# patrickzbhe/ray-tracing-series-rust

Hardware: AMD Instinct MI355X
Metric: Msamples/s (pixels x spp) on Book-1 final scene (higher is better)
Workload: dtype f64

## Files before the change

### include/rtx_abi.h

```cpp
#ifndef RTX_ABI_H
#define RTX_ABI_H

#include <stddef.h>
#include <stdint.h>

#ifdef __cplusplus
extern "C" {
#endif

#define RTX_ABI_VERSION 1

typedef int32_t rtx_status;
#define RTX_OK 0
#define RTX_EINVAL 1
#define RTX_ENOMEM 2
#define RTX_EHIP 3
#define RTX_EUNSUPPORTED 4
#define RTX_EIO 5
#define RTX_ENCCL 6

typedef int32_t rtx_handle;

typedef struct rtx_builder rtx_builder;
typedef struct rtx_flat rtx_flat;
typedef struct rtx_scene rtx_scene;

int32_t rtx_abi_version(void);
const char* rtx_last_error(void);

rtx_status rtx_builder_create(uint64_t scene_seed, rtx_builder** out);
void rtx_builder_destroy(rtx_builder* b);
double rtx_builder_random(rtx_builder* b);

rtx_handle rtx_solid_color(rtx_builder* b, const double rgb[3]);
rtx_handle rtx_checker(rtx_builder* b, rtx_handle even, rtx_handle odd);
rtx_handle rtx_noise(rtx_builder* b, double scale);
rtx_handle rtx_image_from_ppm(rtx_builder* b, const char* path);
rtx_handle rtx_image_from_texels(rtx_builder* b, int32_t width, int32_t height,
                                 const double* rgb_0_255);
rtx_handle rtx_lambertian(rtx_builder* b, rtx_handle texture);
rtx_handle rtx_metal(rtx_builder* b, const double albedo[3], double fuzz);
rtx_handle rtx_dielectric(rtx_builder* b, double ir);
rtx_handle rtx_diffuse_light(rtx_builder* b, rtx_handle texture);
rtx_handle rtx_isotropic(rtx_builder* b, rtx_handle texture);
rtx_handle rtx_sphere(rtx_builder* b, const double center[3], double radius, rtx_handle mat);
rtx_handle rtx_moving_sphere(rtx_builder* b, const double center0[3], const double center1[3],
                             double time0, double time1, double radius, rtx_handle mat);
rtx_handle rtx_gravity_sphere(rtx_builder* b, const double start[3], double time0, double radius, rtx_handle mat);
rtx_handle rtx_triangle(rtx_builder* b, const double v0[3], const double v1[3], const double v2[3],
                        rtx_handle mat);
rtx_handle rtx_xy_rect(rtx_builder* b, double x0, double x1, double y0, double y1, double k, rtx_handle mat);
rtx_handle rtx_xz_rect(rtx_builder* b, double x0, double x1, double y0, double y1, double k, rtx_handle mat);
rtx_handle rtx_yz_rect(rtx_builder* b, double x0, double x1, double y0, double y1, double k, rtx_handle mat);
rtx_handle rtx_rect_prism(rtx_builder* b, const double p0[3], const double p1[3], rtx_handle mat);
rtx_handle rtx_hittable_list_new(rtx_builder* b);
rtx_status rtx_hittable_list_add(rtx_builder* b, rtx_handle list, rtx_handle object);
rtx_handle rtx_bvh_from_list(rtx_builder* b, rtx_handle list, double time0, double time1);
rtx_handle rtx_translate(rtx_builder* b, const double offset[3], rtx_handle object);
rtx_handle rtx_rotate_y(rtx_builder* b, double angle_degrees, rtx_handle object);
rtx_handle rtx_constant_medium(rtx_builder* b, const double rgb[3], double density, rtx_handle boundary);
rtx_handle rtx_triangle_model(rtx_builder* b, const char* path, double scale);
rtx_handle rtx_triangle_mesh(rtx_builder* b, const double* vertices, int64_t n_vertices,
                             const int64_t* faces, int64_t n_faces, rtx_handle mat);

typedef struct RtxCamera {
  double origin[3], lower_left_corner[3], horizontal[3], vertical[3], u[3], v[3], w[3];
  double lens_radius, time1, time2;
} RtxCamera;
rtx_status rtx_camera_new(const double lookfrom[3], const double lookat[3], const double vup[3],
                          double vfov_degrees, double aspect_ratio, double aperture,
                          double focus_dist, double time1, double time2, RtxCamera* out);

typedef struct RtxConfig {
  double aspect_ratio;
  int32_t image_width;
  int32_t samples_per_pixel;
  int32_t max_depth;
  int32_t threads;
  uint64_t seed;
  double background[3];
  int32_t row_chunk_compat;
  int32_t reserved;
  uint64_t sample_buffer_bytes;
} RtxConfig;
rtx_status rtx_config_new(double aspect_ratio, int32_t image_width, int32_t samples_per_pixel,
                          int32_t max_depth, int32_t threads, RtxConfig* out);
int32_t rtx_image_height(const RtxConfig* cfg);

typedef struct RtxSceneOptions {
  double camera_aspect;
  const char* earth_ppm;
  const char* dragon_ply;
  int64_t mesh_triangles;
  int32_t book2_boxes_per_side;
  int32_t book2_spheres;
} RtxSceneOptions;
rtx_status rtx_get_world_cam(rtx_builder* b, int32_t scene_id, const RtxSceneOptions* options,
                             rtx_handle* world_out, RtxCamera* cam_out, double background_out[3]);

typedef struct RtxBuildOptions {
  int32_t max_leaf;
  int32_t sah_bins;
  int32_t reference_bvh;
  int32_t gpu_builder;
  uint64_t bvh_seed;
} RtxBuildOptions;
typedef struct RtxFlatInfo {
  int64_t n_spheres, n_moving_spheres, n_rects, n_triangles;
  int64_t n_nodes, n_refs, n_entries, n_top_level, n_materials, n_textures, n_perlins, n_images, n_texels;
  int64_t total_bytes;
  int32_t max_stack, n_bvh;
  double sah_cost;
  double bvh_build_ms;
  double bvh_device_ms;
  int64_t n_gravity_spheres;
} RtxFlatInfo;
rtx_status rtx_flatten(const rtx_builder* b, rtx_handle world, const RtxBuildOptions* options,
                       rtx_flat** out);
void rtx_flat_destroy(rtx_flat* f);
rtx_status rtx_flat_info(const rtx_flat* f, RtxFlatInfo* out);
int32_t rtx_flat_top_level_kind(const rtx_flat* f, int32_t index);
rtx_status rtx_scene_upload(const rtx_flat* f, rtx_scene** out);
rtx_status rtx_scene_upload_f32(const rtx_flat* f, rtx_scene** out);
int32_t rtx_scene_is_f32(const rtx_scene* s);
void rtx_scene_destroy(rtx_scene* s);
rtx_status rtx_scene_trim(rtx_scene* s);

typedef struct RtxFrame {
  double* accum_rgb;
  uint8_t* rgb8;
} RtxFrame;
typedef struct RtxRenderStats {
  uint64_t samples, rays, box_tests, sphere_tests, moving_sphere_tests, rect_tests, triangle_tests;
  uint64_t scatters, texels, perlin_calls;
  double trace_ms, reduce_ms, tonemap_ms;
  int32_t trace_launches, passes;
  uint64_t sample_buffer_bytes;
  int32_t trace_kernel;
  int32_t reserved;
} RtxRenderStats;
enum {
  RTX_KERNEL_SIMPLE = 0,
  RTX_KERNEL_PERSISTENT = 1,
  RTX_KERNEL_STREAM = 2,
  RTX_KERNEL_VOTE = 3,
  RTX_KERNEL_LDS = 4,
  RTX_KERNEL_WQ = 5,
  RTX_KERNEL_WORLD = 6,
  RTX_KERNEL_WAVEFRONT = 7
};
const char* rtx_trace_kernel_name(int32_t kernel);
rtx_status rtx_render(const rtx_scene* s, const RtxCamera* cam, const RtxConfig* cfg, RtxFrame* out);

typedef struct RtxShard {
  int32_t shard_index, shard_count, block_rows, reserved;
} RtxShard;
int32_t rtx_shard_rows(const RtxConfig* cfg, const RtxShard* shard);
rtx_status rtx_render_device(const rtx_scene* s, const RtxCamera* cam, const RtxConfig* cfg,
                             const RtxShard* shard, double* d_accum_rgb, uint8_t* d_rgb8,
                             void* hip_stream, RtxRenderStats* stats);
rtx_status rtx_render_count(const rtx_scene* s, const RtxCamera* cam, const RtxConfig* cfg,
                            const RtxShard* shard, RtxRenderStats* stats);

typedef struct rtx_multi rtx_multi;
typedef struct RtxMultiStats {
  double render_ms_max;
  double total_ms;
  uint64_t gathered_bytes;
  int32_t n_shards, n_devices, used_rccl;
  int32_t rccl_ranks;
  double gather_ms;
  double render_ms[16];
} RtxMultiStats;
rtx_status rtx_multi_create(const rtx_flat* f, int32_t n_shards, const int32_t* device_ids, int32_t block_rows,
                            rtx_multi** out);
rtx_status rtx_multi_create_f32(const rtx_flat* f, int32_t n_shards, const int32_t* device_ids, int32_t block_rows,
                                rtx_multi** out);
void rtx_multi_destroy(rtx_multi* m);
rtx_status rtx_multi_render(rtx_multi* m, const RtxCamera* cam, const RtxConfig* cfg, RtxFrame* out, RtxMultiStats* stats);
rtx_status rtx_render_multi(const rtx_flat* f, const RtxCamera* cam, const RtxConfig* cfg, int32_t n_gpus, RtxFrame* out);

typedef struct rtx_progressive rtx_progressive;
typedef struct RtxNoiseStats {
  int32_t spp_done;
  int32_t pixels;
  int32_t pixels_above;
  int32_t reserved;
  double max_rel_err, mean_rel_err, target_rel_err;
} RtxNoiseStats;
rtx_status rtx_progressive_create(const rtx_scene* s, const RtxCamera* cam, const RtxConfig* cfg, const RtxShard* shard,
                                  rtx_progressive** out);
void rtx_progressive_destroy(rtx_progressive* p);
int32_t rtx_progressive_spp(const rtx_progressive* p);
rtx_status rtx_progressive_add(rtx_progressive* p, int32_t n_samples, void* hip_stream, RtxRenderStats* stats);
rtx_status rtx_progressive_read(const rtx_progressive* p, RtxFrame* out, double* sumsq_rgb);
rtx_status rtx_progressive_stats(rtx_progressive* p, double target_rel_err, RtxNoiseStats* out);
rtx_status rtx_progressive_until(rtx_progressive* p, int32_t batch, double target_rel_err, RtxNoiseStats* out);

typedef struct RtxAdaptiveStats {
  int32_t spp_done;
  int32_t min_spp;
  int32_t pixels;
  int32_t pixels_active;
  int32_t pixels_above;
  int32_t reserved;
  uint64_t samples;
  double max_rel_err, mean_rel_err;
  double target_rel_err;
} RtxAdaptiveStats;
rtx_status rtx_progressive_add_adaptive(rtx_progressive* p, int32_t n_samples, int32_t min_spp, double target_rel_err,
                                        void* hip_stream, RtxRenderStats* stats);
rtx_status rtx_progressive_until_adaptive(rtx_progressive* p, int32_t batch, int32_t min_spp, double target_rel_err,
                                          RtxAdaptiveStats* out);
rtx_status rtx_progressive_pixel_spp(const rtx_progressive* p, int32_t* spp);

typedef struct RtxDenoiseParams {
  int32_t iterations, feature_spp, demodulate, reserved;
  double sigma_luminance, sigma_normal, sigma_albedo;
} RtxDenoiseParams;
rtx_status rtx_progressive_features(rtx_progressive* p, int32_t feature_spp, float* albedo_rgb, float* normal_xyz);
rtx_status rtx_progressive_denoise(rtx_progressive* p, const RtxDenoiseParams* params, double* mean_rgb, uint8_t* rgb8);
rtx_status rtx_device_denoise(const double* mean_rgb, const double* var_rgb, const float* albedo_rgb, const float* normal_xyz,
                              int32_t width, int32_t height, const RtxDenoiseParams* params, double* out_mean_rgb,
                              uint8_t* out_rgb8);

rtx_status rtx_render_scene_with_time(const rtx_scene* s, double t0, double t1, const char* path, int32_t row_chunk_compat,
                                      const RtxConfig* overrides);

rtx_status rtx_write_ppm(const char* path, int32_t width, int32_t height, const uint8_t* rgb8);

rtx_status rtx_device_math(int32_t fn, const double* x, const double* y, int64_t n, double* out);
rtx_status rtx_device_stream(uint64_t seed, uint64_t pixel, uint32_t sample, int32_t n, double* out);
rtx_status rtx_device_retire(const double* S, const double* Q, uint32_t npix, const uint32_t* active, uint32_t n,
                             uint32_t spp, double target, int32_t* counts, uint32_t* next, uint32_t* kept);
rtx_status rtx_device_noise_reduce(const double* S, const double* Q, const int32_t* counts, uint32_t npix, uint32_t spp,
                                   double target, double* max_r, double* sum_r, uint64_t* above);

const void* rtx_builder_graph(const rtx_builder* b);
const void* rtx_flat_arrays(const rtx_flat* f);

#ifdef __cplusplus
}
#endif
#endif
```

### ray-tracing-series-rust_amd/api.py

```python
import ctypes as C
import os
import sys

import numpy as np

_PKG_DIR = os.path.dirname(os.path.abspath(__file__))
_LIB_PATH = os.environ.get("RTX_LIBRARY") or os.path.join(_PKG_DIR, "lib", "librtx_hip.so")

RTX_OK, RTX_EINVAL, RTX_ENOMEM, RTX_EHIP, RTX_EUNSUPPORTED, RTX_EIO, RTX_ENCCL = 0, 1, 2, 3, 4, 5, 6
_STATUS_NAMES = {0: "RTX_OK", 1: "RTX_EINVAL", 2: "RTX_ENOMEM", 3: "RTX_EHIP", 4: "RTX_EUNSUPPORTED", 5: "RTX_EIO", 6: "RTX_ENCCL"}

SCENE_CHECKERED_SPHERES, SCENE_TWO_PERLIN, SCENE_EARTH, SCENE_SIMPLE_LIGHT = 0, 1, 2, 3
SCENE_CORNELL_BOX, SCENE_CORNELL_SMOKE, SCENE_BOOK2_FINAL, SCENE_MOVING_TEST = 4, 5, 6, 7
SCENE_RANDOM_MOVING, SCENE_BENCHMARK_TEST, SCENE_TRIANGLE_TEST, SCENE_STANFORD_DRAGON = 8, 9, 10, 11
SCENE_TRIANGULAR_PRISM, SCENE_BOOK1_HEAD, SCENE_BOOK1_CANONICAL, SCENE_EMPTY = 12, 13, 100, 101


class RtxError(RuntimeError):
    def __init__(self, status, message):
        super().__init__("%s: %s" % (_STATUS_NAMES.get(status, status), message))
        self.status = status


class RtxCamera(C.Structure):
    _fields_ = [(n, C.c_double * 3) for n in ("origin", "lower_left_corner", "horizontal", "vertical", "u", "v", "w")] + \
               [("lens_radius", C.c_double), ("time1", C.c_double), ("time2", C.c_double)]


class RtxConfig(C.Structure):
    _fields_ = [("aspect_ratio", C.c_double), ("image_width", C.c_int32), ("samples_per_pixel", C.c_int32),
                ("max_depth", C.c_int32), ("threads", C.c_int32), ("seed", C.c_uint64),
                ("background", C.c_double * 3), ("row_chunk_compat", C.c_int32), ("reserved", C.c_int32),
                ("sample_buffer_bytes", C.c_uint64)]


class RtxSceneOptions(C.Structure):
    _fields_ = [("camera_aspect", C.c_double), ("earth_ppm", C.c_char_p), ("dragon_ply", C.c_char_p),
                ("mesh_triangles", C.c_int64), ("book2_boxes_per_side", C.c_int32), ("book2_spheres", C.c_int32)]


class RtxBuildOptions(C.Structure):
    _fields_ = [("max_leaf", C.c_int32), ("sah_bins", C.c_int32), ("reference_bvh", C.c_int32), ("gpu_builder", C.c_int32),
                ("bvh_seed", C.c_uint64)]


class RtxFlatInfo(C.Structure):
    _fields_ = [(n, C.c_int64) for n in ("n_spheres", "n_moving_spheres", "n_rects", "n_triangles", "n_nodes",
                                         "n_refs", "n_entries", "n_top_level", "n_materials", "n_textures",
                                         "n_perlins", "n_images", "n_texels", "total_bytes")] + \
               [("max_stack", C.c_int32), ("n_bvh", C.c_int32), ("sah_cost", C.c_double), ("bvh_build_ms", C.c_double),
                ("bvh_device_ms", C.c_double), ("n_gravity_spheres", C.c_int64)]


class RtxFrame(C.Structure):
    _fields_ = [("accum_rgb", C.POINTER(C.c_double)), ("rgb8", C.POINTER(C.c_uint8))]


class RtxRenderStats(C.Structure):
    _fields_ = [(n, C.c_uint64) for n in ("samples", "rays", "box_tests", "sphere_tests", "moving_sphere_tests",
                                          "rect_tests", "triangle_tests", "scatters", "texels", "perlin_calls")] + \
               [("trace_ms", C.c_double), ("reduce_ms", C.c_double), ("tonemap_ms", C.c_double),
                ("trace_launches", C.c_int32), ("passes", C.c_int32), ("sample_buffer_bytes", C.c_uint64),
                ("trace_kernel", C.c_int32), ("reserved", C.c_int32)]


class RtxMultiStats(C.Structure):
    _fields_ = [("render_ms_max", C.c_double), ("total_ms", C.c_double), ("gathered_bytes", C.c_uint64),
                ("n_shards", C.c_int32), ("n_devices", C.c_int32), ("used_rccl", C.c_int32), ("rccl_ranks", C.c_int32),
                ("gather_ms", C.c_double), ("render_ms", C.c_double * 16)]


class RtxShard(C.Structure):
    _fields_ = [("shard_index", C.c_int32), ("shard_count", C.c_int32), ("block_rows", C.c_int32), ("reserved", C.c_int32)]


class RtxNoiseStats(C.Structure):
    _fields_ = [("spp_done", C.c_int32), ("pixels", C.c_int32), ("pixels_above", C.c_int32), ("reserved", C.c_int32),
                ("max_rel_err", C.c_double), ("mean_rel_err", C.c_double), ("target_rel_err", C.c_double)]


class RtxAdaptiveStats(C.Structure):
    _fields_ = [("spp_done", C.c_int32), ("min_spp", C.c_int32), ("pixels", C.c_int32), ("pixels_active", C.c_int32),
                ("pixels_above", C.c_int32), ("reserved", C.c_int32), ("samples", C.c_uint64),
                ("max_rel_err", C.c_double), ("mean_rel_err", C.c_double), ("target_rel_err", C.c_double)]


class RtxDenoiseParams(C.Structure):
    _fields_ = [("iterations", C.c_int32), ("feature_spp", C.c_int32), ("demodulate", C.c_int32), ("reserved", C.c_int32),
                ("sigma_luminance", C.c_double), ("sigma_normal", C.c_double), ("sigma_albedo", C.c_double)]


_D3 = C.POINTER(C.c_double)
_F3 = C.POINTER(C.c_float)
_VP = C.c_void_p
_H = C.c_int32
ABI = {
    "rtx_abi_version": (C.c_int32, []),
    "rtx_last_error": (C.c_char_p, []),
    "rtx_trace_kernel_name": (C.c_char_p, [C.c_int32]),
    "rtx_builder_create": (C.c_int32, [C.c_uint64, C.POINTER(_VP)]),
    "rtx_builder_destroy": (None, [_VP]),
    "rtx_builder_random": (C.c_double, [_VP]),
    "rtx_solid_color": (_H, [_VP, _D3]),
    "rtx_checker": (_H, [_VP, _H, _H]),
    "rtx_noise": (_H, [_VP, C.c_double]),
    "rtx_image_from_ppm": (_H, [_VP, C.c_char_p]),
    "rtx_image_from_texels": (_H, [_VP, C.c_int32, C.c_int32, _D3]),
    "rtx_lambertian": (_H, [_VP, _H]),
    "rtx_metal": (_H, [_VP, _D3, C.c_double]),
    "rtx_dielectric": (_H, [_VP, C.c_double]),
    "rtx_diffuse_light": (_H, [_VP, _H]),
    "rtx_isotropic": (_H, [_VP, _H]),
    "rtx_sphere": (_H, [_VP, _D3, C.c_double, _H]),
    "rtx_moving_sphere": (_H, [_VP, _D3, _D3, C.c_double, C.c_double, C.c_double, _H]),
    "rtx_triangle": (_H, [_VP, _D3, _D3, _D3, _H]),
    "rtx_gravity_sphere": (_H, [_VP, _D3, C.c_double, C.c_double, _H]),
    "rtx_render_scene_with_time": (C.c_int32, [_VP, C.c_double, C.c_double, C.c_char_p, C.c_int32, C.POINTER(RtxConfig)]),
    "rtx_xy_rect": (_H, [_VP] + [C.c_double] * 5 + [_H]),
    "rtx_xz_rect": (_H, [_VP] + [C.c_double] * 5 + [_H]),
    "rtx_yz_rect": (_H, [_VP] + [C.c_double] * 5 + [_H]),
    "rtx_rect_prism": (_H, [_VP, _D3, _D3, _H]),
    "rtx_hittable_list_new": (_H, [_VP]),
    "rtx_hittable_list_add": (C.c_int32, [_VP, _H, _H]),
    "rtx_bvh_from_list": (_H, [_VP, _H, C.c_double, C.c_double]),
    "rtx_translate": (_H, [_VP, _D3, _H]),
    "rtx_rotate_y": (_H, [_VP, C.c_double, _H]),
    "rtx_constant_medium": (_H, [_VP, _D3, C.c_double, _H]),
    "rtx_triangle_model": (_H, [_VP, C.c_char_p, C.c_double]),
    "rtx_triangle_mesh": (_H, [_VP, _D3, C.c_int64, C.POINTER(C.c_int64), C.c_int64, _H]),
    "rtx_camera_new": (C.c_int32, [_D3, _D3, _D3] + [C.c_double] * 6 + [C.POINTER(RtxCamera)]),
    "rtx_config_new": (C.c_int32, [C.c_double, C.c_int32, C.c_int32, C.c_int32, C.c_int32, C.POINTER(RtxConfig)]),
    "rtx_image_height": (C.c_int32, [C.POINTER(RtxConfig)]),
    "rtx_flat_top_level_kind": (C.c_int32, [_VP, C.c_int32]),
    "rtx_scene_trim": (C.c_int32, [_VP]),
    "rtx_multi_create": (C.c_int32, [_VP, C.c_int32, C.POINTER(C.c_int32), C.c_int32, C.POINTER(_VP)]),
    "rtx_multi_create_f32": (C.c_int32, [_VP, C.c_int32, C.POINTER(C.c_int32), C.c_int32, C.POINTER(_VP)]),
    "rtx_multi_destroy": (None, [_VP]),
    "rtx_multi_render": (C.c_int32, [_VP, C.POINTER(RtxCamera), C.POINTER(RtxConfig), C.POINTER(RtxFrame), C.POINTER(RtxMultiStats)]),
    "rtx_render_multi": (C.c_int32, [_VP, C.POINTER(RtxCamera), C.POINTER(RtxConfig), C.c_int32, C.POINTER(RtxFrame)]),
    "rtx_get_world_cam": (C.c_int32, [_VP, C.c_int32, C.POINTER(RtxSceneOptions), C.POINTER(_H), C.POINTER(RtxCamera), _D3]),
    "rtx_flatten": (C.c_int32, [_VP, _H, C.POINTER(RtxBuildOptions), C.POINTER(_VP)]),
    "rtx_flat_destroy": (None, [_VP]),
    "rtx_flat_info": (C.c_int32, [_VP, C.POINTER(RtxFlatInfo)]),
    "rtx_scene_upload": (C.c_int32, [_VP, C.POINTER(_VP)]),
    "rtx_scene_upload_f32": (C.c_int32, [_VP, C.POINTER(_VP)]),
    "rtx_scene_is_f32": (C.c_int32, [_VP]),
    "rtx_scene_destroy": (None, [_VP]),
    "rtx_render": (C.c_int32, [_VP, C.POINTER(RtxCamera), C.POINTER(RtxConfig), C.POINTER(RtxFrame)]),
    "rtx_shard_rows": (C.c_int32, [C.POINTER(RtxConfig), C.POINTER(RtxShard)]),
    "rtx_render_device": (C.c_int32, [_VP, C.POINTER(RtxCamera), C.POINTER(RtxConfig), C.POINTER(RtxShard),
                                      _VP, _VP, _VP, C.POINTER(RtxRenderStats)]),
    "rtx_render_count": (C.c_int32, [_VP, C.POINTER(RtxCamera), C.POINTER(RtxConfig), C.POINTER(RtxShard),
                                     C.POINTER(RtxRenderStats)]),
    "rtx_write_ppm": (C.c_int32, [C.c_char_p, C.c_int32, C.c_int32, C.POINTER(C.c_uint8)]),
    "rtx_device_math": (C.c_int32, [C.c_int32, _D3, _D3, C.c_int64, _D3]),
    "rtx_device_stream": (C.c_int32, [C.c_uint64, C.c_uint64, C.c_uint32, C.c_int32, _D3]),
    "rtx_device_retire": (C.c_int32, [_D3, _D3, C.c_uint32, C.POINTER(C.c_uint32), C.c_uint32, C.c_uint32, C.c_double,
                                      C.POINTER(C.c_int32), C.POINTER(C.c_uint32), C.POINTER(C.c_uint32)]),
    "rtx_device_noise_reduce": (C.c_int32, [_D3, _D3, C.POINTER(C.c_int32), C.c_uint32, C.c_uint32, C.c_double, _D3, _D3,
                                            C.POINTER(C.c_uint64)]),
    "rtx_progressive_create": (C.c_int32, [_VP, C.POINTER(RtxCamera), C.POINTER(RtxConfig), C.POINTER(RtxShard), C.POINTER(_VP)]),
    "rtx_progressive_destroy": (None, [_VP]),
    "rtx_progressive_spp": (C.c_int32, [_VP]),
    "rtx_progressive_add": (C.c_int32, [_VP, C.c_int32, _VP, C.POINTER(RtxRenderStats)]),
    "rtx_progressive_read": (C.c_int32, [_VP, C.POINTER(RtxFrame), _D3]),
    "rtx_progressive_stats": (C.c_int32, [_VP, C.c_double, C.POINTER(RtxNoiseStats)]),
    "rtx_progressive_until": (C.c_int32, [_VP, C.c_int32, C.c_double, C.POINTER(RtxNoiseStats)]),
    "rtx_progressive_add_adaptive": (C.c_int32, [_VP, C.c_int32, C.c_int32, C.c_double, _VP, C.POINTER(RtxRenderStats)]),
    "rtx_progressive_until_adaptive": (C.c_int32, [_VP, C.c_int32, C.c_int32, C.c_double, C.POINTER(RtxAdaptiveStats)]),
    "rtx_progressive_pixel_spp": (C.c_int32, [_VP, C.POINTER(C.c_int32)]),
    "rtx_progressive_features": (C.c_int32, [_VP, C.c_int32, _F3, _F3]),
    "rtx_progressive_denoise": (C.c_int32, [_VP, C.POINTER(RtxDenoiseParams), _D3, C.POINTER(C.c_uint8)]),
    "rtx_device_denoise": (C.c_int32, [_D3, _D3, _F3, _F3, C.c_int32, C.c_int32, C.POINTER(RtxDenoiseParams), _D3,
                                       C.POINTER(C.c_uint8)]),
    "rtx_builder_graph": (_VP, [_VP]),
    "rtx_flat_arrays": (_VP, [_VP]),
}


def _load():
    if not os.path.exists(_LIB_PATH):
        raise ImportError(
            "HIP library %s is missing: run `python __graft_entry__.py` (or ray-tracing-series-rust_amd/build.py). "
            "This package has no CPU fallback." % _LIB_PATH)
    lib = C.CDLL(_LIB_PATH)
    for name, (res, args) in ABI.items():
        fn = getattr(lib, name)
        fn.restype = res
        fn.argtypes = args
    return lib


lib = _load()
LIB_PATH = _LIB_PATH


def last_error():
    return (lib.rtx_last_error() or b"").decode("utf-8", "replace")


def _check(status):
    if status != RTX_OK:
        raise RtxError(status, last_error())


def _v3(v):
    a = (C.c_double * 3)(float(v[0]), float(v[1]), float(v[2]))
    return a


def _handle(h):
    if h < 0:
        raise RtxError(RTX_EINVAL, last_error())
    return h


class Camera:

    @staticmethod
    def new(lookfrom, lookat, vup, vfov, aspect_ratio, aperture, focus_dist, time1, time2):
        cam = RtxCamera()
        _check(lib.rtx_camera_new(_v3(lookfrom), _v3(lookat), _v3(vup), vfov, aspect_ratio, aperture, focus_dist,
                                  time1, time2, C.byref(cam)))
        return cam


class Config:

    @staticmethod
    def new(aspect_ratio, image_width, samples_per_pixel, max_depth, threads, seed=1, background=(0.7, 0.8, 1.0),
            row_chunk_compat=False, sample_buffer_bytes=0):
        cfg = RtxConfig()
        _check(lib.rtx_config_new(aspect_ratio, image_width, samples_per_pixel, max_depth, threads, C.byref(cfg)))
        cfg.seed = seed
        cfg.background[0], cfg.background[1], cfg.background[2] = background
        cfg.row_chunk_compat = 1 if row_chunk_compat else 0
        cfg.sample_buffer_bytes = sample_buffer_bytes
        return cfg


def image_height(cfg):
    return lib.rtx_image_height(C.byref(cfg))


class Builder:

    def __init__(self, scene_seed=1):
        p = _VP()
        _check(lib.rtx_builder_create(scene_seed, C.byref(p)))
        self._p = p

    def __del__(self):
        p, self._p = getattr(self, "_p", None), None
        if p:
            lib.rtx_builder_destroy(p)

    @property
    def ptr(self):
        return self._p

    def graph_ptr(self):
        return lib.rtx_builder_graph(self._p)

    def random(self):
        return lib.rtx_builder_random(self._p)

    def solid_color(self, rgb):
        return _handle(lib.rtx_solid_color(self._p, _v3(rgb)))

    def checker(self, even, odd):
        return _handle(lib.rtx_checker(self._p, even, odd))

    def checker_from_colors(self, even_rgb, odd_rgb):
        return self.checker(self.solid_color(even_rgb), self.solid_color(odd_rgb))

    def noise(self, scale):
        return _handle(lib.rtx_noise(self._p, scale))

    def image_from_ppm(self, path):
        return _handle(lib.rtx_image_from_ppm(self._p, os.fsencode(path)))

    def image_from_texels(self, texels):
        t = np.ascontiguousarray(texels, dtype=np.float64)
        h, w = t.shape[0], t.shape[1]
        return _handle(lib.rtx_image_from_texels(self._p, w, h, t.ctypes.data_as(_D3)))

    def lambertian(self, albedo):
        tex = albedo if isinstance(albedo, int) else self.solid_color(albedo)
        return _handle(lib.rtx_lambertian(self._p, tex))

    def metal(self, albedo, fuzz):
        return _handle(lib.rtx_metal(self._p, _v3(albedo), fuzz))

    def dielectric(self, ir):
        return _handle(lib.rtx_dielectric(self._p, ir))

    def diffuse_light(self, emit):
        tex = emit if isinstance(emit, int) else self.solid_color(emit)
        return _handle(lib.rtx_diffuse_light(self._p, tex))

    def isotropic(self, albedo):
        tex = albedo if isinstance(albedo, int) else self.solid_color(albedo)
        return _handle(lib.rtx_isotropic(self._p, tex))

    def sphere(self, center, radius, mat):
        return _handle(lib.rtx_sphere(self._p, _v3(center), radius, mat))

    def moving_sphere(self, center0, center1, time0, time1, radius, mat):
        return _handle(lib.rtx_moving_sphere(self._p, _v3(center0), _v3(center1), time0, time1, radius, mat))

    def gravity_sphere(self, start, time0, radius, mat):
        return _handle(lib.rtx_gravity_sphere(self._p, _v3(start), time0, radius, mat))

    def triangle(self, v0, v1, v2, mat):
        return _handle(lib.rtx_triangle(self._p, _v3(v0), _v3(v1), _v3(v2), mat))

    def xy_rect(self, x0, x1, y0, y1, k, mat):
        return _handle(lib.rtx_xy_rect(self._p, x0, x1, y0, y1, k, mat))

    def xz_rect(self, x0, x1, y0, y1, k, mat):
        return _handle(lib.rtx_xz_rect(self._p, x0, x1, y0, y1, k, mat))

    def yz_rect(self, x0, x1, y0, y1, k, mat):
        return _handle(lib.rtx_yz_rect(self._p, x0, x1, y0, y1, k, mat))

    def rect_prism(self, p0, p1, mat):
        return _handle(lib.rtx_rect_prism(self._p, _v3(p0), _v3(p1), mat))

    def hittable_list(self, objects=()):
        lst = _handle(lib.rtx_hittable_list_new(self._p))
        for o in objects:
            self.list_add(lst, o)
        return lst

    def list_add(self, lst, obj):
        _check(lib.rtx_hittable_list_add(self._p, lst, obj))

    def bvh_from_list(self, lst, time0, time1):
        return _handle(lib.rtx_bvh_from_list(self._p, lst, time0, time1))

    def translate(self, offset, obj):
        return _handle(lib.rtx_translate(self._p, _v3(offset), obj))

    def rotate_y(self, angle_degrees, obj):
        return _handle(lib.rtx_rotate_y(self._p, angle_degrees, obj))

    def constant_medium(self, rgb, density, boundary):
        return _handle(lib.rtx_constant_medium(self._p, _v3(rgb), density, boundary))

    def triangle_model(self, path, scale):
        return _handle(lib.rtx_triangle_model(self._p, os.fsencode(path), scale))

    def triangle_mesh(self, vertices, faces, mat):
        v = np.ascontiguousarray(vertices, dtype=np.float64).reshape(-1, 3)
        f = np.ascontiguousarray(faces, dtype=np.int64).reshape(-1, 3)
        return _handle(lib.rtx_triangle_mesh(self._p, v.ctypes.data_as(_D3), v.shape[0],
                                             f.ctypes.data_as(C.POINTER(C.c_int64)), f.shape[0], mat))

    def get_world_cam(self, scene_id, camera_aspect=0.0, earth_ppm=None, dragon_ply=None, mesh_triangles=0,
                      book2_boxes_per_side=0, book2_spheres=0):
        opt = RtxSceneOptions(camera_aspect, os.fsencode(earth_ppm) if earth_ppm else None,
                              os.fsencode(dragon_ply) if dragon_ply else None, mesh_triangles,
                              book2_boxes_per_side, book2_spheres)
        world = _H()
        cam = RtxCamera()
        bg = (C.c_double * 3)()
        _check(lib.rtx_get_world_cam(self._p, scene_id, C.byref(opt), C.byref(world), C.byref(cam), bg))
        return world.value, cam, (bg[0], bg[1], bg[2])

    def flatten(self, world, max_leaf=0, sah_bins=0, reference_bvh=False, bvh_seed=0, gpu_builder=False):
        return Flat(self, world, max_leaf, sah_bins, reference_bvh, bvh_seed, gpu_builder)


class Flat:

    def __init__(self, builder, world, max_leaf=0, sah_bins=0, reference_bvh=False, bvh_seed=0, gpu_builder=False):
        opt = RtxBuildOptions(max_leaf, sah_bins, 1 if reference_bvh else 0, 1 if gpu_builder else 0, bvh_seed)
        p = _VP()
        _check(lib.rtx_flatten(builder.ptr, world, C.byref(opt), C.byref(p)))
        self._p = p
        self._builder = builder

    def __del__(self):
        p, self._p = getattr(self, "_p", None), None
        if p:
            lib.rtx_flat_destroy(p)

    @property
    def ptr(self):
        return self._p

    def arrays_ptr(self):
        return lib.rtx_flat_arrays(self._p)

    def info(self):
        info = RtxFlatInfo()
        _check(lib.rtx_flat_info(self._p, C.byref(info)))
        return {n: getattr(info, n) for n, _ in RtxFlatInfo._fields_}

    def top_level_kinds(self):
        n = self.info()["n_top_level"]
        return [lib.rtx_flat_top_level_kind(self._p, i) for i in range(n)]

    def upload(self, f32=False):
        return Scene(self, f32=f32)


class Scene:

    def __init__(self, flat, f32=False):
        p = _VP()
        _check((lib.rtx_scene_upload_f32 if f32 else lib.rtx_scene_upload)(flat.ptr, C.byref(p)))
        self._p = p

    @property
    def is_f32(self):
        return bool(lib.rtx_scene_is_f32(self._p))

    def __del__(self):
        p, self._p = getattr(self, "_p", None), None
        if p:
            lib.rtx_scene_destroy(p)

    @property
    def ptr(self):
        return self._p

    def render(self, cam, cfg, want_accum=True):
        w, h = cfg.image_width, image_height(cfg)
        accum = np.zeros((h, w, 3), dtype=np.float64) if want_accum else None
        rgb8 = np.zeros((h, w, 3), dtype=np.uint8)
        frame = RtxFrame(accum.ctypes.data_as(C.POINTER(C.c_double)) if want_accum else None,
                         rgb8.ctypes.data_as(C.POINTER(C.c_uint8)))
        _check(lib.rtx_render(self._p, C.byref(cam), C.byref(cfg), C.byref(frame)))
        return Screen(w, h, rgb8, accum)

    def trim(self):
        _check(lib.rtx_scene_trim(self._p))

    def render_scene_with_time(self, t0, t1, path, row_chunk_compat=True, overrides=None):
        _check(lib.rtx_render_scene_with_time(self._p, t0, t1, path.encode(), 1 if row_chunk_compat else 0,
                                              C.byref(overrides) if overrides is not None else None))

    def render_device(self, cam, cfg, shard=None, d_accum=0, d_rgb8=0, stream=0, want_stats=False):
        sh = RtxShard(*shard, 0) if shard is not None else None
        stats = RtxRenderStats() if want_stats else None
        _check(lib.rtx_render_device(self._p, C.byref(cam), C.byref(cfg), C.byref(sh) if sh else None,
                                     _VP(d_accum or None), _VP(d_rgb8 or None), _VP(stream or None),
                                     C.byref(stats) if stats else None))
        return stats

    def progressive(self, cam, cfg, shard=None):
        return Progressive(self, cam, cfg, shard)

    def render_count(self, cam, cfg, shard=None):
        sh = RtxShard(*shard, 0) if shard is not None else None
        stats = RtxRenderStats()
        _check(lib.rtx_render_count(self._p, C.byref(cam), C.byref(cfg), C.byref(sh) if sh else None, C.byref(stats)))
        return stats


class Progressive:

    def __init__(self, scene, cam, cfg, shard=None):
        self.scene = scene
        self.width = cfg.image_width
        self.height = shard_rows(cfg, shard) if shard is not None else image_height(cfg)
        sh = RtxShard(*shard, 0) if shard is not None else None
        p = _VP()
        _check(lib.rtx_progressive_create(scene.ptr, C.byref(cam), C.byref(cfg), C.byref(sh) if sh else None, C.byref(p)))
        self._p = p

    def __del__(self):
        p, self._p = getattr(self, "_p", None), None
        if p:
            lib.rtx_progressive_destroy(p)

    @property
    def spp_done(self):
        return lib.rtx_progressive_spp(self._p)

    def add(self, n, stream=0, want_stats=False):
        stats = RtxRenderStats() if want_stats else None
        _check(lib.rtx_progressive_add(self._p, n, _VP(stream or None), C.byref(stats) if stats else None))
        return stats

    def screen(self, want_accum=True):
        accum = np.zeros((self.height, self.width, 3), dtype=np.float64) if want_accum else None
        rgb8 = np.zeros((self.height, self.width, 3), dtype=np.uint8)
        frame = RtxFrame(accum.ctypes.data_as(_D3) if want_accum else None, rgb8.ctypes.data_as(C.POINTER(C.c_uint8)))
        _check(lib.rtx_progressive_read(self._p, C.byref(frame), None))
        return Screen(self.width, self.height, rgb8, accum)

    def moments(self):
        s = np.zeros((self.height, self.width, 3), dtype=np.float64)
        q = np.zeros_like(s)
        frame = RtxFrame(s.ctypes.data_as(_D3), None)
        _check(lib.rtx_progressive_read(self._p, C.byref(frame), q.ctypes.data_as(_D3)))
        return s, q

    def stats(self, target_rel_err=0.0):
        out = RtxNoiseStats()
        _check(lib.rtx_progressive_stats(self._p, target_rel_err, C.byref(out)))
        return out

    def until(self, batch, target_rel_err):
        out = RtxNoiseStats()
        _check(lib.rtx_progressive_until(self._p, batch, target_rel_err, C.byref(out)))
        return out

    def add_adaptive(self, n, min_spp, target_rel_err, stream=0, want_stats=False):
        stats = RtxRenderStats() if want_stats else None
        _check(lib.rtx_progressive_add_adaptive(self._p, n, min_spp, target_rel_err, _VP(stream or None),
                                                C.byref(stats) if stats else None))
        return stats

    def until_adaptive(self, batch, min_spp, target_rel_err):
        out = RtxAdaptiveStats()
        _check(lib.rtx_progressive_until_adaptive(self._p, batch, min_spp, target_rel_err, C.byref(out)))
        return out

    def pixel_spp(self):
        out = np.zeros((self.height, self.width), dtype=np.int32)
        _check(lib.rtx_progressive_pixel_spp(self._p, out.ctypes.data_as(C.POINTER(C.c_int32))))
        return out

    def features(self, feature_spp=4):
        albedo = np.zeros((self.height, self.width, 3), dtype=np.float32)
        normal = np.zeros_like(albedo)
        _check(lib.rtx_progressive_features(self._p, feature_spp, albedo.ctypes.data_as(_F3), normal.ctypes.data_as(_F3)))
        return albedo, normal

    def denoise(self, **params):
        prm = denoise_params(**params)
        accum = np.zeros((self.height, self.width, 3), dtype=np.float64)
        rgb8 = np.zeros((self.height, self.width, 3), dtype=np.uint8)
        _check(lib.rtx_progressive_denoise(self._p, C.byref(prm), accum.ctypes.data_as(_D3),
                                           rgb8.ctypes.data_as(C.POINTER(C.c_uint8))))
        return Screen(self.width, self.height, rgb8, accum)


class MultiScene:

    def __init__(self, flat, n_shards, device_ids=None, block_rows=1, f32=False):
        ids = (C.c_int32 * n_shards)(*device_ids) if device_ids is not None else None
        p = _VP()
        _check((lib.rtx_multi_create_f32 if f32 else lib.rtx_multi_create)(flat.ptr, n_shards, ids, block_rows, C.byref(p)))
        self._p = p

    def __del__(self):
        p, self._p = getattr(self, "_p", None), None
        if p:
            lib.rtx_multi_destroy(p)

    def render(self, cam, cfg, want_accum=True):
        w, h = cfg.image_width, image_height(cfg)
        accum = np.zeros((h, w, 3), dtype=np.float64) if want_accum else None
        rgb8 = np.zeros((h, w, 3), dtype=np.uint8)
        frame = RtxFrame(accum.ctypes.data_as(C.POINTER(C.c_double)) if want_accum else None,
                         rgb8.ctypes.data_as(C.POINTER(C.c_uint8)))
        stats = RtxMultiStats()
        _check(lib.rtx_multi_render(self._p, C.byref(cam), C.byref(cfg), C.byref(frame), C.byref(stats)))
        screen = Screen(w, h, rgb8, accum)
        screen.stats = stats
        return screen


def render_multi(flat, cam, cfg, n_gpus, want_accum=True):
    w, h = cfg.image_width, image_height(cfg)
    accum = np.zeros((h, w, 3), dtype=np.float64) if want_accum else None
    rgb8 = np.zeros((h, w, 3), dtype=np.uint8)
    frame = RtxFrame(accum.ctypes.data_as(C.POINTER(C.c_double)) if want_accum else None,
                     rgb8.ctypes.data_as(C.POINTER(C.c_uint8)))
    _check(lib.rtx_render_multi(flat.ptr, C.byref(cam), C.byref(cfg), n_gpus, C.byref(frame)))
    return Screen(w, h, rgb8, accum)


def trace_kernel_name(kernel):
    return (lib.rtx_trace_kernel_name(kernel) or b"").decode()


def device_math(fn, x, y=None):
    names = {"sin": 0, "cos": 1, "log": 2, "acos": 3, "atan2": 4, "tan": 5, "sqrt": 6, "div": 7, "muladd": 8, "floor": 9, "wide_key": 10}
    x = np.ascontiguousarray(x, dtype=np.float64)
    y = np.ascontiguousarray(y if y is not None else np.ones_like(x), dtype=np.float64)
    out = np.empty_like(x)
    _check(lib.rtx_device_math(names[fn], x.ctypes.data_as(_D3), y.ctypes.data_as(_D3), x.size, out.ctypes.data_as(_D3)))
    return out


def device_stream(seed, pixel, sample, n):
    out = np.empty(n, dtype=np.float64)
    _check(lib.rtx_device_stream(seed, pixel, sample, n, out.ctypes.data_as(_D3)))
    return out


def _moments_arg(S, Q):
    S = np.ascontiguousarray(S, dtype=np.float64).reshape(-1, 3)
    Q = np.ascontiguousarray(Q, dtype=np.float64).reshape(-1, 3)
    if S.shape != Q.shape:
        raise ValueError("S and Q must have the same shape")
    return S, Q


def device_retire(S, Q, active, spp, target, counts):
    S, Q = _moments_arg(S, Q)
    active = np.ascontiguousarray(active, dtype=np.uint32).ravel()
    counts = np.array(counts, dtype=np.int32).ravel()
    if counts.size != S.shape[0]:
        raise ValueError("counts must hold one entry per pixel")
    nxt = np.zeros(max(active.size, 1), dtype=np.uint32)
    kept = C.c_uint32()
    u32 = C.POINTER(C.c_uint32)
    _check(lib.rtx_device_retire(S.ctypes.data_as(_D3), Q.ctypes.data_as(_D3), S.shape[0], active.ctypes.data_as(u32),
                                 active.size, spp, target, counts.ctypes.data_as(C.POINTER(C.c_int32)), nxt.ctypes.data_as(u32),
                                 C.byref(kept)))
    return nxt[:kept.value].copy(), counts


def device_noise_reduce(S, Q, spp, target, counts=None):
    S, Q = _moments_arg(S, Q)
    if counts is not None:
        counts = np.ascontiguousarray(counts, dtype=np.int32).ravel()
        if counts.size != S.shape[0]:
            raise ValueError("counts must hold one entry per pixel")
    max_r, sum_r, above = C.c_double(), C.c_double(), C.c_uint64()
    _check(lib.rtx_device_noise_reduce(S.ctypes.data_as(_D3), Q.ctypes.data_as(_D3),
                                       counts.ctypes.data_as(C.POINTER(C.c_int32)) if counts is not None else None,
                                       S.shape[0], spp, target, C.byref(max_r), C.byref(sum_r), C.byref(above)))
    return max_r.value, sum_r.value, above.value


def denoise_params(**params):
    prm = RtxDenoiseParams()
    names = [n for n, _ in RtxDenoiseParams._fields_ if n != "reserved"]
    for k, v in params.items():
        if k not in names:
            raise TypeError("unknown denoise parameter %r (expected one of %s)" % (k, ", ".join(names)))
        setattr(prm, k, v)
    return prm


def device_denoise(mean, var, albedo, normal, **params):
    mean = np.ascontiguousarray(mean, dtype=np.float64)
    if mean.ndim != 3 or mean.shape[2] != 3:
        raise ValueError("mean must be rows x width x 3")
    var = np.ascontiguousarray(var, dtype=np.float64)
    albedo = np.ascontiguousarray(albedo, dtype=np.float32)
    normal = np.ascontiguousarray(normal, dtype=np.float32)
    for a in (var, albedo, normal):
        if a.shape != mean.shape:
            raise ValueError("mean, var, albedo and normal must have the same shape")
    h, w = mean.shape[:2]
    prm = denoise_params(**params)
    out = np.zeros_like(mean)
    rgb8 = np.zeros(mean.shape, dtype=np.uint8)
    _check(lib.rtx_device_denoise(mean.ctypes.data_as(_D3), var.ctypes.data_as(_D3), albedo.ctypes.data_as(_F3),
                                  normal.ctypes.data_as(_F3), w, h, C.byref(prm), out.ctypes.data_as(_D3),
                                  rgb8.ctypes.data_as(C.POINTER(C.c_uint8))))
    return out, rgb8


def shard_rows(cfg, shard):
    sh = RtxShard(*shard, 0)
    return lib.rtx_shard_rows(C.byref(cfg), C.byref(sh))


class Screen:

    def __init__(self, width, height, rgb8, accum=None):
        self.width, self.height, self.rgb8, self.accum = width, height, rgb8, accum

    def write_to_ppm_file(self, path):
        buf = np.ascontiguousarray(self.rgb8)
        _check(lib.rtx_write_ppm(os.fsencode(path), self.width, self.height, buf.ctypes.data_as(C.POINTER(C.c_uint8))))

    def write_to_ppm(self):
        sys.stdout.flush()
        buf = np.ascontiguousarray(self.rgb8)
        _check(lib.rtx_write_ppm(None, self.width, self.height, buf.ctypes.data_as(C.POINTER(C.c_uint8))))


def render_scene(builder, world, cam, background, config, max_leaf=0):
    cfg = RtxConfig.from_buffer_copy(config)
    cfg.background[0], cfg.background[1], cfg.background[2] = background
    scene = builder.flatten(world, max_leaf=max_leaf).upload()
    return scene.render(cam, cfg)


def render_scene_progressive(builder, world, cam, background, config, batch, target_rel_err, max_leaf=0, adaptive=False,
                             min_spp=2, denoise=False):
    cfg = RtxConfig.from_buffer_copy(config)
    cfg.background[0], cfg.background[1], cfg.background[2] = background
    scene = builder.flatten(world, max_leaf=max_leaf).upload()
    prog = scene.progressive(cam, cfg)
    if adaptive:
        stats = prog.until_adaptive(batch, min_spp, target_rel_err)
    else:
        stats = prog.until(batch, target_rel_err)
    screen = prog.screen()
    if adaptive:
        screen.spp = prog.pixel_spp()
    if denoise:
        noisy, screen = screen, prog.denoise()
        screen.noisy = noisy
        if adaptive:
            screen.spp = noisy.spp
    return screen, stats
```

### ray-tracing-series-rust_amd/build.py

```python
import os
import shutil
import subprocess
import sys

PKG_DIR = os.path.dirname(os.path.abspath(__file__))
REPO_DIR = os.path.dirname(PKG_DIR)
LIB_DIR = os.path.join(PKG_DIR, "lib")
LIB_PATH = os.path.join(LIB_DIR, "librtx_hip.so")
APP_PATH = os.path.join(LIB_DIR, "rtx_render")

HIP_SOURCES = [
    "csrc/hip/render.hip",
    "csrc/hip/render_f32.hip",
    "csrc/hip/lbvh.hip",
    "csrc/hip/abi.cpp",
    "csrc/host/scene_graph.cpp",
    "csrc/host/flatten.cpp",
    "csrc/host/bvh_build.cpp",
    "csrc/host/scenes.cpp",
]
HIP_FLAGS = [
    "--offload-arch=gfx950", "-O3", "-std=c++17", "-ffp-contract=off", "-fPIC",
    "-Wall", "-Wno-unused-function",
]
LICM_FLAGS = ["-Xarch_device", "-mllvm=-disable-machine-licm"]
CFG_FLAGS = ["-Xarch_device", "-mllvm=-structurizecfg-skip-uniform-regions"]
TRACE_SOURCES = ("csrc/hip/render.hip", "csrc/hip/render_f32.hip")
_probed = {}


def _accepted(flags):
    key = " ".join(flags)
    if key not in _probed:
        import tempfile
        with tempfile.TemporaryDirectory() as td:
            src = os.path.join(td, "probe.hip")
            with open(src, "w") as f:
                f.write("#include <hip/hip_runtime.h>\n__global__ void k(float* p) { p[threadIdx.x] = 1.f; }\n")
            rc = subprocess.run([_hipcc(), "--offload-arch=gfx950", "-O3", "-c", src, "-o", os.path.join(td, "probe.o")] + flags,
                                stdout=subprocess.DEVNULL, stderr=subprocess.DEVNULL).returncode
        _probed[key] = list(flags) if rc == 0 else []
    return _probed[key]


def licm_flags():
    return _accepted(LICM_FLAGS)


def cfg_flags():
    return _accepted(CFG_FLAGS)


def trace_flags():
    return licm_flags() + cfg_flags()


def flags_for(src):
    return HIP_FLAGS + (trace_flags() if src in TRACE_SOURCES else []) + os.environ.get("RTX_EXTRA_HIPFLAGS", "").split()


def _hipcc():
    for cand in (shutil.which("hipcc"), "/opt/rocm/bin/hipcc"):
        if cand and os.path.exists(cand):
            return cand
    raise RuntimeError("hipcc not found: the HIP library cannot be built")


def _newest(paths):
    t = 0.0
    for p in paths:
        for root, _, files in os.walk(p) if os.path.isdir(p) else [(os.path.dirname(p), [], [os.path.basename(p)])]:
            for f in files:
                fp = os.path.join(root, f)
                if os.path.exists(fp):
                    t = max(t, os.path.getmtime(fp))
    return t


def needs_build(target, deps):
    return (not os.path.exists(target)) or os.path.getmtime(target) < _newest(deps)


def build_library(force=False, verbose=True):
    deps = [os.path.join(PKG_DIR, "csrc"), os.path.join(REPO_DIR, "include")]
    if not force and not needs_build(LIB_PATH, deps):
        return LIB_PATH
    obj_dir = os.path.join(LIB_DIR, "obj")
    os.makedirs(obj_dir, exist_ok=True)
    jobs = []
    for src in HIP_SOURCES:
        obj = os.path.join(obj_dir, os.path.basename(src).rsplit(".", 1)[0] + ".o")
        if force or needs_build(obj, deps):
            cmd = [_hipcc()] + flags_for(src) + ["-c", os.path.join(PKG_DIR, src), "-o", obj]
            if verbose:
                print("[build]", " ".join(cmd), flush=True)
            jobs.append((cmd, subprocess.Popen(cmd, cwd=PKG_DIR)))
        else:
            jobs.append((None, None))
    for cmd, proc in jobs:
        if proc is not None and proc.wait() != 0:
            for _, other in jobs:
                if other is not None:
                    other.wait()
            raise subprocess.CalledProcessError(proc.returncode, cmd)
    objs = [os.path.join(obj_dir, os.path.basename(src).rsplit(".", 1)[0] + ".o") for src in HIP_SOURCES]
    cmd = [_hipcc(), "--offload-arch=gfx950", "-fPIC", "-shared"] + objs + ["-o", LIB_PATH]
    if verbose:
        print("[build]", " ".join(cmd), flush=True)
    subprocess.run(cmd, check=True, cwd=PKG_DIR)
    import json
    with open(os.path.join(LIB_DIR, "build_flags.json"), "w") as f:
        json.dump({"hip_flags": HIP_FLAGS, "trace_kernel_flags": trace_flags(), "machine_licm_disabled": bool(licm_flags()),
                   "uniform_regions_not_structurized": bool(cfg_flags()), "trace_sources": list(TRACE_SOURCES)}, f, indent=1)
    return LIB_PATH


def build_roofline_tools(force=False, verbose=True):
    mix = os.path.join(LIB_DIR, "kernel_mix.json")
    calib = os.path.join(LIB_DIR, "issue_calib")
    tools = os.path.join(REPO_DIR, "tools")
    deps = [os.path.join(PKG_DIR, "csrc")] + [os.path.join(tools, f) for f in sorted(os.listdir(tools)) if os.path.isfile(os.path.join(tools, f))]
    if not force and not needs_build(mix, deps) and not needs_build(calib, deps):
        return mix
    gen_dir = os.path.join(tools, "_gen")
    os.makedirs(gen_dir, exist_ok=True)
    asm = os.path.join(gen_dir, "render_gfx950.s")
    flags = [f for f in flags_for("csrc/hip/render.hip") if f != "-fPIC"]
    cmds = [
        [_hipcc()] + flags + ["-S", "--cuda-device-only", os.path.join(PKG_DIR, "csrc/hip/render.hip"), "-o", asm],
        [sys.executable, os.path.join(tools, "kernel_mix.py"), asm, mix],
        [sys.executable, os.path.join(tools, "gen_issue_calib.py"), asm, os.path.join(gen_dir, "issue_calib_auto.hip")],
        [_hipcc(), "--offload-arch=gfx950", "-O1", "-std=c++17", os.path.join(gen_dir, "issue_calib_auto.hip"), "-o", calib],
    ]
    for cmd in cmds:
        if verbose:
            print("[build]", " ".join(cmd), flush=True)
        subprocess.run(cmd, check=True, cwd=PKG_DIR)
    return mix


def build_app(force=False, verbose=True):
    src = os.path.join(PKG_DIR, "apps", "rtx_render.cpp")
    if not os.path.exists(src):
        return None
    if not force and not needs_build(APP_PATH, [src, LIB_PATH]):
        return APP_PATH
    cmd = [_hipcc(), "-O2", "-std=c++17", "-ffp-contract=off", src, "-I", os.path.join(REPO_DIR, "include"),
           "-L", LIB_DIR, "-lrtx_hip", "-Wl,-rpath,$ORIGIN", "-o", APP_PATH]
    if verbose:
        print("[build]", " ".join(cmd), flush=True)
    subprocess.run(cmd, check=True, cwd=PKG_DIR)
    return APP_PATH


if __name__ == "__main__":
    force = "--force" in sys.argv
    build_library(force=force)
    build_app(force=force)
    build_roofline_tools(force=force)
```

### ray-tracing-series-rust_amd/csrc/hip/abi.cpp

```cpp
#include <cstdio>
#include <cstdlib>
#include <cstring>
#include <new>
#include <string>
#include "../host/scenes.hpp"
#include "abi_internal.hpp"

namespace rtx {
static thread_local std::string g_last_error;
void set_error(const std::string& msg) { g_last_error = msg; }
}

using namespace rtx;

namespace {
inline rtx_handle checked(rtx_builder* b, int32_t h) {
  if (h < 0) set_error(b->graph.error.empty() ? "invalid argument" : b->graph.error);
  return h;
}
#define NEED_BUILDER(b)                                  \
  if (!(b)) { set_error("NULL builder"); return -1; }
}

extern "C" {

int32_t rtx_abi_version(void) { return RTX_ABI_VERSION; }
const char* rtx_last_error(void) { return g_last_error.c_str(); }
const char* rtx_trace_kernel_name(int32_t kernel) {
  switch (kernel) {
    case RTX_KERNEL_SIMPLE: return "k_trace_simple";
    case RTX_KERNEL_PERSISTENT: return "k_trace_persistent";
    case RTX_KERNEL_STREAM: return "k_trace_stream";
    case RTX_KERNEL_VOTE: return "k_trace_vote";
    case RTX_KERNEL_LDS: return "k_trace_lds";
    case RTX_KERNEL_WQ: return "k_trace_wq";
    case RTX_KERNEL_WORLD: return "k_trace_world";
    case RTX_KERNEL_WAVEFRONT: return "k_wf_trace";
    default: return "?";
  }
}

rtx_status rtx_builder_create(uint64_t scene_seed, rtx_builder** out) {
  if (!out) { set_error("rtx_builder_create: NULL out"); return RTX_EINVAL; }
  *out = new (std::nothrow) rtx_builder(scene_seed);
  if (!*out) { set_error("out of memory"); return RTX_ENOMEM; }
  return RTX_OK;
}
void rtx_builder_destroy(rtx_builder* b) { delete b; }
double rtx_builder_random(rtx_builder* b) { return b ? rt::host_rng_f64(b->graph.rng) : 0.0; }

rtx_handle rtx_solid_color(rtx_builder* b, const double rgb[3]) { NEED_BUILDER(b); if (!rgb) { set_error("NULL rgb"); return -1; } return checked(b, b->graph.solid_color(rgb)); }
rtx_handle rtx_checker(rtx_builder* b, rtx_handle even, rtx_handle odd) { NEED_BUILDER(b); return checked(b, b->graph.checker(even, odd)); }
rtx_handle rtx_noise(rtx_builder* b, double scale) { NEED_BUILDER(b); return checked(b, b->graph.noise(scale)); }
rtx_handle rtx_image_from_ppm(rtx_builder* b, const char* path) { NEED_BUILDER(b); if (!path) { set_error("NULL path"); return -1; } return checked(b, b->graph.image_from_ppm(path)); }
rtx_handle rtx_image_from_texels(rtx_builder* b, int32_t w, int32_t h, const double* t) { NEED_BUILDER(b); return checked(b, b->graph.image_from_texels(w, h, t)); }

rtx_handle rtx_lambertian(rtx_builder* b, rtx_handle tex) { NEED_BUILDER(b); return checked(b, b->graph.lambertian(tex)); }
rtx_handle rtx_metal(rtx_builder* b, const double albedo[3], double fuzz) { NEED_BUILDER(b); if (!albedo) { set_error("NULL albedo"); return -1; } return checked(b, b->graph.metal(albedo, fuzz)); }
rtx_handle rtx_dielectric(rtx_builder* b, double ir) { NEED_BUILDER(b); return checked(b, b->graph.dielectric(ir)); }
rtx_handle rtx_diffuse_light(rtx_builder* b, rtx_handle tex) { NEED_BUILDER(b); return checked(b, b->graph.diffuse_light(tex)); }
rtx_handle rtx_isotropic(rtx_builder* b, rtx_handle tex) { NEED_BUILDER(b); return checked(b, b->graph.isotropic(tex)); }

rtx_handle rtx_sphere(rtx_builder* b, const double c[3], double r, rtx_handle mat) { NEED_BUILDER(b); if (!c) { set_error("NULL center"); return -1; } return checked(b, b->graph.sphere(c, r, mat)); }
rtx_handle rtx_gravity_sphere(rtx_builder* b, const double start[3], double time0, double radius, rtx_handle mat) {
  if (!b || !start) { set_error("rtx_gravity_sphere: NULL argument"); return -1; }
  return checked(b, b->graph.gravity_sphere(start, time0, radius, mat));
}
rtx_handle rtx_moving_sphere(rtx_builder* b, const double c0[3], const double c1[3], double t0, double t1, double r, rtx_handle mat) {
  NEED_BUILDER(b);
  if (!c0 || !c1) { set_error("NULL center"); return -1; }
  return checked(b, b->graph.moving_sphere(c0, c1, t0, t1, r, mat));
}
rtx_handle rtx_triangle(rtx_builder* b, const double v0[3], const double v1[3], const double v2[3], rtx_handle mat) {
  NEED_BUILDER(b);
  if (!v0 || !v1 || !v2) { set_error("NULL vertex"); return -1; }
  return checked(b, b->graph.triangle(v0, v1, v2, mat));
}
rtx_handle rtx_xy_rect(rtx_builder* b, double x0, double x1, double y0, double y1, double k, rtx_handle mat) { NEED_BUILDER(b); return checked(b, b->graph.rect(H_XY_RECT, x0, x1, y0, y1, k, mat)); }
rtx_handle rtx_xz_rect(rtx_builder* b, double x0, double x1, double y0, double y1, double k, rtx_handle mat) { NEED_BUILDER(b); return checked(b, b->graph.rect(H_XZ_RECT, x0, x1, y0, y1, k, mat)); }
rtx_handle rtx_yz_rect(rtx_builder* b, double x0, double x1, double y0, double y1, double k, rtx_handle mat) { NEED_BUILDER(b); return checked(b, b->graph.rect(H_YZ_RECT, x0, x1, y0, y1, k, mat)); }
rtx_handle rtx_rect_prism(rtx_builder* b, const double p0[3], const double p1[3], rtx_handle mat) {
  NEED_BUILDER(b);
  if (!p0 || !p1) { set_error("NULL corner"); return -1; }
  return checked(b, b->graph.rect_prism(p0, p1, mat));
}
rtx_handle rtx_hittable_list_new(rtx_builder* b) { NEED_BUILDER(b); return b->graph.list_new(); }
rtx_status rtx_hittable_list_add(rtx_builder* b, rtx_handle list, rtx_handle object) {
  if (!b) { set_error("NULL builder"); return RTX_EINVAL; }
  if (!b->graph.list_add(list, object)) { set_error(b->graph.error); return RTX_EINVAL; }
  return RTX_OK;
}
rtx_handle rtx_bvh_from_list(rtx_builder* b, rtx_handle list, double t0, double t1) { NEED_BUILDER(b); return checked(b, b->graph.bvh_from_list(list, t0, t1)); }
rtx_handle rtx_translate(rtx_builder* b, const double offset[3], rtx_handle obj) { NEED_BUILDER(b); if (!offset) { set_error("NULL offset"); return -1; } return checked(b, b->graph.translate(offset, obj)); }
rtx_handle rtx_rotate_y(rtx_builder* b, double angle, rtx_handle obj) { NEED_BUILDER(b); return checked(b, b->graph.rotate_y(angle, obj)); }
rtx_handle rtx_constant_medium(rtx_builder* b, const double rgb[3], double density, rtx_handle boundary) {
  NEED_BUILDER(b);
  if (!rgb) { set_error("NULL rgb"); return -1; }
  return checked(b, b->graph.constant_medium(rgb, density, boundary));
}
rtx_handle rtx_triangle_model(rtx_builder* b, const char* path, double scale) { NEED_BUILDER(b); if (!path) { set_error("NULL path"); return -1; } return checked(b, b->graph.triangle_model(path, scale)); }
rtx_handle rtx_triangle_mesh(rtx_builder* b, const double* vertices, int64_t n_vertices, const int64_t* faces, int64_t n_faces, rtx_handle mat) {
  NEED_BUILDER(b);
  if (!vertices || !faces || n_vertices < 0 || n_faces < 0) { set_error("triangle_mesh: NULL or negative"); return -1; }
  return checked(b, b->graph.triangle_mesh(vertices, n_vertices, faces, n_faces, mat));
}

rtx_status rtx_camera_new(const double lookfrom[3], const double lookat[3], const double vup[3],
                          double vfov, double aspect_ratio, double aperture, double focus_dist,
                          double time1, double time2, RtxCamera* out) {
  if (!lookfrom || !lookat || !vup || !out) { set_error("rtx_camera_new: NULL argument"); return RTX_EINVAL; }
  if (!(time1 < time2)) { set_error("rtx_camera_new: time1 >= time2 (gen_range(time1..time2) panics, camera.rs:69)"); return RTX_EINVAL; }
  rt::FlatCamera c = camera_new(lookfrom, lookat, vup, vfov, aspect_ratio, aperture, focus_dist, time1, time2);
  static_assert(sizeof(RtxCamera) == sizeof(rt::FlatCamera), "camera layout");
  memcpy(out, &c, sizeof(c));
  return RTX_OK;
}

rtx_status rtx_config_new(double aspect_ratio, int32_t image_width, int32_t samples_per_pixel,
                          int32_t max_depth, int32_t threads, RtxConfig* out) {
  if (!out) { set_error("rtx_config_new: NULL out"); return RTX_EINVAL; }
  if (threads <= 0) { set_error("Config::new: assert!(threads > 0)"); return RTX_EINVAL; }
  if (image_width <= 0) { set_error("Config::new: assert!(image_width > 0)"); return RTX_EINVAL; }
  if (samples_per_pixel <= 0) { set_error("Config::new: assert!(samples_per_pixel > 0)"); return RTX_EINVAL; }
  if (max_depth <= 0) { set_error("Config::new: assert!(max_depth > 0)"); return RTX_EINVAL; }
  memset(out, 0, sizeof(*out));
  out->aspect_ratio = aspect_ratio;
  out->image_width = image_width;
  out->samples_per_pixel = samples_per_pixel;
  out->max_depth = max_depth;
  out->threads = threads;
  out->seed = 1;
  out->background[0] = 0.7; out->background[1] = 0.8; out->background[2] = 1.0;
  return RTX_OK;
}

int32_t rtx_image_height(const RtxConfig* cfg) {
  if (!cfg) return 0;
  return rt::rt_f64_as_i32((double)cfg->image_width / cfg->aspect_ratio);
}

int32_t rtx_shard_rows(const RtxConfig* cfg, const RtxShard* shard) {
  if (!cfg) return 0;
  int32_t h = rtx_image_height(cfg);
  RtxShard sh = {0, 1, 1, 0};
  if (shard) sh = *shard;
  if (sh.shard_count <= 0 || sh.block_rows <= 0) return 0;
  int n = 0;
  for (int32_t j = 0; j < h; ++j)
    if ((j / sh.block_rows) % sh.shard_count == sh.shard_index) ++n;
  return n;
}

rtx_status rtx_get_world_cam(rtx_builder* b, int32_t scene_id, const RtxSceneOptions* options,
                             rtx_handle* world_out, RtxCamera* cam_out, double background_out[3]) {
  if (!b || !world_out || !cam_out || !background_out) { set_error("rtx_get_world_cam: NULL argument"); return RTX_EINVAL; }
  SceneOptions opt;
  if (options) {
    opt.camera_aspect = options->camera_aspect;
    opt.earth_ppm = options->earth_ppm;
    opt.dragon_ply = options->dragon_ply;
    if (options->mesh_triangles > 0) opt.mesh_triangles = options->mesh_triangles;
    if (options->book2_boxes_per_side > 0) opt.book2_boxes_per_side = options->book2_boxes_per_side;
    if (options->book2_spheres > 0) opt.book2_spheres = options->book2_spheres;
  }
  WorldCam wc;
  std::string err;
  if (!get_world_cam(b->graph, scene_id, opt, &wc, &err)) {
    set_error(err);
    return scene_id == RTX_SCENE_RANDOM_MOVING ? RTX_EUNSUPPORTED : RTX_EINVAL;
  }
  *world_out = wc.world;
  memcpy(cam_out, &wc.cam, sizeof(wc.cam));
  background_out[0] = wc.background[0]; background_out[1] = wc.background[1]; background_out[2] = wc.background[2];
  return RTX_OK;
}

rtx_status rtx_flatten(const rtx_builder* b, rtx_handle world, const RtxBuildOptions* options, rtx_flat** out) {
  if (!b || !out) { set_error("rtx_flatten: NULL argument"); return RTX_EINVAL; }
  *out = nullptr;
  BuildOptions opt;
  if (options) {
    if (options->max_leaf > 0) opt.max_leaf = options->max_leaf;
    if (options->sah_bins > 0) opt.sah_bins = options->sah_bins;
    opt.reference_bvh = options->reference_bvh ? 1 : 0;
    opt.gpu_builder = options->gpu_builder ? 1 : 0;
    if (options->bvh_seed) opt.bvh_seed = options->bvh_seed;
  }
  if (const char* e = getenv("RTX_LEAF_FIRST")) opt.leaf_first = atoi(e) != 0 ? 1 : 0;
  if (const char* e = getenv("RTX_MOTION_TOPOLOGY")) opt.motion_topology = atoi(e) != 0 ? 1 : 0;
  rtx_flat* f = new (std::nothrow) rtx_flat();
  if (!f) { set_error("out of memory"); return RTX_ENOMEM; }
  std::string err;
  if (!b->graph.valid_hittable(world)) { delete f; set_error("rtx_flatten: bad world handle"); return RTX_EINVAL; }
  if (!flatten_scene(b->graph, world, opt, &f->scene, &err)) {
    delete f;
    set_error(err);
    return RTX_EUNSUPPORTED;
  }
  *out = f;
  return RTX_OK;
}
void rtx_flat_destroy(rtx_flat* f) { delete f; }

rtx_status rtx_flat_info(const rtx_flat* f, RtxFlatInfo* o) {
  if (!f || !o) { set_error("rtx_flat_info: NULL argument"); return RTX_EINVAL; }
  const FlatScene& s = f->scene;
  o->n_spheres = (int64_t)s.spheres.size(); o->n_moving_spheres = (int64_t)s.moving_spheres.size();
  o->n_rects = (int64_t)s.rects.size(); o->n_triangles = (int64_t)s.triangles.size();
  o->n_nodes = (int64_t)s.nodes.size(); o->n_refs = (int64_t)s.refs.size();
  o->n_entries = (int64_t)s.entries.size(); o->n_top_level = (int64_t)s.top_level.size();
  o->n_materials = (int64_t)s.materials.size(); o->n_textures = (int64_t)s.textures.size();
  o->n_perlins = (int64_t)s.perlins.size(); o->n_images = (int64_t)s.images.size();
  o->n_texels = (int64_t)(s.texels.size() / 3);
  o->total_bytes = (int64_t)s.total_bytes();
  o->max_stack = s.max_stack; o->n_bvh = s.n_bvh; o->sah_cost = s.sah_cost;
  o->bvh_build_ms = s.bvh_build_ms; o->bvh_device_ms = s.bvh_device_ms;
  o->n_gravity_spheres = (int64_t)s.gravity_spheres.size();
  return RTX_OK;
}

int32_t rtx_flat_top_level_kind(const rtx_flat* f, int32_t index) {
  if (!f || index < 0 || (size_t)index >= f->scene.top_level.size()) return -1;
  return f->scene.entries[f->scene.top_level[index]].kind;
}

rtx_status rtx_write_ppm(const char* path, int32_t width, int32_t height, const uint8_t* rgb8) {
  if (width <= 0 || height <= 0 || !rgb8) { set_error("rtx_write_ppm: bad argument"); return RTX_EINVAL; }
  FILE* fp = stdout;
  bool to_file = path && strcmp(path, "-") != 0;
  if (to_file) {
    fp = fopen(path, "wb");
    if (!fp) { set_error(std::string("rtx_write_ppm: cannot open ") + path); return RTX_EIO; }
  }
  std::string buf;
  buf.reserve((size_t)width * height * 12 + 32);
  char line[64];
  snprintf(line, sizeof(line), "P3\n%d %d\n255\n", width, height);
  buf += line;
  for (int32_t j = height - 1; j >= 0; --j) {
    for (int32_t i = 0; i < width; ++i) {
      const uint8_t* p = rgb8 + 3 * ((size_t)j * width + i);
      int n = snprintf(line, sizeof(line), "%u %u %u\n", (unsigned)p[0], (unsigned)p[1], (unsigned)p[2]);
      buf.append(line, (size_t)n);
    }
  }
  size_t wrote = fwrite(buf.data(), 1, buf.size(), fp);
  if (to_file) fclose(fp); else fflush(fp);
  if (wrote != buf.size()) { set_error("rtx_write_ppm: short write"); return RTX_EIO; }
  return RTX_OK;
}

const void* rtx_builder_graph(const rtx_builder* b) { return b ? (const void*)&b->graph : nullptr; }
const void* rtx_flat_arrays(const rtx_flat* f) { return f ? (const void*)&f->scene : nullptr; }

}
```

### ray-tracing-series-rust_amd/csrc/hip/render.hip

```cpp
#include <hip/hip_runtime.h>
#include <cstdio>
#include <cstdlib>
#include <algorithm>
#include <chrono>
#include <cfloat>
#include <cmath>
#include <cstring>
#include <new>
#include <type_traits>
#include <utility>
#include <string>
#include <vector>
#include "../../../include/rtx_abi.h"
#include "../core/cull32.hpp"
#include "../core/integrator.hpp"
#include "../host/flat_scene.hpp"
#include "f32_bridge.hpp"
#ifndef RTX_F32_TU
#include "abi_internal.hpp"
#else
namespace rtx { void set_error(const std::string& msg); }
#endif

namespace rtx {

#include "pass_items.inc"

struct FlatNode4;
typedef const FlatNode4 FlatNode4Dev;
struct WorldDesc;

struct LdsSceneDims {
  uint32_t n_nodes, n_refs, n_spheres, n_moving;
  uint32_t node_dwords;
  uint32_t n_uni;
};

struct VoteTop {
  int32_t n;
  int32_t all_rects;
  int32_t k[8];
  uint32_t ref[8];
  rt::FlatRect rect[8];
};

enum class ForcedKernel { none, simple, vote, world, wavefront };

struct TraceSwitches {
  ForcedKernel kernel = ForcedKernel::none;
  bool diag = false;
  int ring = -1, wide = -1, scene_lds = -1;
  bool vote_top = true, tri_direct = true, mat_lds = true, perlin_lds = true;
  bool mv_common = true, motion = true, motion_axis = true;
  bool single_leaf = true, pass_pipeline = true, validate = false;
  uint32_t chunk = TRACE_CHUNK;
  uint32_t world_threshold = 8;
  uint32_t walk_threshold = 0, regen_min = 0, leaf_weight = 0;
  uint32_t wf_paths = 1u << 22, wf_refill = 16, wf_check = 8;
  int wf_occ = 4;
  bool wf_verbose = false;
};

struct Workspace {
  double* samples = nullptr;
  size_t samples_bytes = 0;
  double* accum = nullptr;
  size_t accum_bytes = 0;
  rt::TraceCounters* counters = nullptr;
  unsigned int* work_counter = nullptr;
  unsigned long long* diag = nullptr;
  hipEvent_t ev[2] = {nullptr, nullptr};
  hipStream_t aux_stream = nullptr;
  hipEvent_t ev_pass[3] = {nullptr, nullptr, nullptr};
  void* wave_mem = nullptr;
  size_t wave_bytes = 0;
  uint32_t* wave_host_ctrl = nullptr;
};

struct VotePlan {
  bool ok = false;
  int32_t bvh_pos = 0;
  int32_t tri_base = -1;
  VoteTop top;
  int blocks_per_cu[2] = {1, 1};
  bool ring[2] = {false, false};
  uint32_t tables = 0;
  size_t tables_bytes = 0;
};

struct WidePlan {
  FlatNode4Dev* nodes4 = nullptr;
  int levels = 0;
  int vote_blocks_per_cu = 1;
};

struct WorldPlan {
  const WorldDesc* desc = nullptr;
  uint32_t mat_lds = 0, tex_lds = 0;
  uint32_t perlin_lds = 0;
  int blocks_per_cu[4][2] = {{1, 1}, {1, 1}, {1, 1}, {1, 1}};
};

struct LdsFit {
  bool ok = false;
  uint32_t ring_cap = 0;
  uint32_t levels = 0;
  LdsSceneDims dims = {0, 0, 0, 0, 0, 0};
};

struct LdsPlan {
  LdsFit plain;
  LdsFit motion;
  int motion_axis = -1;
  double motion_t0 = 0.0, motion_t1 = 0.0;
  bool mv_common = false;
  double mv_t0 = 0.0, mv_t1 = 1.0;
};

struct WalkTuning {
  uint32_t walk_threshold = 18;
  uint32_t regen_min = 1;
  uint32_t leaf_weight = 3;
  bool single_leaf = false;
};

struct DeviceScene {
  int device = -1;
  std::vector<void*> allocations;
  rt::SceneView view;
  size_t scene_bytes = 0;
  int n_cu = 256;
  double gravity_time_limit = 1e300;
  TraceSwitches sw;
  Workspace ws;
  VotePlan vote;
  WidePlan wide;
  WorldPlan world;
  LdsPlan lds;
  WalkTuning walk;
};

#define HIP_TRY(expr)                                                                      \
  do {                                                                                     \
    hipError_t _e = (expr);                                                                \
    if (_e != hipSuccess) {                                                                \
      set_error(std::string(#expr) + ": " + hipGetErrorString(_e));                        \
      return RTX_EHIP;                                                                     \
    }                                                                                      \
  } while (0)

template <class T>
static rtx_status upload_array(DeviceScene* ds, const std::vector<T>& v, const T** out) {
  *out = nullptr;
  if (v.empty()) return RTX_OK;
  void* p = nullptr;
  size_t bytes = v.size() * sizeof(T);
  HIP_TRY(hipMalloc(&p, bytes));
  ds->allocations.push_back(p);
  HIP_TRY(hipMemcpy(p, v.data(), bytes, hipMemcpyHostToDevice));
  ds->scene_bytes += bytes;
  *out = (const T*)p;
  return RTX_OK;
}

static void free_device_scene(DeviceScene* ds) {
  if (!ds) return;
  Workspace& ws = ds->ws;
  for (void* p : ds->allocations) (void)hipFree(p);
  if (ws.samples) (void)hipFree(ws.samples);
  if (ws.accum) (void)hipFree(ws.accum);
  if (ws.counters) (void)hipFree(ws.counters);
  if (ws.work_counter) (void)hipFree(ws.work_counter);
  if (ws.diag) (void)hipFree(ws.diag);
  if (ws.wave_mem) (void)hipFree(ws.wave_mem);
  if (ws.wave_host_ctrl) (void)hipHostFree(ws.wave_host_ctrl);
  for (int i = 0; i < 2; ++i)
    if (ws.ev[i]) (void)hipEventDestroy(ws.ev[i]);
  for (int i = 0; i < 3; ++i)
    if (ws.ev_pass[i]) (void)hipEventDestroy(ws.ev_pass[i]);
  if (ws.aux_stream) (void)hipStreamDestroy(ws.aux_stream);
  delete ds;
}

template <class T>
__device__ __forceinline__ T dev_load_uniform(const T* p) { return *(const __attribute__((address_space(4))) T*)(p); }

__device__ __forceinline__ unsigned long long wave_ballot(bool p) { return __builtin_amdgcn_ballot_w64(p); }

#define TRACE_BLOCK 256
struct LdsStack {
  int32_t* base;
  int n;
  static constexpr bool kBottom = false;
  __device__ __forceinline__ void reset() { n = 0; }
  __device__ __forceinline__ void push(int32_t v) { base[n * TRACE_BLOCK] = v; ++n; }
  __device__ __forceinline__ int32_t pop() { --n; return base[n * TRACE_BLOCK]; }
  __device__ __forceinline__ bool empty() const { return n == 0; }
};
struct LdsStackB {
  int32_t* base;
  int n;
  static constexpr bool kBottom = true;
  __device__ __forceinline__ void reset() { base[0] = 0x7fffffff; n = 1; }
  __device__ __forceinline__ void init() { reset(); }
  __device__ __forceinline__ void push(int32_t v) { base[n * TRACE_BLOCK] = v; ++n; }
  __device__ __forceinline__ int32_t pop() { --n; return base[n * TRACE_BLOCK]; }
  __device__ __forceinline__ int32_t top() const { return base[(n - 1) * TRACE_BLOCK]; }
  __device__ __forceinline__ bool empty() const { return n <= 1; }
};

__device__ __forceinline__ void flush_counters(const rt::TraceCounters& c, rt::TraceCounters* g) {
  atomicAdd(&g->box_tests, c.box_tests);
  atomicAdd(&g->sphere_tests, c.sphere_tests);
  atomicAdd(&g->moving_sphere_tests, c.moving_sphere_tests);
  atomicAdd(&g->rect_tests, c.rect_tests);
  atomicAdd(&g->triangle_tests, c.triangle_tests);
  atomicAdd(&g->scatters, c.scatters);
  atomicAdd(&g->texels, c.texels);
  atomicAdd(&g->perlin_calls, c.perlin_calls);
  atomicAdd(&g->rays, c.rays);
  atomicAdd(&g->samples, c.samples);
}

#include "trace_basic.inc"
#include "trace_vote.inc"
#include "trace_world.inc"
#include "trace_lds.inc"
#include "trace_wave.inc"
#include "post_kernels.inc"
#include "denoise.inc"

static int shard_row_count(int32_t height, const RtxShard& sh, int32_t row_limit) {
  int n = 0;
  for (int32_t j = 0; j < height && j < row_limit; ++j)
    if ((j / sh.block_rows) % sh.shard_count == sh.shard_index) ++n;
  return n;
}

static rtx_status validate(const void* s, const RtxCamera* cam, const RtxConfig* cfg,
                           const RtxShard* shard, RtxShard* sh_out) {
  if (!s || !cam || !cfg) { set_error("render: NULL scene, camera or config"); return RTX_EINVAL; }
  if (cfg->threads <= 0 || cfg->image_width <= 0 || cfg->samples_per_pixel <= 0 || cfg->max_depth <= 0) {
    set_error("render: Config::new asserts threads, image_width, samples_per_pixel, max_depth > 0 (world.rs:36-40)");
    return RTX_EINVAL;
  }
  if (rtx_image_height(cfg) <= 0) { set_error("render: image height <= 0 (Screen::new asserts, screen.rs:14)"); return RTX_EINVAL; }
  if (!(cam->time1 < cam->time2)) { set_error("render: camera time1 >= time2 (gen_range panics on an empty range, camera.rs:69)"); return RTX_EINVAL; }
  RtxShard sh = {0, 1, 1, 0};
  if (shard) sh = *shard;
  if (sh.shard_count <= 0 || sh.shard_index < 0 || sh.shard_index >= sh.shard_count || sh.block_rows <= 0) {
    set_error("render: bad shard");
    return RTX_EINVAL;
  }
  *sh_out = sh;
  return RTX_OK;
}

static rt::RenderParams make_params(const RtxCamera* cam, const RtxConfig* cfg) {
  rt::RenderParams rp;
  static_assert(sizeof(RtxCamera) == 24 * sizeof(double) && sizeof(rt::FlatCamera) == 24 * sizeof(rt::real), "camera layout");
  for (int k = 0; k < 24; ++k) ((rt::real*)&rp.cam)[k] = (rt::real)((const double*)cam)[k];
  rp.background = rt::v3(cfg->background[0], cfg->background[1], cfg->background[2]);
  rp.image_width = cfg->image_width;
  rp.image_height = rtx_image_height(cfg);
  rp.samples_per_pixel = cfg->samples_per_pixel;
  rp.max_depth = cfg->max_depth;
  rp.seed = cfg->seed;
  return rp;
}

static TraceSwitches read_switches() {
  auto num = [](const char* n, int lo, int hi, uint32_t dflt) { const char* s = getenv(n); return s && atoi(s) >= lo && atoi(s) <= hi ? (uint32_t)atoi(s) : dflt; };
  auto flag = [](const char* n) { const char* s = getenv(n); return s ? (atoi(s) != 0 ? 1 : 0) : -1; };
  TraceSwitches sw;
  if (const char* k = getenv("RTX_TRACE_KERNEL")) {
    const std::string s = k;
    if (s == "simple") sw.kernel = ForcedKernel::simple;
    else if (s == "vote" || s == "vote_diag") sw.kernel = ForcedKernel::vote;
    else if (s == "world" || s == "world_diag") sw.kernel = ForcedKernel::world;
    else if (s == "wavefront") sw.kernel = ForcedKernel::wavefront;
    sw.diag = s == "vote_diag" || s == "world_diag";
  }
  sw.ring = flag("RTX_RING"); sw.wide = flag("RTX_WIDE"); sw.scene_lds = flag("RTX_SCENE_LDS");
  sw.vote_top = flag("RTX_VOTE_TOP") != 0; sw.tri_direct = flag("RTX_TRI_DIRECT") != 0;
  sw.mat_lds = flag("RTX_MAT_LDS") != 0; sw.perlin_lds = flag("RTX_PERLIN_LDS") != 0;
  sw.mv_common = flag("RTX_MV_COMMON") != 0; sw.motion = flag("RTX_MOTION") != 0; sw.motion_axis = flag("RTX_MOTION_AXIS") != 0;
  sw.single_leaf = flag("RTX_SINGLE_LEAF") != 0; sw.pass_pipeline = flag("RTX_PASS_PIPELINE") != 0;
  sw.validate = getenv("RTX_VALIDATE") != nullptr;
  sw.chunk = num("RTX_CHUNK", 64, 65536, sw.chunk);
  sw.world_threshold = num("RTX_WORLD_THRESHOLD", 0, 64, sw.world_threshold);
  sw.walk_threshold = num("RTX_WALK_THRESHOLD", 1, 64, 0); sw.regen_min = num("RTX_REGEN_MIN", 1, 64, 0); sw.leaf_weight = num("RTX_LEAF_WEIGHT", 1, 64, 0);
  const char* wp = getenv("RTX_WF_PATHS");
  if (wp && atol(wp) >= 256 && atol(wp) <= (1l << 27)) sw.wf_paths = (uint32_t)atol(wp);
  sw.wf_refill = num("RTX_WF_REFILL", 1, 64, sw.wf_refill); sw.wf_check = num("RTX_WF_CHECK", 1, 4096, sw.wf_check);
  sw.wf_occ = (int)num("RTX_WF_OCC", 4, 6, (uint32_t)sw.wf_occ); sw.wf_verbose = getenv("RTX_WF_VERBOSE") != nullptr;
  return sw;
}

static size_t stack_bytes(uint32_t levels) { return (size_t)levels * TRACE_BLOCK * sizeof(int32_t); }

template <class K>
static int occupancy(K kernel, size_t lds) {
  int nb = 0;
  return hipOccupancyMaxActiveBlocksPerMultiprocessor(&nb, kernel, TRACE_BLOCK, lds) == hipSuccess ? nb : 0;
}

static uint32_t grid_size(uint32_t total, uint32_t block, uint64_t resident) {
  const uint64_t want = ((uint64_t)total + block - 1) / block;
  return (uint32_t)(want < resident ? want : resident);
}

static rtx_status grow_buffer(void** p, size_t* bytes, size_t need, hipStream_t stream) {
  if (need <= *bytes) return RTX_OK;
  if (*p) { HIP_TRY(hipStreamSynchronize(stream)); HIP_TRY(hipFree(*p)); *p = nullptr; *bytes = 0; }
  HIP_TRY(hipMalloc(p, need));
  *bytes = need;
  return RTX_OK;
}

struct PassArgs {
  rt::RenderParams rp;
  ShardMap sm;
  uint32_t s_begin, total, npix;
  double* samples;
  unsigned int* work_counter;
  hipStream_t stream;
  int preset;
  uint32_t feat;
  uint32_t stack_levels;
  size_t stack_lds;
  const uint32_t* active;
};

template <class Launch>
static void with_map(const PassArgs& a, Launch launch) {
  if (a.active) launch(ActiveMap{a.sm, a.active});
  else launch(a.sm);
}

template <class Launch>
static rtx_status run_diag(DeviceScene* ds, hipStream_t stream, Launch launch, const char* tag, int width, const char* const* names,
                           int n, unsigned long long (&h)[24]) {
  if (!ds->ws.diag) HIP_TRY(hipMalloc((void**)&ds->ws.diag, sizeof(h)));
  HIP_TRY(hipMemsetAsync(ds->ws.diag, 0, sizeof(h), stream));
  launch();
  HIP_TRY(hipStreamSynchronize(stream));
  HIP_TRY(hipMemcpy(h, ds->ws.diag, sizeof(h), hipMemcpyDeviceToHost));
  for (int k = 0; k < n; ++k)
    fprintf(stderr, "[%s] %-*s executions %llu lanes %llu mean lanes %.2f\n", tag, width, names[k], h[2 * k], h[2 * k + 1],
            h[2 * k] ? (double)h[2 * k + 1] / (double)h[2 * k] : 0.0);
  return RTX_OK;
}

struct LeafScan { uint32_t max_count = 0, max_end = 0; };
static LeafScan scan_leaves(const FlatScene& fs) {
  LeafScan s;
  for (const rt::FlatNode& nd : fs.nodes)
    for (int ch = 0; ch < 2; ++ch)
      if (nd.child[ch] < 0) {
        s.max_count = std::max(s.max_count, rt::leaf_count(nd.child[ch]));
        s.max_end = std::max(s.max_end, rt::leaf_first(nd.child[ch]) + rt::leaf_count(nd.child[ch]));
      }
  return s;
}

static void plan_vote(DeviceScene* ds, const FlatScene& fs) {
  VotePlan& p = ds->vote;
  const TraceSwitches& sw = ds->sw;
  const size_t lds = stack_bytes((uint32_t)fs.max_stack + 1u), lds_ring = lds + (TRACE_BLOCK / 64) * ring_bytes(64);
  const bool ring_fits = lds_ring <= 64 * 1024;
  auto fit = [&](int preset, int nb0, int nb1, bool ring_by_default) {
    p.ring[preset] = ring_by_default && nb1 > 0 && nb1 >= nb0 && ring_fits;
    if (sw.ring >= 0 && nb1 > 0 && ring_fits) p.ring[preset] = sw.ring != 0;
    const int nb = p.ring[preset] ? nb1 : nb0;
    if (nb > 0) p.blocks_per_cu[preset] = nb;
  };
  fit(0, occupancy(k_trace_vote<P_SPHERES, false, false, false>, lds), occupancy(k_trace_vote<P_SPHERES, false, true, false>, lds_ring), true);
  fit(1, occupancy(k_trace_vote<P_MESH, false, false, false>, lds), occupancy(k_trace_vote<P_MESH, false, true, false>, lds_ring), false);

  memset(&p.top, 0, sizeof(p.top));
  p.top.n = -1;
  int n_bvh = 0, n_other = 0;
  for (size_t k = 0; k < fs.top_level.size(); ++k) {
    const int32_t kind = fs.entries[fs.top_level[k]].kind;
    if (kind == rt::ENTRY_BVH) { ++n_bvh; p.bvh_pos = (int32_t)k; }
    else if (kind != rt::ENTRY_PRIM) ++n_other;
  }
  p.ok = n_bvh == 1 && n_other == 0;
  if (p.ok && fs.top_level.size() <= 9 && sw.vote_top) {
    p.top.n = 0;
    p.top.all_rects = 1;
    for (size_t k = 0; k < fs.top_level.size(); ++k) {
      if ((int32_t)k == p.bvh_pos) continue;
      const rt::PrimRef ref = (rt::PrimRef)fs.entries[fs.top_level[k]].a;
      p.top.k[p.top.n] = (int32_t)k;
      p.top.ref[p.top.n] = (uint32_t)ref;
      if (rt::primref_type(ref) == rt::PRIM_RECT) p.top.rect[p.top.n] = fs.rects[rt::primref_index(ref)];
      else p.top.all_rects = 0;
      p.top.n += 1;
    }
    if (!p.top.all_rects) p.top.n = -1;
  }
  if (p.ok) {
    const rt::FlatEntry& be = fs.entries[fs.top_level[p.bvh_pos]];
    bool pure = be.c > 0 && rt::primref_type(fs.refs[be.b]) == rt::PRIM_TRIANGLE;
    const uint32_t t0 = pure ? rt::primref_index(fs.refs[be.b]) : 0u;
    for (int32_t k = 0; pure && k < be.c; ++k)
      pure = fs.refs[be.b + k] == rt::make_primref(rt::PRIM_TRIANGLE, t0 + (uint32_t)k);
    if (pure && sw.tri_direct) p.tri_base = (int32_t)t0;
  }
  if (!fs.materials.empty() && !fs.textures.empty() && fs.materials.size() <= 16 && fs.textures.size() <= 16 && sw.mat_lds) {
    p.tables = (uint32_t)fs.materials.size() | ((uint32_t)fs.textures.size() << 16);
    p.tables_bytes = fs.materials.size() * sizeof(rt::FlatMaterial) + fs.textures.size() * sizeof(rt::FlatTexture);
  }
}

static rtx_status launch_vote_wide(DeviceScene* ds, const PassArgs& a, bool diag) {
  const VotePlan& p = ds->vote;
  const WidePlan& wt = ds->wide;
  uint32_t lds_tables = 0;
  size_t lds = stack_bytes((uint32_t)wt.levels);
  if (p.tables_bytes > 0 && (lds + p.tables_bytes) * (size_t)wt.vote_blocks_per_cu <= 160 * 1024) {
    lds_tables = p.tables;
    lds += p.tables_bytes;
  }
  const uint32_t grid = grid_size(a.total, TRACE_BLOCK, (uint64_t)ds->n_cu * (uint64_t)wt.vote_blocks_per_cu);
  const uint32_t threshold = ds->walk.walk_threshold | (ds->walk.regen_min << 16);
#define LAUNCH_VOTE_WIDE(FEAT, DIAGF, THRESHOLD, MAP)                                                                  \
  hipLaunchKernelGGL(HIP_KERNEL_NAME(k_trace_vote<FEAT, DIAGF, false, true, decltype(MAP)>), dim3(grid), dim3(TRACE_BLOCK), lds, \
                     a.stream, ds->view, a.rp, MAP, a.s_begin, a.total, a.npix, a.samples, a.work_counter,             \
                     DIAGF ? ds->ws.diag : nullptr, ds->walk.leaf_weight, THRESHOLD, (uint32_t)wt.levels,              \
                     (uint32_t)p.bvh_pos, wt.nodes4, p.tri_base, lds_tables, p.top)
  const bool room = (a.feat & ~P_MESH_ROOM) == 0;
  if (diag && room) {
    unsigned long long h[24];
    static const char* const names[6] = {"outer", "regen", "node_step", "leaf_step", "shade_hit", "shade_all"};
    const rtx_status st = run_diag(ds, a.stream, [&] { LAUNCH_VOTE_WIDE(P_MESH_ROOM, true, ds->walk.walk_threshold, a.sm); }, "vote_diag", 10, names, 6, h);
    if (st != RTX_OK) return st;
    if (h[12]) {
      float v[12];
      for (int k = 0; k < 6; ++k) { uint32_t lo = (uint32_t)h[13 + k], hi = (uint32_t)(h[13 + k] >> 32); memcpy(&v[2 * k], &lo, 4); memcpy(&v[2 * k + 1], &hi, 4); }
      fprintf(stderr, "[vote_diag] %llu walks of >= 50000 node steps; the first: origin (%g %g %g) direction (%g %g %g) 1/d (%g %g %g) err2 %g t_min %g t_max %g depth left %llu\n",
              h[12], v[0], v[1], v[2], v[3], v[4], v[5], v[6], v[7], v[8], v[9], v[10], v[11], h[19]);
    }
  } else if (room) {
    with_map(a, [&](auto map) { LAUNCH_VOTE_WIDE(P_MESH_ROOM, false, threshold, map); });
  } else {
    with_map(a, [&](auto map) { LAUNCH_VOTE_WIDE(P_MESH, false, threshold, map); });
  }
#undef LAUNCH_VOTE_WIDE
  return RTX_OK;
}

static rtx_status launch_vote(DeviceScene* ds, const PassArgs& a) {
  const VotePlan& p = ds->vote;
  HIP_TRY(hipMemsetAsync(a.work_counter, 0, sizeof(unsigned int), a.stream));
  const bool diag = ds->sw.kernel == ForcedKernel::vote && ds->sw.diag && !a.active;
  if (a.preset == 1 && ds->wide.nodes4) return launch_vote_wide(ds, a, diag);
  const bool ring = p.ring[a.preset];
  const size_t lds = a.stack_lds + (ring ? (TRACE_BLOCK / 64) * ring_bytes(64) : 0);
  const uint32_t grid = grid_size(a.total, TRACE_BLOCK, (uint64_t)ds->n_cu * (uint64_t)p.blocks_per_cu[a.preset]);
#define LAUNCH_VOTE3(FEAT, DIAGF, RINGF, MAP)                                                                            \
  hipLaunchKernelGGL(HIP_KERNEL_NAME(k_trace_vote<FEAT, DIAGF, RINGF, false, decltype(MAP)>), dim3(grid), dim3(TRACE_BLOCK), lds, \
                     a.stream, ds->view, a.rp, MAP, a.s_begin, a.total, a.npix, a.samples, a.work_counter,              \
                     DIAGF ? ds->ws.diag : nullptr, ds->walk.leaf_weight, ds->walk.walk_threshold, a.stack_levels,      \
                     (uint32_t)p.bvh_pos, (const FlatNode4*)nullptr, p.tri_base, 0u, p.top)
#define LAUNCH_VOTE2(FEAT, RINGF) with_map(a, [&](auto map) { LAUNCH_VOTE3(FEAT, false, RINGF, map); })
#define LAUNCH_VOTE(FEAT) do { if (ring) { LAUNCH_VOTE2(FEAT, true); } else { LAUNCH_VOTE2(FEAT, false); } } while (0)
  if (diag && a.preset == 0) {
    unsigned long long h[24];
    static const char* const names[6] = {"outer", "regen", "node_step", "leaf_step", "shade_hit", "walking"};
    return run_diag(ds, a.stream, [&] {
      if (ring) { LAUNCH_VOTE3(P_SPHERES, true, true, a.sm); } else { LAUNCH_VOTE3(P_SPHERES, true, false, a.sm); }
    }, "vote_diag", 10, names, 6, h);
  }
  if (a.preset == 0) { LAUNCH_VOTE(P_SPHERES); }
  else { LAUNCH_VOTE(P_MESH); }
#undef LAUNCH_VOTE
#undef LAUNCH_VOTE2
#undef LAUNCH_VOTE3
  return RTX_OK;
}

static void validate_wide_tree(const FlatScene& fs, const std::vector<FlatNode4>& wide, int levels) {
  for (const rt::FlatEntry& e : fs.entries) {
    if (e.kind != rt::ENTRY_BVH) continue;
    std::vector<std::pair<int32_t, int>> todo;
    todo.push_back({e.a, 0});
    size_t visited = 0, bad = 0; int deepest = 0;
    while (!todo.empty()) {
      auto [code, below] = todo.back(); todo.pop_back();
      if (code < 0) { if (rt::leaf_first(code) + rt::leaf_count(code) > (uint32_t)e.c) ++bad; continue; }
      if ((size_t)code >= wide.size()) { ++bad; continue; }
      ++visited;
      int nk = 0;
      for (int k = 0; k < 4; ++k) if (wide[code].child[k] != 0x7fffffff) ++nk;
      deepest = std::max(deepest, below + nk);
      for (int k = 0; k < 4; ++k) if (wide[code].child[k] != 0x7fffffff) todo.push_back({wide[code].child[k], below + nk - 1});
    }
    fprintf(stderr, "[rtx] RTX_VALIDATE: BVH root %d refs %d: %zu wide nodes walked, %zu bad codes, deepest stack %d of %d levels, sizeof(real) %zu\n",
            e.a, e.c, visited, bad, deepest, levels, sizeof(rt::real));
  }
}

static rtx_status plan_wide(DeviceScene* ds, const FlatScene& fs) {
  WidePlan& p = ds->wide;
  const bool spheres_preset = (fs.features & ~P_SPHERES) == 0;
  const bool mesh_preset = !spheres_preset && (fs.features & ~P_MESH) == 0;
  const int preset = spheres_preset ? 0 : (mesh_preset ? 1 : 2);
  const bool for_vote = ds->vote.ok && mesh_preset;
  const bool for_world = !(ds->vote.ok && preset < 2) && preset >= 1;
  bool want_wide = (for_vote && fs.nodes.size() >= 4096) || (for_world && fs.nodes.size() >= 256);
  if (ds->sw.wide >= 0) want_wide = (for_vote || for_world) && ds->sw.wide != 0 && !fs.nodes.empty();
  if (!want_wide) return RTX_OK;
  std::vector<FlatNode4> wide(fs.nodes.size());
  memset(wide.data(), 0, wide.size() * sizeof(FlatNode4));
  int peak = 0;
  for (const rt::FlatEntry& e : fs.entries)
    if (e.kind == rt::ENTRY_BVH) peak = std::max(peak, build_wide_nodes(fs.nodes, e.a, &wide));
  p.levels = peak + 1;
  const size_t lds = stack_bytes((uint32_t)p.levels);
  bool ok = lds <= 64 * 1024;
  if (ok && for_vote) {
    const int nb = occupancy(k_trace_vote<P_MESH, false, false, true>, lds);
    ok = nb > 0;
    if (ok) p.vote_blocks_per_cu = nb;
  }
  if (ok) {
    rtx_status st = upload_array(ds, wide, &p.nodes4);
    if (st != RTX_OK) return st;
  }
  if (ds->sw.wide >= 0) fprintf(stderr, "[rtx] RTX_WIDE: 4-wide tree %s (%d stack levels)\n", p.nodes4 ? "on" : "off", p.levels);
  if (ds->sw.validate) validate_wide_tree(fs, wide, p.levels);
  return RTX_OK;
}

static rtx_status plan_world(DeviceScene* ds, const FlatScene& fs) {
  WorldPlan& p = ds->world;
  const TraceSwitches& sw = ds->sw;
  rtx_status st = upload_array(ds, build_world_desc(fs), &p.desc);
  if (st != RTX_OK) return st;
  for (int wd = 0; wd < 2; ++wd) {
    const uint32_t levels = (uint32_t)(wd ? ds->wide.levels : fs.max_stack + 1);
    size_t wl = stack_bytes(levels) + (size_t)WORLD_SLOT_F64 * TRACE_BLOCK * sizeof(rt::real);
    if (wl > 64 * 1024) continue;
    if ((wd != 0) == (ds->wide.nodes4 != nullptr)) {
      const size_t n_p = fs.perlins.size();
      if (n_p >= 1 && n_p <= 2 && sw.perlin_lds && wl + n_p * sizeof(rt::FlatPerlin) <= 52 * 1024) {
        p.perlin_lds = (uint32_t)n_p;
        wl += n_p * sizeof(rt::FlatPerlin);
      }
      const size_t mt = fs.materials.size() * sizeof(rt::FlatMaterial) + fs.textures.size() * sizeof(rt::FlatTexture);
      if (!fs.materials.empty() && !fs.textures.empty() && fs.materials.size() <= 64 && fs.textures.size() <= 64 && sw.mat_lds &&
          wl + mt <= 52 * 1024) {
        p.mat_lds = (uint32_t)fs.materials.size();
        p.tex_lds = (uint32_t)fs.textures.size();
        wl += mt;
      }
    }
    int n = 0;
#define WORLD_OCC(I, FEAT) if ((n = occupancy(wd ? k_trace_world<FEAT, true, WORLD_WPS> : k_trace_world<FEAT, false, WORLD_WPS>, wl)) > 0) p.blocks_per_cu[I][wd] = n
    WORLD_OCC(0, P_BOOK2); WORLD_OCC(1, P_ANY); WORLD_OCC(2, P_ALL); WORLD_OCC(3, P_NO_SPHERE_MEDIA);
#undef WORLD_OCC
  }
  return RTX_OK;
}

static rtx_status launch_world(DeviceScene* ds, const PassArgs& a) {
  const WorldPlan& p = ds->world;
  HIP_TRY(hipMemsetAsync(a.work_counter, 0, sizeof(unsigned int), a.stream));
  const bool wide = ds->wide.nodes4 != nullptr;
  const bool book2 = (a.feat & ~P_BOOK2) == 0;
  const bool has_gravity = (a.feat & rt::F_GRAVITY_SPHERE) != 0;
  const bool no_sphere_media = (a.feat & rt::F_MEDIUM_SPHERE) == 0;
  const uint32_t levels = wide ? (uint32_t)ds->wide.levels : a.stack_levels;
  const size_t lds = stack_bytes(levels) + (size_t)WORLD_SLOT_F64 * TRACE_BLOCK * sizeof(rt::real) +
                     (size_t)p.perlin_lds * sizeof(rt::FlatPerlin) + (size_t)p.mat_lds * sizeof(rt::FlatMaterial) +
                     (size_t)p.tex_lds * sizeof(rt::FlatTexture);
  const int family = has_gravity ? 2 : (book2 ? 0 : (no_sphere_media ? 3 : 1));
  const uint32_t grid = grid_size(a.total, TRACE_BLOCK, (uint64_t)ds->n_cu * (uint64_t)p.blocks_per_cu[family][wide ? 1 : 0]);
  const rt::SceneView& v = ds->view;
#define LAUNCH_WORLD3(FEAT, WIDEF, DIAGF, MAP)                                                                               \
  hipLaunchKernelGGL(HIP_KERNEL_NAME(k_trace_world<FEAT, WIDEF, WORLD_WPS, DIAGF, decltype(MAP)>), dim3(grid), dim3(TRACE_BLOCK), lds, \
                     a.stream, v, a.rp, MAP, a.s_begin, a.total, a.npix, a.samples, a.work_counter, v.entries, v.top_level, v.spheres, \
                     v.moving_spheres, v.rects, v.triangles, v.materials, v.textures, v.refs, ds->wide.nodes4, p.desc,     \
                     ds->walk.leaf_weight, ds->sw.world_threshold, levels, p.perlin_lds, p.mat_lds, p.tex_lds,             \
                     DIAGF ? ds->ws.diag : nullptr)
#define LAUNCH_WORLD2(FEAT, WIDEF) with_map(a, [&](auto map) { LAUNCH_WORLD3(FEAT, WIDEF, false, map); })
#define LAUNCH_WORLD(FEAT) do { if (wide) { LAUNCH_WORLD2(FEAT, true); } else { LAUNCH_WORLD2(FEAT, false); } } while (0)
  if (ds->sw.kernel == ForcedKernel::world && ds->sw.diag && book2 && wide && !a.active) {
    unsigned long long h[24];
    static const char* const names[8] = {"node_step", "leaf_step", "sweep", "shade(lean)", "regen", "direct_entry(all)", "direct_entry(run)", "shade(rare)"};
    return run_diag(ds, a.stream, [&] { LAUNCH_WORLD3(P_BOOK2, true, true, a.sm); }, "world_diag", 18, names, 8, h);
  }
  if (has_gravity) { LAUNCH_WORLD(P_ALL); }
  else if (book2) { LAUNCH_WORLD(P_BOOK2); }
  else if (no_sphere_media) { LAUNCH_WORLD(P_NO_SPHERE_MEDIA); }
  else { LAUNCH_WORLD(P_ANY); }
#undef LAUNCH_WORLD
#undef LAUNCH_WORLD2
#undef LAUNCH_WORLD3
  return RTX_OK;
}

static void fit_lds(LdsFit* f, bool want_ring, uint32_t lds_max) {
  for (uint32_t cap : {64u, 48u, 0u})
    if ((want_ring || cap == 0u) && ldsk_layout(f->levels, cap, f->dims).total <= lds_max) {
      f->ok = true;
      f->ring_cap = cap;
      return;
    }
}

static rtx_status plan_lds(DeviceScene* ds, const FlatScene& fs, const LeafScan& leaves) {
  const bool single_bvh = fs.top_level.size() == 1 && fs.entries[fs.top_level[0]].kind == rt::ENTRY_BVH;
  if (!single_bvh || (fs.features & ~P_SPHERES) != 0 || fs.nodes32.size() > LDSK_MAX_NODES) return RTX_OK;
  LdsPlan& p = ds->lds;
  const TraceSwitches& sw = ds->sw;
  const uint32_t max_end = leaves.max_end, levels = (uint32_t)fs.max_stack + 1u;
  int lds_max = 0;
  (void)hipDeviceGetAttribute(&lds_max, hipDeviceAttributeMaxSharedMemoryPerBlock, ds->device);
  if (lds_max > 160 * 1024) lds_max = 160 * 1024;
  p.plain.levels = levels;
  p.plain.dims = {(uint32_t)fs.nodes32.size(), max_end, max_end, 0u, LDSK_NODE_DWORDS, 0u};
  if (!fs.moving_spheres.empty()) {
    bool same = sw.mv_common;
    for (const rt::FlatMovingSphere& ms : fs.moving_spheres)
      same = same && ms.time0 == fs.moving_spheres[0].time0 && ms.time1 == fs.moving_spheres[0].time1;
    if (same) { p.mv_common = true; p.mv_t0 = (double)fs.moving_spheres[0].time0; p.mv_t1 = (double)fs.moving_spheres[0].time1; }
  }
  if (fs.features & rt::F_MOVING_SPHERE) {
    p.plain.dims.n_uni = (uint32_t)fs.spheres.size();
    p.plain.dims.n_moving = max_end;
    p.plain.dims.n_spheres = 0u;
  }
  p.motion.levels = levels;
  p.motion.dims = p.plain.dims;
  p.motion.dims.node_dwords = LDSK_MOTION_NODE_DWORDS;
  {
    bool moves[3] = {false, false, false};
    for (const rt::FlatMotion32& m : fs.motion32)
      for (int ch = 0; ch < 2; ++ch)
        for (int a = 0; a < 3; ++a) moves[a] = moves[a] || m.dlo[ch][a] != 0.0f || m.dhi[ch][a] != 0.0f;
    if (!fs.motion32.empty() && moves[1] && !moves[0] && !moves[2] && sw.motion_axis) {
      p.motion_axis = 1;
      p.motion.dims.node_dwords = LDSK_MOTION1_NODE_DWORDS;
    }
  }
  if (leaves.max_count <= 4 && max_end <= LDSK_MAX_SLOTS && sw.scene_lds != 0 && lds_max > 0) {
    const bool want_ring = sw.ring != 0;
    fit_lds(&p.plain, want_ring, (uint32_t)lds_max);
    const rt::FlatEntry& be = fs.entries[fs.top_level[0]];
    if (p.plain.ok && !fs.motion32.empty() && (fs.features & rt::F_MOVING_SPHERE) && (double)be.f[0] < (double)be.f[1] && sw.motion) {
      p.motion_t0 = (double)be.f[0]; p.motion_t1 = (double)be.f[1];
      fit_lds(&p.motion, want_ring, (uint32_t)lds_max);
    }
  }
  if (p.plain.ok) {
    hipError_t ae = hipSuccess;
#define LDS_ATTR1(K) if (ae == hipSuccess) ae = hipFuncSetAttribute((const void*)K, hipFuncAttributeMaxDynamicSharedMemorySize, lds_max)
#define LDS_ATTR(FEAT, RINGF, MOTIONF) LDS_ATTR1((k_trace_lds<FEAT, RINGF, MOTIONF>)); LDS_ATTR1((k_trace_lds<FEAT, RINGF, MOTIONF, ActiveMap>))
    LDS_ATTR(P_SPHERES, true, 0u); LDS_ATTR(P_SPHERES, false, 0u); LDS_ATTR(P_STATIC_SPHERES, true, 0u); LDS_ATTR(P_STATIC_SPHERES, false, 0u);
    LDS_ATTR(P_SPHERES, true, 1u); LDS_ATTR(P_SPHERES, false, 1u); LDS_ATTR(P_SPHERES, true, 3u); LDS_ATTR(P_SPHERES, false, 3u);
#undef LDS_ATTR
#undef LDS_ATTR1
    if (ae != hipSuccess) { (void)hipGetLastError(); p.plain.ok = false; }
  }
  if (sw.scene_lds >= 0) {
    auto bytes = [](const LdsFit& f) { return f.ok ? ldsk_layout(f.levels, f.ring_cap, f.dims).total : 0u; };
    fprintf(stderr, "[rtx] RTX_SCENE_LDS: k_trace_lds %s (ring of %u, %u B of LDS); time-aware boxes %s (ring of %u, %u B)\n",
            p.plain.ok ? "on" : "off", p.plain.ring_cap, ldsk_layout(levels, p.plain.ring_cap, p.plain.dims).total,
            p.motion.ok ? "on" : "off", p.motion.ring_cap, bytes(p.motion));
  }
  return RTX_OK;
}

static rtx_status launch_lds(DeviceScene* ds, const PassArgs& a, const RtxCamera* cam) {
  const LdsPlan& p = ds->lds;
  HIP_TRY(hipMemsetAsync(a.work_counter, 0, sizeof(unsigned int), a.stream));
  const bool motion = p.motion.ok && (double)cam->time1 >= p.motion_t0 && (double)cam->time2 <= p.motion_t1;
  const LdsFit& f = motion ? p.motion : p.plain;
  const bool ring = f.ring_cap != 0u;
  const rt::real m_t0 = (rt::real)p.motion_t0, m_inv = (rt::real)(1.0 / (p.motion_t1 - p.motion_t0));
  const LdsKernelLayout L = ldsk_layout(f.levels, f.ring_cap, f.dims);
  const uint32_t grid = grid_size(a.total, LDSK_BLOCK, (uint64_t)ds->n_cu);
  const WalkTuning& wk = ds->walk;
#define LAUNCH_LDS2(FEAT, RINGF, MOTIONF)                                                                               \
  with_map(a, [&](auto map) {                                                                                           \
    hipLaunchKernelGGL(HIP_KERNEL_NAME(k_trace_lds<FEAT, RINGF, MOTIONF, decltype(map)>), dim3(grid), dim3(LDSK_BLOCK), L.total, \
                       a.stream, ds->view, a.rp, map, a.s_begin, a.total, a.npix, a.samples, a.work_counter, wk.leaf_weight, \
                       wk.walk_threshold | (wk.single_leaf ? 0x100u : 0u), ds->sw.chunk, f.ring_cap, f.levels, f.dims,  \
                       m_t0, m_inv, p.mv_common ? 1u : 0u, (rt::real)p.mv_t0, (rt::real)p.mv_t1);                        \
  })
#define LAUNCH_LDS(FEAT, MOTIONF) do { if (ring) { LAUNCH_LDS2(FEAT, true, MOTIONF); } else { LAUNCH_LDS2(FEAT, false, MOTIONF); } } while (0)
  if ((a.feat & ~P_STATIC_SPHERES) == 0) { LAUNCH_LDS(P_STATIC_SPHERES, 0u); }
  else if (motion && p.motion_axis == 1) { LAUNCH_LDS(P_SPHERES, 3u); }
  else if (motion) { LAUNCH_LDS(P_SPHERES, 1u); }
  else { LAUNCH_LDS(P_SPHERES, 0u); }
#undef LAUNCH_LDS
#undef LAUNCH_LDS2
  return RTX_OK;
}

template <bool COUNT>
static void launch_simple(const DeviceScene* ds, const PassArgs& a) {
  const uint32_t grid = grid_size(a.total, TRACE_BLOCK, (uint64_t)ds->n_cu * 8);
#define LAUNCH_SIMPLE2(FEAT, MAP)                                                                                       \
  hipLaunchKernelGGL(HIP_KERNEL_NAME(k_trace_simple<FEAT, COUNT, decltype(MAP)>), dim3(grid), dim3(TRACE_BLOCK), a.stack_lds, \
                     a.stream, ds->view, a.rp, MAP, a.s_begin, a.total, a.npix, a.samples, ds->ws.counters)
#define LAUNCH_SIMPLE(FEAT) with_map(a, [&](auto map) { LAUNCH_SIMPLE2(FEAT, map); })
  if constexpr (COUNT) { LAUNCH_SIMPLE2(P_ALL, a.sm); }
  else {
    if (a.preset == 0) { LAUNCH_SIMPLE(P_SPHERES); }
    else if (a.preset == 1) { LAUNCH_SIMPLE(P_MESH); }
    else { LAUNCH_SIMPLE(P_ALL); }
  }
#undef LAUNCH_SIMPLE
#undef LAUNCH_SIMPLE2
}

static rtx_status wave_pass(DeviceScene* ds, const PassArgs& a) {
  Workspace& ws = ds->ws;
  const hipStream_t stream = a.stream;
  uint32_t P = ds->sw.wf_paths;
  if ((uint64_t)P > (uint64_t)a.total) P = a.total;
  P = (P + WF_SEG - 1u) & ~(WF_SEG - 1u);
  const uint32_t n_seg = P / WF_SEG;
  const size_t R = sizeof(rt::real);
  const size_t bytes = 64 + (size_t)P * (16 + 7 * R + 3 * R + 3 * R + R + 4 + 4 + 4 + 4) + (size_t)n_seg * 8;
  rtx_status st = grow_buffer(&ws.wave_mem, &ws.wave_bytes, bytes, stream);
  if (st != RTX_OK) return st;
  if (!ws.wave_host_ctrl) HIP_TRY(hipHostMalloc((void**)&ws.wave_host_ctrl, 4 * sizeof(uint32_t), hipHostMallocDefault));
  WavePool pool;
  {
    unsigned char* m = (unsigned char*)ws.wave_mem;
    pool.ctrl = (uint32_t*)m; m += 64;
    pool.rng = (unsigned long long*)m; m += (size_t)P * 16;
    pool.ray = (rt::real*)m; m += (size_t)P * 7 * R;
    pool.product = (rt::real*)m; m += (size_t)P * 3 * R;
    pool.output = (rt::real*)m; m += (size_t)P * 3 * R;
    pool.hit_t = (rt::real*)m; m += (size_t)P * R;
    pool.depth = (int32_t*)m; m += (size_t)P * 4;
    pool.g = (uint32_t*)m; m += (size_t)P * 4;
    pool.hit_ref = (uint32_t*)m; m += (size_t)P * 4;
    pool.free_list = (uint32_t*)m; m += (size_t)P * 4;
    pool.n_free = (uint32_t*)m; m += (size_t)n_seg * 4;
    pool.cursor = (uint32_t*)m; m += (size_t)n_seg * 4;
    pool.P = P;
  }
  const int preset = a.preset;
  const bool wide = preset == 1 && ds->wide.nodes4 != nullptr;
  const uint32_t levels = wide ? (uint32_t)ds->wide.levels : a.stack_levels;
  const size_t lds = stack_bytes(levels);
  if (lds > 64 * 1024) { set_error("render: BVH too deep for the LDS traversal stack"); return RTX_EUNSUPPORTED; }
  const bool room = (a.feat & ~P_MESH_ROOM) == 0;
  const int occ = ds->sw.wf_occ;
  const uint32_t leaf_weight = ds->walk.leaf_weight, refill = ds->sw.wf_refill, bvh_pos = (uint32_t)ds->vote.bvh_pos;
#define WF_CASES(X)                                                                                                          \
  if (preset == 0) { X(P_SPHERES, false, 4); }                                                                               \
  else if (!wide) { X(P_MESH, false, 4); }                                                                                   \
  else if (room && occ == 5) { X(P_MESH_ROOM, true, 5); }                                                                    \
  else if (room && occ == 6) { X(P_MESH_ROOM, true, 6); }                                                                    \
  else if (room) { X(P_MESH_ROOM, true, 4); }                                                                                \
  else { X(P_MESH, true, 4); }
  int nb = 0;
  hipError_t oe = hipSuccess;
#define WF_OCC(FEAT, WIDEF, MB) oe = hipOccupancyMaxActiveBlocksPerMultiprocessor(&nb, k_wf_trace<FEAT, WIDEF, MB>, TRACE_BLOCK, lds)
  WF_CASES(WF_OCC)
#undef WF_OCC
  if (oe != hipSuccess || nb <= 0) { (void)hipGetLastError(); nb = 1; }
  const uint32_t tgrid = grid_size(P, TRACE_BLOCK, (uint64_t)ds->n_cu * (uint64_t)nb);
  hipLaunchKernelGGL(k_wf_init, dim3((P + 255u) / 256u), dim3(256), 0, stream, pool);
  uint32_t check_every = ds->sw.wf_check;
  int it = 0;
  for (;; ++it) {
    with_map(a, [&](auto map) {
      hipLaunchKernelGGL(HIP_KERNEL_NAME(k_wf_generate<decltype(map)>), dim3(n_seg), dim3(WF_SEG), 0, stream, pool, a.rp, map,
                         a.s_begin, a.total, a.npix);
    });
    if ((uint32_t)(it + 1) % check_every == 0u) {
      HIP_TRY(hipMemsetAsync(pool.ctrl, 0, 16, stream));
      hipLaunchKernelGGL(k_wf_count, dim3(256), dim3(256), 0, stream, pool);
      HIP_TRY(hipGetLastError());
      HIP_TRY(hipMemcpyAsync(ws.wave_host_ctrl, pool.ctrl, 4 * sizeof(uint32_t), hipMemcpyDeviceToHost, stream));
      HIP_TRY(hipStreamSynchronize(stream));
      if (ws.wave_host_ctrl[0] == 0u) break;
      if (ws.wave_host_ctrl[0] < P / 2u) check_every = 2;
      if (it > 100000000) { set_error("render: wavefront integrator did not converge"); return RTX_EHIP; }
    }
#define WF_LAUNCH(FEAT, WIDEF, MB)                                                                                           \
  do {                                                                                                                       \
    hipLaunchKernelGGL(HIP_KERNEL_NAME(k_wf_trace<FEAT, WIDEF, MB>), dim3(tgrid), dim3(TRACE_BLOCK), lds, stream, ds->view, pool, \
                       leaf_weight, refill, bvh_pos, ds->wide.nodes4, ds->vote.tri_base);                                    \
    hipLaunchKernelGGL(HIP_KERNEL_NAME(k_wf_shade<FEAT>), dim3(n_seg), dim3(WF_SEG), 0, stream, ds->view, pool, a.rp, a.samples, bvh_pos); \
  } while (0)
    WF_CASES(WF_LAUNCH)
#undef WF_LAUNCH
  }
#undef WF_CASES
  if (ds->sw.wf_verbose) fprintf(stderr, "[rtx] wavefront: %u slots, %d iterations, %d blocks per CU (%u stack levels)\n", P, it + 1, nb, levels);
  return RTX_OK;
}

static void plan_walk(DeviceScene* ds, const LeafScan& leaves) {
  WalkTuning& w = ds->walk;
  const TraceSwitches& sw = ds->sw;
  w.leaf_weight = leaves.max_count <= 1 ? 1u : 3u;
  w.single_leaf = leaves.max_count <= 1;
  if (ds->wide.nodes4) { w.leaf_weight = 1u; w.walk_threshold = 24u; w.regen_min = 8u; }
  else if (ds->lds.plain.ok) w.walk_threshold = 12u;
  if (sw.regen_min) w.regen_min = sw.regen_min;
  if (sw.leaf_weight) w.leaf_weight = sw.leaf_weight;
  if (!sw.single_leaf) w.single_leaf = false;
  if (sw.walk_threshold) w.walk_threshold = sw.walk_threshold;
}

static int32_t choose_trace_kernel(const DeviceScene* ds, int preset, bool count) {
  const ForcedKernel k = ds->sw.kernel;
  if (count || k == ForcedKernel::simple) return RTX_KERNEL_SIMPLE;
  if (ds->lds.plain.ok && preset == 0 && k == ForcedKernel::none) return RTX_KERNEL_LDS;
  if (ds->vote.ok && preset < 2 && k == ForcedKernel::wavefront) return RTX_KERNEL_WAVEFRONT;
  if (ds->vote.ok && preset < 2 && k != ForcedKernel::world) return RTX_KERNEL_VOTE;
  return RTX_KERNEL_WORLD;
}

struct SampleRange {
  uint32_t first, count;
  int cont;
  double* sumsq;
  const uint32_t* active;
  uint32_t n_active;
};

struct PassPlan {
  uint32_t spp_pass;
  bool pipeline;
  size_t sample_bytes;
};

static rtx_status prepare_workspace(DeviceScene* ds, const RtxConfig* cfg, uint64_t npix, uint64_t npix_all, uint32_t spp, bool serial,
                                    hipStream_t stream, double** accum, PassPlan* pp) {
  Workspace& ws = ds->ws;
  uint64_t budget = cfg->sample_buffer_bytes;
  if (budget == 0) {
    budget = 24ull << 30;
    size_t free_b = 0, total_b = 0;
    if (hipMemGetInfo(&free_b, &total_b) == hipSuccess) {
      const uint64_t avail = ((uint64_t)free_b + ws.samples_bytes) / 3;
      if (avail < budget) budget = avail;
    } else {
      (void)hipGetLastError();
    }
    if (budget < ws.samples_bytes) budget = ws.samples_bytes;
  }
  const uint64_t per_sample_plane = npix * 24ull;
  uint32_t spp_pass = spp;
  const bool pipeline = ds->sw.pass_pipeline && !serial && ds->sw.kernel != ForcedKernel::simple && per_sample_plane > 0 &&
                        (uint64_t)spp * per_sample_plane > budget && budget / 2 >= per_sample_plane;
  const uint64_t pass_budget = pipeline ? budget / 2 : budget;
  if (per_sample_plane > 0 && (uint64_t)spp_pass * per_sample_plane > pass_budget) {
    spp_pass = (uint32_t)(pass_budget / per_sample_plane);
    if (spp_pass < 1) spp_pass = 1;
  }
  while (spp_pass > 1 && (uint64_t)spp_pass * npix >= 0xFFFF0000ull) --spp_pass;
  if ((uint64_t)spp_pass * npix >= 0xFFFF0000ull) { set_error("render: shard too large for one pass"); return RTX_EINVAL; }
  size_t need_samples = (size_t)spp_pass * per_sample_plane * (pipeline ? 2 : 1);
  if (need_samples > ws.samples_bytes) {
    if (ws.samples) { HIP_TRY(hipStreamSynchronize(stream)); HIP_TRY(hipFree(ws.samples)); ws.samples = nullptr; ws.samples_bytes = 0; }
    for (;;) {
      hipError_t me = hipMalloc((void**)&ws.samples, need_samples);
      if (me == hipSuccess) break;
      (void)hipGetLastError();
      ws.samples = nullptr;
      if (me != hipErrorOutOfMemory || spp_pass <= 1) {
        set_error(std::string("render: sample buffer of ") + std::to_string(need_samples) + " bytes: " + hipGetErrorString(me));
        return me == hipErrorOutOfMemory ? RTX_ENOMEM : RTX_EHIP;
      }
      spp_pass = (spp_pass + 1) / 2;
      need_samples = (size_t)spp_pass * per_sample_plane * (pipeline ? 2 : 1);
    }
    ws.samples_bytes = need_samples;
  }
  if (!*accum) {
    const rtx_status st = grow_buffer((void**)&ws.accum, &ws.accum_bytes, (size_t)npix_all * 24, stream);
    if (st != RTX_OK) return st;
    *accum = ws.accum;
  }
  if (!ws.counters) HIP_TRY(hipMalloc((void**)&ws.counters, sizeof(rt::TraceCounters)));
  if (!ws.work_counter) HIP_TRY(hipMalloc((void**)&ws.work_counter, 2 * sizeof(unsigned int)));
  if (pipeline && !ws.aux_stream) {
    HIP_TRY(hipStreamCreateWithFlags(&ws.aux_stream, hipStreamNonBlocking));
    for (int i = 0; i < 3; ++i) HIP_TRY(hipEventCreateWithFlags(&ws.ev_pass[i], hipEventDisableTiming));
  }
  if (!ws.ev[0]) { HIP_TRY(hipEventCreate(&ws.ev[0])); HIP_TRY(hipEventCreate(&ws.ev[1])); }
  *pp = {spp_pass, pipeline, need_samples};
  return RTX_OK;
}

template <bool COUNT>
static rtx_status render_impl(DeviceScene* ds, const RtxCamera* cam, const RtxConfig* cfg,
                              const RtxShard* shard, double* d_accum_out, uint8_t* d_rgb8_out,
                              hipStream_t stream, RtxRenderStats* stats, const SampleRange* range = nullptr) {
  RtxShard sh;
  rtx_status st = validate(ds, cam, cfg, shard, &sh);
  if (st != RTX_OK) return st;
  int cur = -1;
  HIP_TRY(hipGetDevice(&cur));
  if (cur != ds->device) { set_error("render: scene was uploaded to a different device than the current one"); return RTX_EINVAL; }
  if ((ds->view.features & rt::F_GRAVITY_SPHERE) && !(cam->time2 <= ds->gravity_time_limit)) {
    set_error("render: shutter time " + std::to_string(cam->time2) + " is beyond the GravitySpheres' stored trajectory (limit " +
              std::to_string(ds->gravity_time_limit) + " s): get_center's fallback loop (hit.rs:380-390) would run unbounded on the GPU");
    return RTX_EINVAL;
  }

  const rt::RenderParams rp = make_params(cam, cfg);
  const int32_t w = rp.image_width, h = rp.image_height;
  int32_t row_limit = h;
  if (cfg->row_chunk_compat) row_limit = (h / cfg->threads) * cfg->threads;
  const int rows_all = shard_row_count(h, sh, h);
  const int rows_active = shard_row_count(h, sh, row_limit);
  const uint64_t npix_all = (uint64_t)rows_all * w, npix = (uint64_t)rows_active * w;
  if (npix_all >= (1ull << 31)) { set_error("render: shard larger than 2^31 pixels"); return RTX_EINVAL; }
  if (stats) memset(stats, 0, sizeof(*stats));
  if (npix_all == 0) return RTX_OK;

  const uint32_t s_first = range ? range->first : 0u;
  const uint32_t spp = range ? range->count : (uint32_t)cfg->samples_per_pixel;
  const bool adaptive = range && range->active;
  if (adaptive && (!range->cont || !range->sumsq || d_rgb8_out || range->n_active > npix)) {
    set_error("render: an adaptive sample range continues S and Q of at most the shard's pixels");
    return RTX_EINVAL;
  }
  const uint64_t nitem = adaptive ? range->n_active : npix;
  double* accum = d_accum_out;
  PassPlan pp;
  st = prepare_workspace(ds, cfg, nitem, npix_all, spp, COUNT || stats != nullptr, stream, &accum, &pp);
  if (st != RTX_OK) return st;
  Workspace& ws = ds->ws;
  if (COUNT) HIP_TRY(hipMemsetAsync(ws.counters, 0, sizeof(rt::TraceCounters), stream));

  if (npix < npix_all) {
    HIP_TRY(hipMemsetAsync(accum + 3 * npix, 0, (size_t)(npix_all - npix) * 24, stream));
    if (d_rgb8_out) HIP_TRY(hipMemsetAsync(d_rgb8_out + 3 * npix, 0, (size_t)(npix_all - npix) * 3, stream));
    if (range && range->sumsq) HIP_TRY(hipMemsetAsync(range->sumsq + 3 * npix, 0, (size_t)(npix_all - npix) * 24, stream));
  }

  const uint32_t stack_levels = (uint32_t)ds->view.max_stack + 1u;
  if (stack_bytes(stack_levels) > 64 * 1024) { set_error("render: BVH too deep for the LDS traversal stack"); return RTX_EUNSUPPORTED; }
  const uint32_t feat = ds->view.features;
  const int preset = ((feat & ~P_SPHERES) == 0) ? 0 : (((feat & ~P_MESH) == 0) ? 1 : 2);
  const int32_t kernel = choose_trace_kernel(ds, preset, COUNT);
  PassArgs a = {rp, {w, sh.block_rows, sh.shard_index, sh.shard_count}, 0u, 0u, (uint32_t)nitem, nullptr, nullptr, stream,
                preset, feat, stack_levels, stack_bytes(stack_levels), adaptive ? range->active : nullptr};

  float trace_ms = 0.f;
  int passes = 0;
  if (nitem > 0) {
    if (pp.pipeline) {
      HIP_TRY(hipEventRecord(ws.ev_pass[2], stream));
      HIP_TRY(hipStreamWaitEvent(ws.aux_stream, ws.ev_pass[2], 0));
    }
    for (uint32_t s_off = 0; s_off < spp; s_off += pp.spp_pass, ++passes) {
      const int half = pp.pipeline ? (passes & 1) : 0;
      const uint32_t s_count = spp - s_off < pp.spp_pass ? spp - s_off : pp.spp_pass;
      a.s_begin = s_first + s_off;
      a.total = (uint32_t)((uint64_t)s_count * nitem);
      a.stream = half ? ws.aux_stream : stream;
      a.samples = ws.samples + (size_t)half * (size_t)pp.spp_pass * (size_t)nitem * 3u;
      a.work_counter = ws.work_counter + half;
      if (stats) HIP_TRY(hipEventRecord(ws.ev[0], a.stream));
      switch (kernel) {
        case RTX_KERNEL_SIMPLE: launch_simple<COUNT>(ds, a); break;
        case RTX_KERNEL_LDS: st = launch_lds(ds, a, cam); break;
        case RTX_KERNEL_WAVEFRONT: st = wave_pass(ds, a); break;
        case RTX_KERNEL_VOTE: st = launch_vote(ds, a); break;
        default: st = launch_world(ds, a); break;
      }
      if (st != RTX_OK) return st;
      HIP_TRY(hipGetLastError());
      if (stats) {
        HIP_TRY(hipEventRecord(ws.ev[1], a.stream));
        HIP_TRY(hipEventSynchronize(ws.ev[1]));
        float ms = 0.f;
        HIP_TRY(hipEventElapsedTime(&ms, ws.ev[0], ws.ev[1]));
        trace_ms += ms;
      }
      uint32_t pgrid = (uint32_t)((nitem + 255) / 256);
      if (pp.pipeline && passes > 0) HIP_TRY(hipStreamWaitEvent(a.stream, ws.ev_pass[1 - half], 0));
      const int first_pass = s_off == 0 && !(range && range->cont) ? 1 : 0;
      if (adaptive)
        hipLaunchKernelGGL(k_reduce_samples_moments_active, dim3(pgrid), dim3(256), 0, a.stream, a.samples, accum, range->sumsq,
                           range->active, (uint32_t)nitem, s_count);
      else if (range && range->sumsq)
        hipLaunchKernelGGL(k_reduce_samples_moments, dim3(pgrid), dim3(256), 0, a.stream, a.samples, accum, range->sumsq,
                           (uint32_t)npix, s_count, first_pass);
      else
        hipLaunchKernelGGL(k_reduce_samples, dim3(pgrid), dim3(256), 0, a.stream, a.samples, accum, (uint32_t)npix, s_count, first_pass);
      HIP_TRY(hipGetLastError());
      if (pp.pipeline) HIP_TRY(hipEventRecord(ws.ev_pass[half], a.stream));
    }
    if (pp.pipeline && passes > 0 && ((passes - 1) & 1)) HIP_TRY(hipStreamWaitEvent(stream, ws.ev_pass[1], 0));
    if (d_rgb8_out) {
      uint32_t pgrid = (uint32_t)((npix + 255) / 256);
      hipLaunchKernelGGL(k_tonemap, dim3(pgrid), dim3(256), 0, stream, accum, d_rgb8_out, (uint32_t)npix, s_first + spp);
      HIP_TRY(hipGetLastError());
    }
  }
  if (stats) {
    HIP_TRY(hipStreamSynchronize(stream));
    stats->trace_ms = trace_ms;
    stats->trace_launches = passes;
    stats->passes = passes;
    stats->trace_kernel = passes > 0 ? kernel : RTX_KERNEL_SIMPLE;
    stats->sample_buffer_bytes = pp.sample_bytes;
    stats->samples = (uint64_t)spp * nitem;
    if (COUNT) {
      rt::TraceCounters c;
      HIP_TRY(hipMemcpy(&c, ws.counters, sizeof(c), hipMemcpyDeviceToHost));
      stats->samples = c.samples; stats->rays = c.rays; stats->box_tests = c.box_tests;
      stats->sphere_tests = c.sphere_tests; stats->moving_sphere_tests = c.moving_sphere_tests;
      stats->rect_tests = c.rect_tests; stats->triangle_tests = c.triangle_tests;
      stats->scatters = c.scatters; stats->texels = c.texels; stats->perlin_calls = c.perlin_calls;
    }
  }
  return RTX_OK;
}

static rtx_status tonemap_impl(const double* accum, uint8_t* rgb8, uint32_t npix, uint32_t spp, hipStream_t stream) {
  if (npix == 0) return RTX_OK;
  hipLaunchKernelGGL(k_tonemap, dim3((npix + 255) / 256), dim3(256), 0, stream, accum, rgb8, npix, spp);
  HIP_TRY(hipGetLastError());
  return RTX_OK;
}

static rtx_status tonemap_counts_impl(const double* accum, uint8_t* rgb8, const int32_t* counts, uint32_t npix, uint32_t spp,
                                      hipStream_t stream) {
  if (npix == 0) return RTX_OK;
  hipLaunchKernelGGL(k_tonemap_counts, dim3((npix + 255) / 256), dim3(256), 0, stream, accum, rgb8, counts, npix, spp);
  HIP_TRY(hipGetLastError());
  return RTX_OK;
}

static rtx_status features_impl(DeviceScene* ds, const RtxCamera* cam, const RtxConfig* cfg, int32_t feature_spp,
                                float4* d_albedo, float4* d_normal, hipStream_t stream) {
  int cur = -1;
  HIP_TRY(hipGetDevice(&cur));
  if (cur != ds->device) { set_error("features: scene was uploaded to a different device than the current one"); return RTX_EINVAL; }
  if ((ds->view.features & rt::F_GRAVITY_SPHERE) && !(cam->time2 <= ds->gravity_time_limit)) {
    set_error("features: shutter time beyond the GravitySpheres' stored trajectory");
    return RTX_EINVAL;
  }
  const rt::RenderParams rp = make_params(cam, cfg);
  const uint64_t npix = (uint64_t)rp.image_width * (uint64_t)rp.image_height;
  if (npix == 0) return RTX_OK;
  const uint32_t stack_levels = (uint32_t)ds->view.max_stack + 1u;
  if (stack_bytes(stack_levels) > 64 * 1024) { set_error("features: BVH too deep for the LDS traversal stack"); return RTX_EUNSUPPORTED; }
  const uint32_t grid = grid_size((uint32_t)npix, TRACE_BLOCK, (uint64_t)ds->n_cu * 8);
  hipLaunchKernelGGL(HIP_KERNEL_NAME(k_features<P_ALL>), dim3(grid), dim3(TRACE_BLOCK), stack_bytes(stack_levels), stream, ds->view,
                     rp, (uint32_t)npix, (uint32_t)feature_spp, d_albedo, d_normal);
  HIP_TRY(hipGetLastError());
  return RTX_OK;
}

static rtx_status scene_upload_impl(const FlatScene& fs, DeviceScene** out) {
  *out = nullptr;
  DeviceScene* ds = new (std::nothrow) DeviceScene();
  if (!ds) { set_error("out of memory"); return RTX_ENOMEM; }
  hipError_t e = hipGetDevice(&ds->device);
  if (e != hipSuccess) {
    set_error(std::string("hipGetDevice: ") + hipGetErrorString(e) + " (this library has no CPU render path)");
    delete ds;
    return RTX_EHIP;
  }
  rt::SceneView& v = ds->view;
  memset(&v, 0, sizeof(v));
  rtx_status st;
#define UP(field, vec) if ((st = upload_array(ds, fs.vec, &v.field)) != RTX_OK) { free_device_scene(ds); return st; }
  UP(spheres, spheres) UP(moving_spheres, moving_spheres) UP(rects, rects) UP(triangles, triangles)
  UP(nodes, nodes) UP(nodes32, nodes32) UP(motion32, motion32) UP(refs, refs) UP(entries, entries) UP(top_level, top_level)
  UP(materials, materials) UP(textures, textures) UP(perlins, perlins) UP(images, images) UP(texels, texels)
  UP(top_box32, top_box32) UP(gravity_spheres, gravity_spheres) UP(gravity_y, gravity_y)
#undef UP
  v.n_top_level = (int32_t)fs.top_level.size();
  v.max_stack = fs.max_stack;
  v.features = fs.features;
  for (const rt::FlatGravitySphere& g : fs.gravity_spheres)
    ds->gravity_time_limit = std::min(ds->gravity_time_limit, (double)g.table_len * 0.001 + 10.0);
  hipDeviceProp_t prop;
  if (hipGetDeviceProperties(&prop, ds->device) == hipSuccess && prop.multiProcessorCount > 0) ds->n_cu = prop.multiProcessorCount;

  ds->sw = read_switches();
  const LeafScan leaves = scan_leaves(fs);
  plan_vote(ds, fs);
  if ((st = plan_wide(ds, fs)) != RTX_OK || (st = plan_world(ds, fs)) != RTX_OK || (st = plan_lds(ds, fs, leaves)) != RTX_OK) {
    free_device_scene(ds);
    return st;
  }
  plan_walk(ds, leaves);
  *out = ds;
  return RTX_OK;
}

static rtx_status scene_trim_impl(DeviceScene* ds) {
  int cur = -1;
  HIP_TRY(hipGetDevice(&cur));
  if (cur != ds->device) { set_error("rtx_scene_trim: scene lives on a different device than the current one"); return RTX_EINVAL; }
  HIP_TRY(hipDeviceSynchronize());
  Workspace& ws = ds->ws;
  if (ws.samples) { HIP_TRY(hipFree(ws.samples)); ws.samples = nullptr; ws.samples_bytes = 0; }
  if (ws.accum) { HIP_TRY(hipFree(ws.accum)); ws.accum = nullptr; ws.accum_bytes = 0; }
  return RTX_OK;
}

}

using namespace rtx;

#ifdef RTX_F32_TU
#include "f32_entry.inc"
#else
#include "f32_convert.inc"

template <bool COUNT>
static rtx_status render_any(const rtx_scene* s, const RtxCamera* cam, const RtxConfig* cfg, const RtxShard* shard,
                             double* d_accum_rgb, uint8_t* d_rgb8, hipStream_t stream, RtxRenderStats* stats) {
  if (!s) { set_error("render: NULL scene, camera or config"); return RTX_EINVAL; }
  if (s->f32) {
    if (COUNT) { set_error("rtx_render_count: the work counters belong to the f64 path (upload the scene with rtx_scene_upload)"); return RTX_EUNSUPPORTED; }
    return rtx_f32_render(s->device_scene, cam, cfg, shard, d_accum_rgb, d_rgb8, (void*)stream, stats);
  }
  return render_impl<COUNT>(scene_device(s), cam, cfg, shard, d_accum_rgb, d_rgb8, stream, stats);
}

extern "C" {

rtx_status rtx_scene_upload(const rtx_flat* f, rtx_scene** out) {
  if (!f || !out) { set_error("rtx_scene_upload: NULL argument"); return RTX_EINVAL; }
  *out = nullptr;
  DeviceScene* ds = nullptr;
  rtx_status st = scene_upload_impl(*flat_of(f), &ds);
  if (st != RTX_OK) return st;
  *out = make_scene_handle(ds, 0);
  return RTX_OK;
}

rtx_status rtx_scene_upload_f32(const rtx_flat* f, rtx_scene** out) {
  if (!f || !out) { set_error("rtx_scene_upload_f32: NULL argument"); return RTX_EINVAL; }
  *out = nullptr;
  void* ds32 = nullptr;
  rtx_status st = upload_as_f32(*flat_of(f), &ds32);
  if (st != RTX_OK) return st;
  *out = make_scene_handle((DeviceScene*)ds32, 1);
  return RTX_OK;
}

int32_t rtx_scene_is_f32(const rtx_scene* s) { return s && s->f32 ? 1 : 0; }

rtx_status rtx_scene_trim(rtx_scene* s) {
  if (!s) { set_error("rtx_scene_trim: NULL scene"); return RTX_EINVAL; }
  if (s->f32) return rtx_f32_trim(s->device_scene);
  return scene_trim_impl(scene_device(s));
}

void rtx_scene_destroy(rtx_scene* s) {
  if (!s) return;
  if (s->f32) rtx_f32_destroy(s->device_scene);
  else free_device_scene(scene_device(s));
  free_scene_handle(s);
}

rtx_status rtx_render_device(const rtx_scene* s, const RtxCamera* cam, const RtxConfig* cfg,
                             const RtxShard* shard, double* d_accum_rgb, uint8_t* d_rgb8,
                             void* hip_stream, RtxRenderStats* stats) {
  return render_any<false>(s, cam, cfg, shard, d_accum_rgb, d_rgb8, (hipStream_t)hip_stream, stats);
}

rtx_status rtx_render_count(const rtx_scene* s, const RtxCamera* cam, const RtxConfig* cfg,
                            const RtxShard* shard, RtxRenderStats* stats) {
  if (!stats) { set_error("rtx_render_count: stats is NULL"); return RTX_EINVAL; }
  return render_any<true>(s, cam, cfg, shard, nullptr, nullptr, (hipStream_t) nullptr, stats);
}

rtx_status rtx_device_math(int32_t fn, const double* x, const double* y, int64_t n, double* out) {
  if (!x || !y || !out || n < 0) { set_error("rtx_device_math: bad argument"); return RTX_EINVAL; }
  if (n == 0) return RTX_OK;
  double *dx = nullptr, *dy = nullptr, *dout = nullptr;
  size_t bytes = (size_t)n * sizeof(double);
  rtx_status st = RTX_OK;
  auto fail = [&](const char* what, hipError_t e) { set_error(std::string(what) + ": " + hipGetErrorString(e)); st = RTX_EHIP; };
  hipError_t e;
  if ((e = hipMalloc((void**)&dx, bytes)) != hipSuccess) fail("hipMalloc", e);
  if (st == RTX_OK && (e = hipMalloc((void**)&dy, bytes)) != hipSuccess) fail("hipMalloc", e);
  if (st == RTX_OK && (e = hipMalloc((void**)&dout, bytes)) != hipSuccess) fail("hipMalloc", e);
  if (st == RTX_OK && (e = hipMemcpy(dx, x, bytes, hipMemcpyHostToDevice)) != hipSuccess) fail("hipMemcpy", e);
  if (st == RTX_OK && (e = hipMemcpy(dy, y, bytes, hipMemcpyHostToDevice)) != hipSuccess) fail("hipMemcpy", e);
  if (st == RTX_OK) {
    hipLaunchKernelGGL(k_device_math, dim3((unsigned)((n + 255) / 256)), dim3(256), 0, 0, (int)fn, dx, dy, (long long)n, dout);
    if ((e = hipGetLastError()) != hipSuccess) fail("k_device_math", e);
  }
  if (st == RTX_OK && (e = hipMemcpy(out, dout, bytes, hipMemcpyDeviceToHost)) != hipSuccess) fail("hipMemcpy", e);
  if (dx) (void)hipFree(dx);
  if (dy) (void)hipFree(dy);
  if (dout) (void)hipFree(dout);
  return st;
}

rtx_status rtx_device_stream(uint64_t seed, uint64_t pixel, uint32_t sample, int32_t n, double* out) {
  if (!out || n < 0) { set_error("rtx_device_stream: bad argument"); return RTX_EINVAL; }
  if (n == 0) return RTX_OK;
  double* d = nullptr;
  HIP_TRY(hipMalloc((void**)&d, (size_t)n * sizeof(double)));
  hipLaunchKernelGGL(k_device_stream, dim3(1), dim3(64), 0, 0, (unsigned long long)seed, (unsigned long long)pixel, (unsigned int)sample, (int)n, d);
  hipError_t e = hipMemcpy(out, d, (size_t)n * sizeof(double), hipMemcpyDeviceToHost);
  (void)hipFree(d);
  if (e != hipSuccess) { set_error(std::string("rtx_device_stream: ") + hipGetErrorString(e)); return RTX_EHIP; }
  return RTX_OK;
}

rtx_status rtx_render(const rtx_scene* s, const RtxCamera* cam, const RtxConfig* cfg, RtxFrame* out) {
  if (!out) { set_error("rtx_render: NULL frame"); return RTX_EINVAL; }
  RtxShard sh;
  rtx_status st = validate(s, cam, cfg, nullptr, &sh);
  if (st != RTX_OK) return st;
  size_t npix = (size_t)cfg->image_width * (size_t)rtx_image_height(cfg);
  double* d_accum = nullptr;
  uint8_t* d_rgb = nullptr;
  if (hipMalloc((void**)&d_accum, npix * 24) != hipSuccess || hipMalloc((void**)&d_rgb, npix * 3) != hipSuccess) {
    if (d_accum) (void)hipFree(d_accum);
    set_error("rtx_render: hipMalloc of the frame failed");
    return RTX_EHIP;
  }
  st = render_any<false>(s, cam, cfg, nullptr, d_accum, d_rgb, (hipStream_t) nullptr, nullptr);
  if (st == RTX_OK) {
    hipError_t e = hipDeviceSynchronize();
    if (e == hipSuccess && out->accum_rgb) e = hipMemcpy(out->accum_rgb, d_accum, npix * 24, hipMemcpyDeviceToHost);
    if (e == hipSuccess && out->rgb8) e = hipMemcpy(out->rgb8, d_rgb, npix * 3, hipMemcpyDeviceToHost);
    if (e != hipSuccess) { set_error(std::string("rtx_render: ") + hipGetErrorString(e)); st = RTX_EHIP; }
  }
  (void)hipFree(d_accum);
  (void)hipFree(d_rgb);
  return st;
}

}

extern "C" rtx_status rtx_render_scene_with_time(const rtx_scene* s, double t0, double t1, const char* path,
                                                 int32_t row_chunk_compat, const RtxConfig* overrides) {
  using namespace rtx;
  if (!s || !path) { set_error("rtx_render_scene_with_time: NULL argument"); return RTX_EINVAL; }
  const double lookfrom[3] = {13, 2, 3}, lookat[3] = {0, 0, 0}, vup[3] = {0, 1, 0};
  RtxCamera cam;
  rtx_status st = rtx_camera_new(lookfrom, lookat, vup, 20.0, 1.0, 0.1, 10.0, t0, t1, &cam);
  if (st != RTX_OK) return st;
  RtxConfig cfg;
  st = rtx_config_new(1.0, 500, 500, 50, 11, &cfg);
  if (st != RTX_OK) return st;
  cfg.background[0] = 0.7; cfg.background[1] = 0.8; cfg.background[2] = 1.0;
  cfg.row_chunk_compat = row_chunk_compat ? 1 : 0;
  if (overrides) {
    if (overrides->image_width > 0) cfg.image_width = overrides->image_width;
    if (overrides->samples_per_pixel > 0) cfg.samples_per_pixel = overrides->samples_per_pixel;
    if (overrides->max_depth > 0) cfg.max_depth = overrides->max_depth;
    cfg.seed = overrides->seed;
    cfg.sample_buffer_bytes = overrides->sample_buffer_bytes;
  }
  const size_t npix = (size_t)cfg.image_width * (size_t)rtx_image_height(&cfg);
  std::vector<uint8_t> rgb(npix * 3);
  RtxFrame frame = {nullptr, rgb.data()};
  st = rtx_render(s, &cam, &cfg, &frame);
  if (st != RTX_OK) return st;
  return rtx_write_ppm(path, cfg.image_width, rtx_image_height(&cfg), rgb.data());
}

#include "multi.inc"
#include "progressive.inc"
#endif
```

### ray-tracing-series-rust_amd/csrc/hip/trace_lds.inc

```

#define LDSK_BLOCK 1024
#define LDSK_DONE (-1)
#define LDSK_NO_REF 0xFFFFFFFFu
#define LDSK_MAX_SLOTS 8190u
#define LDSK_MAX_NODES 8191u
#define LDSK_NODE_DWORDS 21u
#ifndef LDSK_NODE_BURST
#define LDSK_NODE_BURST 1
#endif
#define LDSK_MOTION_NODE_DWORDS 39u
#define LDSK_MOTION1_NODE_DWORDS 27u

struct LdsKernelLayout {
  uint32_t off_ring, off_nodes, off_refs, off_spheres, off_moving, total;
};
__host__ __device__ inline LdsKernelLayout ldsk_layout(uint32_t levels, uint32_t ring_cap, const LdsSceneDims& d) {
  LdsKernelLayout L;
  uint32_t o = levels * LDSK_BLOCK * 2u;
  o = (o + 15u) & ~15u;
  L.off_ring = o; o += (LDSK_BLOCK / 64u) * ring_bytes(ring_cap);
  L.off_nodes = o; o += (d.n_nodes * d.node_dwords * 4u + 15u) & ~15u;
  L.off_refs = o;
  L.off_spheres = o; o += (d.n_spheres * (uint32_t)sizeof(rt::FlatSphere) + 15u) & ~15u;
  L.off_moving = o; o += (d.n_moving * (uint32_t)sizeof(rt::FlatMovingSphere) + 15u) & ~15u;
  L.total = o;
  return L;
}

struct LdsStack16 {
  unsigned short* base;
  int n;
  __device__ __forceinline__ void init() { base[0] = 0xFFFFu; n = 1; }
  __device__ __forceinline__ void reset() { n = 1; }
  __device__ __forceinline__ void push(int32_t v) { base[n * LDSK_BLOCK] = (unsigned short)v; ++n; }
  __device__ __forceinline__ int32_t pop() { --n; return (int32_t)(short)base[n * LDSK_BLOCK]; }
  __device__ __forceinline__ int32_t top() const { return (int32_t)(short)base[(n - 1) * LDSK_BLOCK]; }
};
__host__ __device__ __forceinline__ int32_t ldsk_item(int32_t child) {
  if (child >= 0) return child;
  return (int32_t)(short)(unsigned short)(0x8000u | (rt::leaf_first(child) << 2) | (rt::leaf_count(child) - 1u));
}

template <uint32_t F, bool RING, uint32_t MOTION, class SM = ShardMap>
__global__ __launch_bounds__(LDSK_BLOCK) void k_trace_lds(rt::SceneView sv, rt::RenderParams rp, SM sm,
                                                          uint32_t s_begin, uint32_t total, uint32_t npix,
                                                          double* __restrict__ samples, unsigned int* work_counter,
                                                          uint32_t leaf_weight, uint32_t walk_threshold, uint32_t chunk, uint32_t ring_cap,
                                                          uint32_t stack_levels, LdsSceneDims dims, rt::real motion_t0, rt::real motion_inv_dt,
                                                          uint32_t mv_common, rt::real mv_t0, rt::real mv_t1) {
  static_assert(!MOTION || (F & rt::F_MOVING_SPHERE), "time-aware boxes only make sense with moving spheres");
  const bool single_leaf = (walk_threshold & 0x100u) != 0u;
  walk_threshold &= 0xFFu;
  constexpr bool UNI = (F & rt::F_MOVING_SPHERE) != 0;
  constexpr uint32_t FL = UNI ? (F & ~rt::F_SPHERE) : F;
  static_assert(MOTION <= 4u, "0: no slopes, 1: all axes, 2 + a: axis a only");
  constexpr uint32_t ND = MOTION == 1u ? LDSK_MOTION_NODE_DWORDS : (MOTION >= 2u ? LDSK_MOTION1_NODE_DWORDS : LDSK_NODE_DWORDS);
  constexpr uint32_t CBD = MOTION == 1u ? 19u : (MOTION >= 2u ? 13u : 10u);
  constexpr uint32_t MA = MOTION >= 2u ? MOTION - 2u : 0u;
  constexpr uint32_t CB = CBD * 4u;
  constexpr uint32_t ITEM_OFF = CB - 4u;
  static_assert((F & ~(rt::F_SPHERE | rt::F_MOVING_SPHERE | rt::F_BVH | rt::F_LAMBERTIAN | rt::F_METAL |
                       rt::F_DIELECTRIC | rt::F_CHECKER)) == 0, "k_trace_lds caches spheres and moving spheres only");
  extern __shared__ __attribute__((aligned(16))) unsigned char ldsk[];
  const LdsKernelLayout L = ldsk_layout(stack_levels, RING ? ring_cap : 0u, dims);
  const uint32_t lane = threadIdx.x & 63u;
  const rt::FlatEntry& bvh = sv.entries[sv.top_level[0]];
  const int32_t root = bvh.a | (sv.nodes32[bvh.a].axis << 13);
  const uint32_t first_ref = (uint32_t)bvh.b;

  uint32_t* const lds_nodes = (uint32_t*)(ldsk + L.off_nodes);
  rt::FlatSphere* const lds_spheres = (rt::FlatSphere*)(ldsk + L.off_spheres);
  rt::FlatMovingSphere* const lds_moving = (rt::FlatMovingSphere*)(ldsk + L.off_moving);
  {
    static_assert(sizeof(rt::FlatNode32) == 64 && offsetof(rt::FlatNode32, child) == 48 && offsetof(rt::FlatNode32, axis) == 56,
                  "the padded LDS copy assumes FlatNode32's layout");
    const uint32_t* src = (const uint32_t*)sv.nodes32;
    const uint32_t* msrc = (const uint32_t*)sv.motion32;
    for (uint32_t k = threadIdx.x; k < dims.n_nodes * 2u * CBD; k += LDSK_BLOCK) {
      const uint32_t node = k / (2u * CBD), field = k - node * (2u * CBD);
      const uint32_t c = field / CBD, r = field - c * CBD;
      uint32_t v;
      if (r < 9u) {
        const uint32_t a = r / 3u, t = r - a * 3u;
        v = MOTION ? msrc[node * 24u + (t == 1u ? 6u : 0u) + c * 3u + a]
                   : src[node * 16u + (t == 1u ? 6u : 0u) + c * 3u + a];
      } else if (MOTION == 1u && r < 18u) {
        const uint32_t a = (r - 9u) / 3u, t = (r - 9u) - a * 3u;
        v = msrc[node * 24u + (t == 1u ? 18u : 12u) + c * 3u + a];
      } else if (MOTION >= 2u && r < 12u) {
        const uint32_t t = r - 9u;
        v = msrc[node * 24u + (t == 1u ? 18u : 12u) + c * 3u + MA];
      } else {
        const int32_t child = (int32_t)src[node * 16u + 12u + c];
        int32_t item = ldsk_item(child);
        if (child >= 0) item |= sv.nodes32[child].axis << 13;
        v = (uint32_t)item;
      }
      lds_nodes[node * ND + field] = v;
    }
    if (UNI) {
      for (uint32_t k = threadIdx.x; k < dims.n_refs; k += LDSK_BLOCK) {
        const rt::PrimRef ref = sv.refs[first_ref + k];
        rt::FlatMovingSphere m;
        if (rt::primref_type(ref) == rt::PRIM_SPHERE) {
          const rt::FlatSphere sp = sv.spheres[rt::primref_index(ref)];
          m.c0[0] = sp.cx; m.c0[1] = sp.cy; m.c0[2] = sp.cz; m.c1[0] = sp.cx; m.c1[1] = sp.cy; m.c1[2] = sp.cz;
          m.time0 = rt::real(0.0); m.time1 = rt::real(1.0); m.radius = sp.radius; m.mat = sp.mat; m.pad = 0;
        } else {
          m = sv.moving_spheres[rt::primref_index(ref)];
        }
        lds_moving[k] = m;
      }
    } else {
      constexpr uint32_t SD = (uint32_t)(sizeof(rt::FlatSphere) / 4);
      uint32_t* ds = (uint32_t*)lds_spheres;
      const uint32_t* ss = (const uint32_t*)sv.spheres;
      for (uint32_t k = threadIdx.x; k < dims.n_refs * SD; k += LDSK_BLOCK) {
        const uint32_t slot = k / SD, field = k - slot * SD;
        ds[k] = ss[rt::primref_index(sv.refs[first_ref + slot]) * SD + field];
      }
    }
  }
  __syncthreads();
  rt::SceneView lsv = sv;
  lsv.spheres = lds_spheres;
  lsv.moving_spheres = lds_moving;

  LdsStack16 stack;
  stack.base = (unsigned short*)ldsk + threadIdx.x;
  stack.init();
  double* const ring_f = (double*)(ldsk + L.off_ring + (threadIdx.x >> 6) * ring_bytes(ring_cap));
  uint32_t* const ring_g = (uint32_t*)(ring_f + RING_F64 * ring_cap);
  uint32_t ring_n = 0;
  uint32_t chunk_pos = 0, chunk_end = 0;
  bool queue_empty = false;
  bool active = false;
  uint32_t g = 0;
  rt::PathState ps;
  bool midwalk = false;
  rt::Ray32 q = {0.f, 0.f, 0.f, 0.f, 0.f, 0.f, 0.f, 0.f};
  uint32_t dir_neg = 0;
  uint32_t off_x = 0, off_y = 12, off_z = 24;
  uint32_t flip_b = 0;
  float t_max32 = 0.f;
  float s32 = 0.f;
  rt::real mv_ratio = rt::real(0.0);
  int32_t cur = LDSK_DONE;
  rt::Closest best;
  best.t = 0.0; best.ref = LDSK_NO_REF; best.order = 0; best.hit = false;

  for (;;) {
    const unsigned long long need_mask = wave_ballot(!active);
    if (need_mask != 0ull) {
      const uint32_t n_need = (uint32_t)__popcll(need_mask);
      const uint32_t rank = __builtin_amdgcn_mbcnt_hi((uint32_t)(need_mask >> 32),
                                                      __builtin_amdgcn_mbcnt_lo((uint32_t)need_mask, 0u));
      if (RING) {
        for (int rep = 0; rep < 2 && ring_n < n_need && !queue_empty; ++rep) {
          if (chunk_pos >= chunk_end) {
            uint32_t base = 0;
            if (lane == 0) base = atomicAdd(work_counter, chunk);
            base = __builtin_amdgcn_readfirstlane(base);
            if (base >= total) { queue_empty = true; break; }
            chunk_pos = base;
            chunk_end = (total - base < chunk) ? total : base + chunk;
          }
          const uint32_t room = ring_cap - ring_n, avail = chunk_end - chunk_pos;
          const uint32_t m = room < avail ? room : avail;
          if (lane < m) {
            const uint32_t gg = chunk_pos + lane;
            rt::PathState fresh;
            start_path(rp, sm, npix, s_begin, gg, &fresh);
            const uint32_t slot = ring_n + lane;
            ring_f[0 * ring_cap + slot] = fresh.ray.origin.x; ring_f[1 * ring_cap + slot] = fresh.ray.origin.y;
            ring_f[2 * ring_cap + slot] = fresh.ray.origin.z; ring_f[3 * ring_cap + slot] = fresh.ray.direction.x;
            ring_f[4 * ring_cap + slot] = fresh.ray.direction.y; ring_f[5 * ring_cap + slot] = fresh.ray.direction.z;
            ring_f[6 * ring_cap + slot] = fresh.ray.time;
            ring_f[7 * ring_cap + slot] = rt::bits_f64(fresh.rng.s0); ring_f[8 * ring_cap + slot] = rt::bits_f64(fresh.rng.s1);
            ring_g[slot] = gg;
          }
          chunk_pos += m;
          ring_n += m;
          __builtin_amdgcn_fence(__ATOMIC_ACQ_REL, "wavefront");
        }
        const uint32_t take = n_need < ring_n ? n_need : ring_n;
        if (!active && rank < take) {
          const uint32_t slot = ring_n - 1u - rank;
          ps.ray = rt::make_ray(rt::v3(ring_f[0 * ring_cap + slot], ring_f[1 * ring_cap + slot], ring_f[2 * ring_cap + slot]),
                                rt::v3(ring_f[3 * ring_cap + slot], ring_f[4 * ring_cap + slot], ring_f[5 * ring_cap + slot]),
                                ring_f[6 * ring_cap + slot]);
          ps.rng.s0 = rt::f64_bits(ring_f[7 * ring_cap + slot]); ps.rng.s1 = rt::f64_bits(ring_f[8 * ring_cap + slot]);
          ps.product = rt::v3(1, 1, 1);
          ps.output = rt::v3(0, 0, 0);
          ps.depth = rp.max_depth;
          g = ring_g[slot];
          active = true;
        }
        ring_n -= take;
        __builtin_amdgcn_fence(__ATOMIC_ACQ_REL, "wavefront");
      } else {
        if (chunk_pos >= chunk_end && !queue_empty) {
          uint32_t base = 0;
          if (lane == 0) base = atomicAdd(work_counter, chunk);
          base = __builtin_amdgcn_readfirstlane(base);
          if (base >= total) {
            queue_empty = true;
          } else {
            chunk_pos = base;
            chunk_end = (total - base < chunk) ? total : base + chunk;
          }
        }
        if (chunk_pos < chunk_end) {
          const uint32_t avail = chunk_end - chunk_pos;
          if (!active && rank < avail) {
            g = chunk_pos + rank;
            start_path(rp, sm, npix, s_begin, g, &ps);
            active = true;
          }
          chunk_pos += (n_need < avail) ? n_need : avail;
        }
      }
    }
    if (wave_ballot(active) == 0ull) break;
    if (active && !midwalk) {
      if (rt::path_bounce_begin(&ps)) {
        store_sample(samples, g, ps.output);
        active = false;
      } else {
        q = rt::make_ray32(ps.ray, rt::ray_t_min(ps.ray));
        dir_neg = rt::ray_dir_neg(ps.ray);
        off_x = (dir_neg & 1u) << 2; off_y = 12u + ((dir_neg & 2u) << 1); off_z = 24u + (dir_neg & 4u);
        flip_b = ((dir_neg & 1u) * CB) | (((dir_neg >> 1) & 1u) * (CB << 8)) | (((dir_neg >> 2) & 1u) * (CB << 16));
        t_max32 = __builtin_huge_valf();
        if (UNI && mv_common != 0u) mv_ratio = (ps.ray.time - mv_t0) / (mv_t1 - mv_t0);
        if (MOTION) s32 = __builtin_fminf(__builtin_fmaxf((float)((ps.ray.time - motion_t0) * motion_inv_dt), 0.f), 1.f);
        best.t = RT_INFINITY; best.ref = LDSK_NO_REF; best.order = 0;
        stack.reset();
        cur = root;
        midwalk = true;
      }
    }
    const uint32_t threshold = (queue_empty && ring_n == 0u) ? 1u : walk_threshold;
    auto node_step = [&]() {
      const unsigned char* nd = (const unsigned char*)(lds_nodes + ((uint32_t)cur & 0x1FFFu) * ND);
      const uint32_t first_b = __builtin_amdgcn_ubfe(flip_b, ((uint32_t)cur >> 10) & 0x18u, 8u);
      const unsigned char* bf = nd + first_b;
      const unsigned char* bs = nd + (CB - first_b);
      const float *fx = (const float*)(bf + off_x), *fy = (const float*)(bf + off_y), *fz = (const float*)(bf + off_z);
      const float *sx = (const float*)(bs + off_x), *sy = (const float*)(bs + off_y), *sz = (const float*)(bs + off_z);
      const int32_t top = stack.top();
      bool hf, hs;
      if (MOTION >= 2u) {
        constexpr uint32_t SO = 9u - 3u * MA;
        const float* fm = MA == 0u ? fx : (MA == 1u ? fy : fz);
        const float* sm = MA == 0u ? sx : (MA == 1u ? sy : sz);
        const float fn = __builtin_fmaf(s32, fm[SO], fm[0]), ff = __builtin_fmaf(s32, fm[SO + 1u], fm[1]);
        const float sn = __builtin_fmaf(s32, sm[SO], sm[0]), sf = __builtin_fmaf(s32, sm[SO + 1u], sm[1]);
        hf = rt::cull32_may_hit_nf_pos(MA == 0u ? fn : fx[0], MA == 0u ? ff : fx[1], MA == 1u ? fn : fy[0], MA == 1u ? ff : fy[1],
                                       MA == 2u ? fn : fz[0], MA == 2u ? ff : fz[1], q, t_max32);
        hs = rt::cull32_may_hit_nf_pos(MA == 0u ? sn : sx[0], MA == 0u ? sf : sx[1], MA == 1u ? sn : sy[0], MA == 1u ? sf : sy[1],
                                       MA == 2u ? sn : sz[0], MA == 2u ? sf : sz[1], q, t_max32);
      } else if (MOTION) {
        hf = rt::cull32_may_hit_nf_pos(__builtin_fmaf(s32, fx[9], fx[0]), __builtin_fmaf(s32, fx[10], fx[1]), __builtin_fmaf(s32, fy[9], fy[0]),
                                   __builtin_fmaf(s32, fy[10], fy[1]), __builtin_fmaf(s32, fz[9], fz[0]), __builtin_fmaf(s32, fz[10], fz[1]), q, t_max32);
        hs = rt::cull32_may_hit_nf_pos(__builtin_fmaf(s32, sx[9], sx[0]), __builtin_fmaf(s32, sx[10], sx[1]), __builtin_fmaf(s32, sy[9], sy[0]),
                                   __builtin_fmaf(s32, sy[10], sy[1]), __builtin_fmaf(s32, sz[9], sz[0]), __builtin_fmaf(s32, sz[10], sz[1]), q, t_max32);
      } else {
        hf = rt::cull32_may_hit_nf_pos(fx[0], fx[1], fy[0], fy[1], fz[0], fz[1], q, t_max32);
        hs = rt::cull32_may_hit_nf_pos(sx[0], sx[1], sy[0], sy[1], sz[0], sz[1], q, t_max32);
      }
      const int32_t cf = *(const int32_t*)(bf + ITEM_OFF), cs = *(const int32_t*)(bs + ITEM_OFF);
      const bool both = hf && hs;
      if (both) stack.base[stack.n * LDSK_BLOCK] = (unsigned short)cs;
      cur = hf ? cf : (hs ? cs : top);
      stack.n += (int)both - (int)!(hf || hs);
    };
    auto leaf_test = [&](uint32_t slot) {
      const rt::PrimRef ref = rt::make_primref(UNI ? rt::PRIM_MOVING_SPHERE : rt::PRIM_SPHERE, slot);
      rt::real t;
      bool ok;
      if (UNI && mv_common != 0u) {
        const rt::FlatMovingSphere& sp = lds_moving[slot];
        const rt::Point3 c0 = rt::load_v3(sp.c0), c1 = rt::load_v3(sp.c1);
        ok = rt::sphere_root(c0 + mv_ratio * (c1 - c0), sp.radius, ps.ray, rt::ray_t_min(ps.ray), best.t, &t);
      } else {
        ok = rt::prim_t<FL, false>(lsv, ref, ps.ray, rt::ray_t_min(ps.ray), best.t, &t, nullptr);
      }
      if (ok && !(t == best.t && slot < best.order)) { best.t = t; best.ref = ref; best.order = slot; }
    };
    for (;;) {
      const bool is_node = cur >= 0;
      const bool is_leaf = cur < -1;
      const uint32_t n_node = (uint32_t)__popcll(wave_ballot(is_node)), n_leaf = (uint32_t)__popcll(wave_ballot(is_leaf));
      if (n_node + n_leaf < threshold) break;
      if (n_node * leaf_weight >= n_leaf) {
        if (is_node) node_step();
#if LDSK_NODE_BURST >= 2
        if (cur >= 0) node_step();
#endif
      } else {
        if (is_leaf) {
          const uint32_t f = ((uint32_t)cur & 0x7FFFu) >> 2;
          if (single_leaf) {
            leaf_test(f);
          } else {
            const uint32_t k = ((uint32_t)cur & 3u) + 1u;
            for (uint32_t i = 0; i < k; ++i) leaf_test(f + i);
          }
          t_max32 = rt::cull_round_up(best.t);
          cur = stack.pop();
        }
      }
    }
    if (midwalk && cur == LDSK_DONE) {
      midwalk = false;
      rt::HitRecord rec;
      const bool hit = best.ref != LDSK_NO_REF;
      if (hit) rt::prim_finalize<FL>(lsv, best.ref, ps.ray, best.t, &rec);
      if (rt::path_bounce_end<F, false>(sv, rp, &ps, hit, rec, nullptr)) {
        store_sample(samples, g, ps.output);
        active = false;
      }
    }
  }
}
```

Before: 7852.

## Add uniform sphere grid with DDA traversal for static-sphere LDS kernel

```diff
diff --git a/include/rtx_abi.h b/include/rtx_abi.h
--- a/include/rtx_abi.h
+++ b/include/rtx_abi.h
@@ -236,6 +236,8 @@
 rtx_status rtx_device_noise_reduce(const double* S, const double* Q, const int32_t* counts, uint32_t npix, uint32_t spp,
                                    double target, double* max_r, double* sum_r, uint64_t* above);
 
+rtx_status rtx_grid_selftest(const rtx_flat* f, double lambda, const double* rays, uint64_t n, uint64_t* out);
+
 const void* rtx_builder_graph(const rtx_builder* b);
 const void* rtx_flat_arrays(const rtx_flat* f);
 
diff --git a/ray-tracing-series-rust_amd/api.py b/ray-tracing-series-rust_amd/api.py
--- a/ray-tracing-series-rust_amd/api.py
+++ b/ray-tracing-series-rust_amd/api.py
@@ -173,6 +173,7 @@
     "rtx_progressive_denoise": (C.c_int32, [_VP, C.POINTER(RtxDenoiseParams), _D3, C.POINTER(C.c_uint8)]),
     "rtx_device_denoise": (C.c_int32, [_D3, _D3, _F3, _F3, C.c_int32, C.c_int32, C.POINTER(RtxDenoiseParams), _D3,
                                        C.POINTER(C.c_uint8)]),
+    "rtx_grid_selftest": (C.c_int32, [_VP, C.c_double, _D3, C.c_uint64, C.POINTER(C.c_uint64)]),
     "rtx_builder_graph": (_VP, [_VP]),
     "rtx_flat_arrays": (_VP, [_VP]),
 }
@@ -601,6 +602,15 @@
     if S.shape != Q.shape:
         raise ValueError("S and Q must have the same shape")
     return S, Q
+
+
+def grid_selftest(flat, rays, lam=0.0):
+    rays = np.ascontiguousarray(rays, dtype=np.float64).reshape(-1, 7)
+    out = (C.c_uint64 * 9)()
+    _check(lib.rtx_grid_selftest(flat.ptr, lam, rays.ctypes.data_as(_D3), rays.shape[0], out))
+    keys = ("rays", "not_offered", "closest_differs", "cells", "candidate_tests", "f64_tests", "grid_cells", "cell_entries",
+            "max_cell")
+    return dict(zip(keys, (int(v) for v in out)))
 
 
 def device_retire(S, Q, active, spp, target, counts):
diff --git a/ray-tracing-series-rust_amd/build.py b/ray-tracing-series-rust_amd/build.py
--- a/ray-tracing-series-rust_amd/build.py
+++ b/ray-tracing-series-rust_amd/build.py
@@ -17,6 +17,7 @@
     "csrc/host/scene_graph.cpp",
     "csrc/host/flatten.cpp",
     "csrc/host/bvh_build.cpp",
+    "csrc/host/grid_build.cpp",
     "csrc/host/scenes.cpp",
 ]
 HIP_FLAGS = [
diff --git a/ray-tracing-series-rust_amd/csrc/core/grid_dda.hpp b/ray-tracing-series-rust_amd/csrc/core/grid_dda.hpp
--- /dev/null
+++ b/ray-tracing-series-rust_amd/csrc/core/grid_dda.hpp
@@ -0,0 +1,129 @@
+#pragma once
+#include "cull32.hpp"
+
+namespace rt {
+
+#define GRID_MAX_AXIS 255u
+#define GRID_MAX_ALWAYS 4u
+#define GRID_SLOPE_CAP 0x1.0p60f
+#define GRID_FIRST (1u << 26)
+
+struct GridDesc {
+  double lo[3];
+  float cs[3], inv_cs[3];
+  uint32_t n[3];
+  uint32_t n_always;
+  uint32_t always[GRID_MAX_ALWAYS];
+  float abox[GRID_MAX_ALWAYS][6];
+};
+
+struct GridRay {
+  Ray32 q;
+  double t0;
+  int32_t e;
+  uint32_t cell;
+  float s_next;
+};
+
+RT_HD double grid_ldexp(double x, int32_t e) {
+#if defined(__HIP_DEVICE_COMPILE__)
+  return __builtin_amdgcn_ldexp(x, e);
+#else
+  return __builtin_ldexp(x, e);
+#endif
+}
+
+RT_HD float grid_slope(float d) {
+#if defined(__HIP_DEVICE_COMPILE__)
+  return __builtin_amdgcn_fmed3f(__builtin_amdgcn_rcpf(d), -GRID_SLOPE_CAP, GRID_SLOPE_CAP);
+#else
+  return __builtin_fminf(__builtin_fmaxf(1.0f / d, -GRID_SLOPE_CAP), GRID_SLOPE_CAP);
+#endif
+}
+
+RT_HD float grid_s_max(const GridRay& w, real best_t) { return cull_round_up(grid_ldexp((double)best_t - w.t0, w.e)); }
+
+RT_HD bool grid_always_may_hit(const GridDesc& g, uint32_t i, const Ray32& q) {
+  const float* b = g.abox[i];
+  const bool nx = q.ix < 0.f, ny = q.iy < 0.f, nz = q.iz < 0.f;
+  return cull32_may_hit_nf_pos(nx ? b[3] : b[0], nx ? b[0] : b[3], ny ? b[4] : b[1], ny ? b[1] : b[4], nz ? b[5] : b[2], nz ? b[2] : b[5],
+                               q, __builtin_huge_valf());
+}
+
+RT_HD bool grid_ray_begin(const GridDesc& g, const Ray& r, real t_min, real t_max, GridRay* w) {
+  const double dx = (double)r.direction.x, dy = (double)r.direction.y, dz = (double)r.direction.z;
+  const double m = __builtin_fmax(__builtin_fabs(dx), __builtin_fmax(__builtin_fabs(dy), __builtin_fabs(dz)));
+  if (!(m > 0.0 && m <= 1.79e308 && dx == dx && dy == dy && dz == dz)) return false;
+#if defined(__HIP_DEVICE_COMPILE__)
+  const int32_t e = __builtin_amdgcn_frexp_exp(m) - 1;
+#else
+  int32_t fe = 0;
+  (void)__builtin_frexp(m, &fe);
+  const int32_t e = fe - 1;
+#endif
+  Ray32 q;
+  q.ix = grid_slope((float)grid_ldexp(dx, -e));
+  q.iy = grid_slope((float)grid_ldexp(dy, -e));
+  q.iz = grid_slope((float)grid_ldexp(dz, -e));
+  float ox = (float)((double)r.origin.x - g.lo[0]), oy = (float)((double)r.origin.y - g.lo[1]), oz = (float)((double)r.origin.z - g.lo[2]);
+  auto finish = [&]() {
+    q.oix = ox * q.ix; q.oiy = oy * q.iy; q.oiz = oz * q.iz;
+    const float ax = __builtin_fabsf(q.ix) < GRID_SLOPE_CAP ? __builtin_fabsf(q.oix) : 0.0f;
+    const float ay = __builtin_fabsf(q.iy) < GRID_SLOPE_CAP ? __builtin_fabsf(q.oiy) : 0.0f;
+    const float az = __builtin_fabsf(q.iz) < GRID_SLOPE_CAP ? __builtin_fabsf(q.oiz) : 0.0f;
+    q.err2 = __builtin_fmaxf(ax, __builtin_fmaxf(ay, az)) * 0x1.0p-20f;
+  };
+  finish();
+  const double smin = grid_ldexp((double)t_min, e);
+  q.t_min = (float)smin * (smin >= 0.0 ? 0.99999988f : 1.00000012f);
+  const float px = (float)g.n[0] * g.cs[0], py = (float)g.n[1] * g.cs[1], pz = (float)g.n[2] * g.cs[2];
+  const bool nx = q.ix < 0.f, ny = q.iy < 0.f, nz = q.iz < 0.f;
+  const float smax = cull_round_up(grid_ldexp((double)t_max, e));
+  if (!cull32_may_hit_nf_pos(nx ? px : 0.f, nx ? 0.f : px, ny ? py : 0.f, ny ? 0.f : py, nz ? pz : 0.f, nz ? 0.f : pz, q, smax))
+    return false;
+  const float tn = __builtin_fmaxf(__builtin_fmaxf(__builtin_fmaf(nx ? px : 0.f, q.ix, -q.oix), __builtin_fmaf(ny ? py : 0.f, q.iy, -q.oiy)),
+                                   __builtin_fmaf(nz ? pz : 0.f, q.iz, -q.oiz));
+  const float s_entry = tn - __builtin_fmaf(__builtin_fabsf(tn), 0x1.0p-21f, q.err2);
+  double t0 = grid_ldexp((double)s_entry, -e);
+  if (!(t0 > (double)t_min)) t0 = (double)t_min;
+  ox = (float)(((double)r.origin.x + t0 * dx) - g.lo[0]);
+  oy = (float)(((double)r.origin.y + t0 * dy) - g.lo[1]);
+  oz = (float)(((double)r.origin.z + t0 * dz) - g.lo[2]);
+  finish();
+  q.t_min = 0.0f;
+  auto start = [](float o, float inv_cs, uint32_t n) {
+    const float c = __builtin_floorf(o * inv_cs);
+    return c >= (float)n ? n - 1u : (c >= 0.f ? (uint32_t)c : 0u);
+  };
+  w->q = q;
+  w->t0 = t0;
+  w->e = e;
+  w->cell = start(ox, g.inv_cs[0], g.n[0]) | start(oy, g.inv_cs[1], g.n[1]) << 8 | start(oz, g.inv_cs[2], g.n[2]) << 16 | GRID_FIRST;
+  w->s_next = 0.0f;
+  return true;
+}
+
+RT_HD bool grid_next_cell(const GridDesc& g, GridRay* w, float s_max) {
+  if (w->s_next > s_max) return false;
+  uint32_t ix = w->cell & 0xFFu, iy = (w->cell >> 8) & 0xFFu, iz = (w->cell >> 16) & 0xFFu;
+  const bool nx = w->q.ix < 0.f, ny = w->q.iy < 0.f, nz = w->q.iz < 0.f;
+  if (!(w->cell & GRID_FIRST)) {
+    const uint32_t axis = (w->cell >> 24) & 3u;
+    if (axis == 0u) { ix = nx ? ix - 1u : ix + 1u; if (ix >= g.n[0]) return false; }
+    else if (axis == 1u) { iy = ny ? iy - 1u : iy + 1u; if (iy >= g.n[1]) return false; }
+    else { iz = nz ? iz - 1u : iz + 1u; if (iz >= g.n[2]) return false; }
+  }
+  const float sx = __builtin_fmaf((float)(nx ? ix : ix + 1u) * g.cs[0], w->q.ix, -w->q.oix);
+  const float sy = __builtin_fmaf((float)(ny ? iy : iy + 1u) * g.cs[1], w->q.iy, -w->q.oiy);
+  const float sz = __builtin_fmaf((float)(nz ? iz : iz + 1u) * g.cs[2], w->q.iz, -w->q.oiz);
+  const uint32_t axis = sx <= sy ? (sx <= sz ? 0u : 2u) : (sy <= sz ? 1u : 2u);
+  w->s_next = __builtin_fminf(sx, __builtin_fminf(sy, sz));
+  w->cell = ix | iy << 8 | iz << 16 | axis << 24;
+  return true;
+}
+
+RT_HD uint32_t grid_cell_index(const GridDesc& g, uint32_t cell) {
+  return (cell & 0xFFu) + g.n[0] * (((cell >> 8) & 0xFFu) + g.n[1] * ((cell >> 16) & 0xFFu));
+}
+
+}
diff --git a/ray-tracing-series-rust_amd/csrc/hip/abi.cpp b/ray-tracing-series-rust_amd/csrc/hip/abi.cpp
--- a/ray-tracing-series-rust_amd/csrc/hip/abi.cpp
+++ b/ray-tracing-series-rust_amd/csrc/hip/abi.cpp
@@ -3,6 +3,7 @@
 #include <cstring>
 #include <new>
 #include <string>
+#include "../host/grid_build.hpp"
 #include "../host/scenes.hpp"
 #include "abi_internal.hpp"
 
@@ -253,4 +254,11 @@
 const void* rtx_builder_graph(const rtx_builder* b) { return b ? (const void*)&b->graph : nullptr; }
 const void* rtx_flat_arrays(const rtx_flat* f) { return f ? (const void*)&f->scene : nullptr; }
 
-}
+rtx_status rtx_grid_selftest(const rtx_flat* f, double lambda, const double* rays, uint64_t n, uint64_t* out) {
+  if (!f || !out || (!rays && n)) { set_error("rtx_grid_selftest: NULL argument"); return RTX_EINVAL; }
+  std::string why;
+  if (!grid_selftest(f->scene, lambda, rays, n, out, &why)) { set_error("rtx_grid_selftest: no grid: " + why); return RTX_EUNSUPPORTED; }
+  return RTX_OK;
+}
+
+}
diff --git a/ray-tracing-series-rust_amd/csrc/hip/render.hip b/ray-tracing-series-rust_amd/csrc/hip/render.hip
--- a/ray-tracing-series-rust_amd/csrc/hip/render.hip
+++ b/ray-tracing-series-rust_amd/csrc/hip/render.hip
@@ -15,6 +15,10 @@
 #include "../core/cull32.hpp"
 #include "../core/integrator.hpp"
 #include "../host/flat_scene.hpp"
+#include "../host/grid_build.hpp"
+#if defined(RTX_F32_TU)
+#include "../host/grid_build.cpp"
+#endif
 #include "f32_bridge.hpp"
 #ifndef RTX_F32_TU
 #include "abi_internal.hpp"
@@ -34,6 +38,7 @@
   uint32_t n_nodes, n_refs, n_spheres, n_moving;
   uint32_t node_dwords;
   uint32_t n_uni;
+  uint32_t grid_cells, grid_entries;
 };
 
 struct VoteTop {
@@ -53,6 +58,8 @@
   bool vote_top = true, tri_direct = true, mat_lds = true, perlin_lds = true;
   bool mv_common = true, motion = true, motion_axis = true;
   bool single_leaf = true, pass_pipeline = true, validate = false;
+  int lds_grid = -1;
+  double grid_lambda = GRID_LAMBDA_DEFAULT;
   uint32_t chunk = TRACE_CHUNK;
   uint32_t world_threshold = 8;
   uint32_t walk_threshold = 0, regen_min = 0, leaf_weight = 0;
@@ -105,7 +112,7 @@
   bool ok = false;
   uint32_t ring_cap = 0;
   uint32_t levels = 0;
-  LdsSceneDims dims = {0, 0, 0, 0, 0, 0};
+  LdsSceneDims dims = {0, 0, 0, 0, 0, 0, 0, 0};
 };
 
 struct LdsPlan {
@@ -115,6 +122,11 @@
   double motion_t0 = 0.0, motion_t1 = 0.0;
   bool mv_common = false;
   double mv_t0 = 0.0, mv_t1 = 1.0;
+  LdsFit grid;
+  rt::GridDesc grid_desc = {};
+  const uint32_t* grid_cells = nullptr;
+  const uint16_t* grid_slots = nullptr;
+  const float* grid_boxes = nullptr;
 };
 
 struct WalkTuning {
@@ -287,6 +299,9 @@
   sw.mv_common = flag("RTX_MV_COMMON") != 0; sw.motion = flag("RTX_MOTION") != 0; sw.motion_axis = flag("RTX_MOTION_AXIS") != 0;
   sw.single_leaf = flag("RTX_SINGLE_LEAF") != 0; sw.pass_pipeline = flag("RTX_PASS_PIPELINE") != 0;
   sw.validate = getenv("RTX_VALIDATE") != nullptr;
+  sw.lds_grid = flag("RTX_LDS_GRID");
+  if (const char* gl = getenv("RTX_GRID_LAMBDA"))
+    if (atof(gl) >= 0.25 && atof(gl) <= 64.0) sw.grid_lambda = atof(gl);
   sw.chunk = num("RTX_CHUNK", 64, 65536, sw.chunk);
   sw.world_threshold = num("RTX_WORLD_THRESHOLD", 0, 64, sw.world_threshold);
   sw.walk_threshold = num("RTX_WALK_THRESHOLD", 1, 64, 0); sw.regen_min = num("RTX_REGEN_MIN", 1, 64, 0); sw.leaf_weight = num("RTX_LEAF_WEIGHT", 1, 64, 0);
@@ -656,21 +671,40 @@
       fit_lds(&p.motion, want_ring, (uint32_t)lds_max);
     }
   }
+  if (p.plain.ok && (fs.features & ~P_STATIC_SPHERES) == 0 && sw.lds_grid != 0) {
+    SphereGrid sg;
+    std::string why;
+    if (build_sphere_grid(fs, sw.grid_lambda, &sg, &why) && max_end == sg.boxes.size() / 9) {
+      p.grid.levels = 2u + sg.desc.n_always + sg.max_cell;
+      p.grid.dims = {0u, max_end, max_end, 0u, 0u, 0u, (uint32_t)sg.cells.size(), (uint32_t)sg.slots.size()};
+      fit_lds(&p.grid, sw.ring != 0, (uint32_t)lds_max);
+      rtx_status st = RTX_OK;
+      if (p.grid.ok && ((st = upload_array(ds, sg.cells, &p.grid_cells)) != RTX_OK || (st = upload_array(ds, sg.slots, &p.grid_slots)) != RTX_OK ||
+                        (st = upload_array(ds, sg.boxes, &p.grid_boxes)) != RTX_OK))
+        return st;
+      p.grid_desc = sg.desc;
+    }
+  }
   if (p.plain.ok) {
     hipError_t ae = hipSuccess;
 #define LDS_ATTR1(K) if (ae == hipSuccess) ae = hipFuncSetAttribute((const void*)K, hipFuncAttributeMaxDynamicSharedMemorySize, lds_max)
 #define LDS_ATTR(FEAT, RINGF, MOTIONF) LDS_ATTR1((k_trace_lds<FEAT, RINGF, MOTIONF>)); LDS_ATTR1((k_trace_lds<FEAT, RINGF, MOTIONF, ActiveMap>))
     LDS_ATTR(P_SPHERES, true, 0u); LDS_ATTR(P_SPHERES, false, 0u); LDS_ATTR(P_STATIC_SPHERES, true, 0u); LDS_ATTR(P_STATIC_SPHERES, false, 0u);
     LDS_ATTR(P_SPHERES, true, 1u); LDS_ATTR(P_SPHERES, false, 1u); LDS_ATTR(P_SPHERES, true, 3u); LDS_ATTR(P_SPHERES, false, 3u);
+    for (bool rg : {true, false}) {
+      LDS_ATTR1((rg ? k_trace_lds<P_STATIC_SPHERES, true, 0u, ShardMap, true> : k_trace_lds<P_STATIC_SPHERES, false, 0u, ShardMap, true>));
+      LDS_ATTR1((rg ? k_trace_lds<P_STATIC_SPHERES, true, 0u, ActiveMap, true> : k_trace_lds<P_STATIC_SPHERES, false, 0u, ActiveMap, true>));
+    }
 #undef LDS_ATTR
 #undef LDS_ATTR1
-    if (ae != hipSuccess) { (void)hipGetLastError(); p.plain.ok = false; }
+    if (ae != hipSuccess) { (void)hipGetLastError(); p.plain.ok = false; p.grid.ok = false; }
   }
   if (sw.scene_lds >= 0) {
     auto bytes = [](const LdsFit& f) { return f.ok ? ldsk_layout(f.levels, f.ring_cap, f.dims).total : 0u; };
-    fprintf(stderr, "[rtx] RTX_SCENE_LDS: k_trace_lds %s (ring of %u, %u B of LDS); time-aware boxes %s (ring of %u, %u B)\n",
+    fprintf(stderr, "[rtx] RTX_SCENE_LDS: k_trace_lds %s (ring of %u, %u B of LDS); time-aware boxes %s (ring of %u, %u B); grid %s (%ux%ux%u, ring of %u, %u B)\n",
             p.plain.ok ? "on" : "off", p.plain.ring_cap, ldsk_layout(levels, p.plain.ring_cap, p.plain.dims).total,
-            p.motion.ok ? "on" : "off", p.motion.ring_cap, bytes(p.motion));
+            p.motion.ok ? "on" : "off", p.motion.ring_cap, bytes(p.motion), p.grid.ok ? "on" : "off", p.grid_desc.n[0],
+            p.grid_desc.n[1], p.grid_desc.n[2], p.grid.ring_cap, bytes(p.grid));
   }
   return RTX_OK;
 }
@@ -679,24 +713,27 @@
   const LdsPlan& p = ds->lds;
   HIP_TRY(hipMemsetAsync(a.work_counter, 0, sizeof(unsigned int), a.stream));
   const bool motion = p.motion.ok && (double)cam->time1 >= p.motion_t0 && (double)cam->time2 <= p.motion_t1;
-  const LdsFit& f = motion ? p.motion : p.plain;
+  const bool use_grid = p.grid.ok && !motion && (a.feat & ~P_STATIC_SPHERES) == 0;
+  const LdsFit& f = use_grid ? p.grid : (motion ? p.motion : p.plain);
   const bool ring = f.ring_cap != 0u;
   const rt::real m_t0 = (rt::real)p.motion_t0, m_inv = (rt::real)(1.0 / (p.motion_t1 - p.motion_t0));
   const LdsKernelLayout L = ldsk_layout(f.levels, f.ring_cap, f.dims);
   const uint32_t grid = grid_size(a.total, LDSK_BLOCK, (uint64_t)ds->n_cu);
   const WalkTuning& wk = ds->walk;
-#define LAUNCH_LDS2(FEAT, RINGF, MOTIONF)                                                                               \
+#define LAUNCH_LDS2(FEAT, RINGF, MOTIONF, GRIDF)                                                                        \
   with_map(a, [&](auto map) {                                                                                           \
-    hipLaunchKernelGGL(HIP_KERNEL_NAME(k_trace_lds<FEAT, RINGF, MOTIONF, decltype(map)>), dim3(grid), dim3(LDSK_BLOCK), L.total, \
-                       a.stream, ds->view, a.rp, map, a.s_begin, a.total, a.npix, a.samples, a.work_counter, wk.leaf_weight, \
-                       wk.walk_threshold | (wk.single_leaf ? 0x100u : 0u), ds->sw.chunk, f.ring_cap, f.levels, f.dims,  \
-                       m_t0, m_inv, p.mv_common ? 1u : 0u, (rt::real)p.mv_t0, (rt::real)p.mv_t1);                        \
+    hipLaunchKernelGGL(HIP_KERNEL_NAME(k_trace_lds<FEAT, RINGF, MOTIONF, decltype(map), GRIDF>), dim3(grid), dim3(LDSK_BLOCK), \
+                       L.total, a.stream, ds->view, a.rp, map, a.s_begin, a.total, a.npix, a.samples, a.work_counter,   \
+                       wk.leaf_weight, wk.walk_threshold | (wk.single_leaf ? 0x100u : 0u), ds->sw.chunk, f.ring_cap,    \
+                       f.levels, f.dims, m_t0, m_inv, p.mv_common ? 1u : 0u, (rt::real)p.mv_t0, (rt::real)p.mv_t1,      \
+                       p.grid_desc, p.grid_cells, p.grid_slots, p.grid_boxes);                                          \
   })
-#define LAUNCH_LDS(FEAT, MOTIONF) do { if (ring) { LAUNCH_LDS2(FEAT, true, MOTIONF); } else { LAUNCH_LDS2(FEAT, false, MOTIONF); } } while (0)
-  if ((a.feat & ~P_STATIC_SPHERES) == 0) { LAUNCH_LDS(P_STATIC_SPHERES, 0u); }
-  else if (motion && p.motion_axis == 1) { LAUNCH_LDS(P_SPHERES, 3u); }
-  else if (motion) { LAUNCH_LDS(P_SPHERES, 1u); }
-  else { LAUNCH_LDS(P_SPHERES, 0u); }
+#define LAUNCH_LDS(FEAT, MOTIONF, GRIDF) do { if (ring) { LAUNCH_LDS2(FEAT, true, MOTIONF, GRIDF); } else { LAUNCH_LDS2(FEAT, false, MOTIONF, GRIDF); } } while (0)
+  if (use_grid) { LAUNCH_LDS(P_STATIC_SPHERES, 0u, true); }
+  else if ((a.feat & ~P_STATIC_SPHERES) == 0) { LAUNCH_LDS(P_STATIC_SPHERES, 0u, false); }
+  else if (motion && p.motion_axis == 1) { LAUNCH_LDS(P_SPHERES, 3u, false); }
+  else if (motion) { LAUNCH_LDS(P_SPHERES, 1u, false); }
+  else { LAUNCH_LDS(P_SPHERES, 0u, false); }
 #undef LAUNCH_LDS
 #undef LAUNCH_LDS2
   return RTX_OK;
diff --git a/ray-tracing-series-rust_amd/csrc/hip/trace_lds.inc b/ray-tracing-series-rust_amd/csrc/hip/trace_lds.inc
--- a/ray-tracing-series-rust_amd/csrc/hip/trace_lds.inc
+++ b/ray-tracing-series-rust_amd/csrc/hip/trace_lds.inc
@@ -12,7 +12,7 @@
 #define LDSK_MOTION1_NODE_DWORDS 27u
 
 struct LdsKernelLayout {
-  uint32_t off_ring, off_nodes, off_refs, off_spheres, off_moving, total;
+  uint32_t off_ring, off_nodes, off_refs, off_spheres, off_moving, off_gcells, off_gslots, off_gboxes, total;
 };
 __host__ __device__ inline LdsKernelLayout ldsk_layout(uint32_t levels, uint32_t ring_cap, const LdsSceneDims& d) {
   LdsKernelLayout L;
@@ -23,6 +23,9 @@
   L.off_refs = o;
   L.off_spheres = o; o += (d.n_spheres * (uint32_t)sizeof(rt::FlatSphere) + 15u) & ~15u;
   L.off_moving = o; o += (d.n_moving * (uint32_t)sizeof(rt::FlatMovingSphere) + 15u) & ~15u;
+  L.off_gcells = o; o += (d.grid_cells * 4u + 15u) & ~15u;
+  L.off_gslots = o; o += (d.grid_entries * 2u + 15u) & ~15u;
+  L.off_gboxes = o; o += d.grid_cells ? (d.n_refs * 36u + 15u) & ~15u : 0u;
   L.total = o;
   return L;
 }
@@ -41,14 +44,16 @@
   return (int32_t)(short)(unsigned short)(0x8000u | (rt::leaf_first(child) << 2) | (rt::leaf_count(child) - 1u));
 }
 
-template <uint32_t F, bool RING, uint32_t MOTION, class SM = ShardMap>
+template <uint32_t F, bool RING, uint32_t MOTION, class SM = ShardMap, bool GRID = false>
 __global__ __launch_bounds__(LDSK_BLOCK) void k_trace_lds(rt::SceneView sv, rt::RenderParams rp, SM sm,
                                                           uint32_t s_begin, uint32_t total, uint32_t npix,
                                                           double* __restrict__ samples, unsigned int* work_counter,
                                                           uint32_t leaf_weight, uint32_t walk_threshold, uint32_t chunk, uint32_t ring_cap,
                                                           uint32_t stack_levels, LdsSceneDims dims, rt::real motion_t0, rt::real motion_inv_dt,
-                                                          uint32_t mv_common, rt::real mv_t0, rt::real mv_t1) {
+                                                          uint32_t mv_common, rt::real mv_t0, rt::real mv_t1, rt::GridDesc grid,
+                                                          const uint32_t* grid_cells, const uint16_t* grid_slots, const float* grid_boxes) {
   static_assert(!MOTION || (F & rt::F_MOVING_SPHERE), "time-aware boxes only make sense with moving spheres");
+  static_assert(!GRID || (!MOTION && !(F & rt::F_MOVING_SPHERE)), "the grid walk is built over static spheres");
   const bool single_leaf = (walk_threshold & 0x100u) != 0u;
   walk_threshold &= 0xFFu;
   constexpr bool UNI = (F & rt::F_MOVING_SPHERE) != 0;
@@ -71,6 +76,14 @@
   uint32_t* const lds_nodes = (uint32_t*)(ldsk + L.off_nodes);
   rt::FlatSphere* const lds_spheres = (rt::FlatSphere*)(ldsk + L.off_spheres);
   rt::FlatMovingSphere* const lds_moving = (rt::FlatMovingSphere*)(ldsk + L.off_moving);
+  const uint32_t* const lds_gcells = (const uint32_t*)(ldsk + L.off_gcells);
+  const unsigned short* const lds_gslots = (const unsigned short*)(ldsk + L.off_gslots);
+  const unsigned char* const lds_gboxes = ldsk + L.off_gboxes;
+  if (GRID) {
+    for (uint32_t k = threadIdx.x; k < dims.grid_cells; k += LDSK_BLOCK) ((uint32_t*)lds_gcells)[k] = grid_cells[k];
+    for (uint32_t k = threadIdx.x; k < dims.grid_entries; k += LDSK_BLOCK) ((unsigned short*)lds_gslots)[k] = grid_slots[k];
+    for (uint32_t k = threadIdx.x; k < dims.n_refs * 9u; k += LDSK_BLOCK) ((float*)lds_gboxes)[k] = grid_boxes[k];
+  }
   {
     static_assert(sizeof(rt::FlatNode32) == 64 && offsetof(rt::FlatNode32, child) == 48 && offsetof(rt::FlatNode32, axis) == 56,
                   "the padded LDS copy assumes FlatNode32's layout");
@@ -146,6 +159,8 @@
   float s32 = 0.f;
   rt::real mv_ratio = rt::real(0.0);
   int32_t cur = LDSK_DONE;
+  rt::GridRay gw;
+  gw.q = q; gw.t0 = 0.0; gw.e = 0; gw.cell = 0; gw.s_next = 0.f;
   rt::Closest best;
   best.t = 0.0; best.ref = LDSK_NO_REF; best.order = 0; best.hit = false;
 
@@ -237,6 +252,17 @@
         best.t = RT_INFINITY; best.ref = LDSK_NO_REF; best.order = 0;
         stack.reset();
         cur = root;
+        if (GRID) {
+          if (rt::grid_ray_begin(grid, ps.ray, rt::ray_t_min(ps.ray), RT_INFINITY, &gw)) {
+            stack.push(0);
+            const uint32_t neg = (gw.q.ix < 0.f ? 1u : 0u) | (gw.q.iy < 0.f ? 2u : 0u) | (gw.q.iz < 0.f ? 4u : 0u);
+            off_x = (neg & 1u) << 2; off_y = 12u + ((neg & 2u) << 1); off_z = 24u + (neg & 4u);
+          }
+          t_max32 = __builtin_huge_valf();
+          for (uint32_t i = 0; i < GRID_MAX_ALWAYS; ++i)
+            if (i < grid.n_always && rt::grid_always_may_hit(grid, i, q)) stack.push((int32_t)(short)(unsigned short)(0x8000u | (grid.always[i] << 2)));
+          cur = stack.pop();
+        }
         midwalk = true;
       }
     }
@@ -275,6 +301,20 @@
       cur = hf ? cf : (hs ? cs : top);
       stack.n += (int)both - (int)!(hf || hs);
     };
+    auto cell_step = [&]() {
+      if (!rt::grid_next_cell(grid, &gw, t_max32)) { cur = stack.pop(); return; }
+      const uint32_t c = lds_gcells[rt::grid_cell_index(grid, gw.cell)];
+      if (gw.s_next <= t_max32) stack.push(0);
+      const uint32_t first = c & 0xFFFFu, n = c >> 16;
+      for (uint32_t i = 0; i < n; ++i) {
+        const uint32_t slot = lds_gslots[first + i];
+        const unsigned char* b = lds_gboxes + slot * 36u;
+        const float *bx = (const float*)(b + off_x), *by = (const float*)(b + off_y), *bz = (const float*)(b + off_z);
+        if (rt::cull32_may_hit_nf_pos(bx[0], bx[1], by[0], by[1], bz[0], bz[1], gw.q, t_max32))
+          stack.push((int32_t)(short)(unsigned short)(0x8000u | (slot << 2)));
+      }
+      cur = stack.pop();
+    };
     auto leaf_test = [&](uint32_t slot) {
       const rt::PrimRef ref = rt::make_primref(UNI ? rt::PRIM_MOVING_SPHERE : rt::PRIM_SPHERE, slot);
       rt::real t;
@@ -294,7 +334,9 @@
       const uint32_t n_node = (uint32_t)__popcll(wave_ballot(is_node)), n_leaf = (uint32_t)__popcll(wave_ballot(is_leaf));
       if (n_node + n_leaf < threshold) break;
       if (n_node * leaf_weight >= n_leaf) {
-        if (is_node) node_step();
+        if (GRID) {
+          if (is_node) cell_step();
+        } else if (is_node) node_step();
 #if LDSK_NODE_BURST >= 2
         if (cur >= 0) node_step();
 #endif
@@ -307,7 +349,7 @@
             const uint32_t k = ((uint32_t)cur & 3u) + 1u;
             for (uint32_t i = 0; i < k; ++i) leaf_test(f + i);
           }
-          t_max32 = rt::cull_round_up(best.t);
+          t_max32 = GRID ? rt::grid_s_max(gw, best.t) : rt::cull_round_up(best.t);
           cur = stack.pop();
         }
       }
diff --git a/ray-tracing-series-rust_amd/csrc/host/grid_build.cpp b/ray-tracing-series-rust_amd/csrc/host/grid_build.cpp
--- /dev/null
+++ b/ray-tracing-series-rust_amd/csrc/host/grid_build.cpp
@@ -0,0 +1,170 @@
+#include "grid_build.hpp"
+#include <algorithm>
+#include <cmath>
+#include "../core/geometry.hpp"
+
+namespace rtx {
+
+namespace {
+
+float round_down(double x) { float f = (float)x; return (double)f > x ? std::nextafter(f, -INFINITY) : f; }
+float round_up(double x) { float f = (float)x; return (double)f < x ? std::nextafter(f, INFINITY) : f; }
+
+}
+
+bool build_sphere_grid(const FlatScene& fs, double lambda, SphereGrid* out, std::string* why) {
+  *out = SphereGrid();
+  if (!(lambda > 0.0)) lambda = GRID_LAMBDA_DEFAULT;
+  if (fs.top_level.size() != 1 || fs.entries[fs.top_level[0]].kind != rt::ENTRY_BVH) { *why = "not a single BVH"; return false; }
+  const rt::FlatEntry& be = fs.entries[fs.top_level[0]];
+  uint32_t n_slots = 0;
+  for (const rt::FlatNode& nd : fs.nodes)
+    for (int ch = 0; ch < 2; ++ch)
+      if (nd.child[ch] < 0) n_slots = std::max(n_slots, rt::leaf_first(nd.child[ch]) + rt::leaf_count(nd.child[ch]));
+  if (n_slots == 0 || n_slots > 0xFFFFu) { *why = "slot count"; return false; }
+  std::vector<double> box(6 * (size_t)n_slots);
+  std::vector<double> side(n_slots);
+  for (uint32_t k = 0; k < n_slots; ++k) {
+    const rt::PrimRef ref = fs.refs[(uint32_t)be.b + k];
+    if (rt::primref_type(ref) != rt::PRIM_SPHERE) { *why = "not static spheres"; return false; }
+    const rt::FlatSphere& s = fs.spheres[rt::primref_index(ref)];
+    const double c[3] = {(double)s.cx, (double)s.cy, (double)s.cz}, r = std::fabs((double)s.radius);
+    for (int a = 0; a < 3; ++a) { box[6 * k + a] = c[a] - r; box[6 * k + 3 + a] = c[a] + r; }
+    side[k] = 2.0 * r;
+    if (!std::isfinite(c[0]) || !std::isfinite(c[1]) || !std::isfinite(c[2]) || !std::isfinite(r)) { *why = "non-finite sphere"; return false; }
+  }
+  std::vector<double> sorted = side;
+  std::nth_element(sorted.begin(), sorted.begin() + n_slots / 2, sorted.end());
+  const double big = 8.0 * sorted[n_slots / 2];
+  rt::GridDesc& g = out->desc;
+  std::vector<uint32_t> gridded;
+  for (uint32_t k = 0; k < n_slots; ++k) {
+    if (side[k] > big) {
+      if (g.n_always == GRID_MAX_ALWAYS) { *why = "too many large primitives"; return false; }
+      for (int a = 0; a < 3; ++a) { g.abox[g.n_always][a] = round_down(box[6 * k + a]); g.abox[g.n_always][3 + a] = round_up(box[6 * k + 3 + a]); }
+      g.always[g.n_always++] = k;
+    } else {
+      gridded.push_back(k);
+    }
+  }
+  double lo[3] = {INFINITY, INFINITY, INFINITY}, hi[3] = {-INFINITY, -INFINITY, -INFINITY};
+  for (uint32_t k : gridded)
+    for (int a = 0; a < 3; ++a) { lo[a] = std::min(lo[a], box[6 * k + a]); hi[a] = std::max(hi[a], box[6 * k + 3 + a]); }
+  double ext_max = 0.0;
+  for (int a = 0; a < 3; ++a) ext_max = std::max(ext_max, hi[a] - lo[a]);
+  if (!(ext_max > 0.0)) { *why = "empty grid"; return false; }
+  const double m = std::ldexp(ext_max, -14);
+  out->margin = (float)m;
+  double ext[3], volume = 1.0;
+  for (int a = 0; a < 3; ++a) {
+    g.lo[a] = lo[a] - 2.0 * m;
+    ext[a] = (hi[a] + 2.0 * m) - g.lo[a];
+    volume *= ext[a];
+  }
+  const double h = std::cbrt(volume / std::max(1.0, lambda * (double)gridded.size()));
+  for (int a = 0; a < 3; ++a) {
+    g.n[a] = (uint32_t)std::min<double>(GRID_MAX_AXIS, std::max(1.0, std::round(ext[a] / h)));
+    float cs = round_up(ext[a] / g.n[a]);
+    while ((double)((float)g.n[a] * cs) < ext[a]) cs = std::nextafter(cs, INFINITY);
+    g.cs[a] = cs;
+    g.inv_cs[a] = 1.0f / cs;
+  }
+  const uint32_t n_cells = g.n[0] * g.n[1] * g.n[2];
+  out->boxes.assign(9 * (size_t)n_slots, 0.f);
+  for (uint32_t k = 0; k < n_slots; ++k)
+    for (int a = 0; a < 3; ++a) {
+      const float l = round_down((box[6 * k + a] - m) - g.lo[a]), u = round_up((box[6 * k + 3 + a] + m) - g.lo[a]);
+      out->boxes[9 * k + 3 * a] = l; out->boxes[9 * k + 3 * a + 1] = u; out->boxes[9 * k + 3 * a + 2] = l;
+    }
+  std::vector<std::vector<uint16_t>> lists(n_cells);
+  for (uint32_t k : gridded) {
+    uint32_t r0[3], r1[3];
+    for (int a = 0; a < 3; ++a) {
+      const float l = out->boxes[9 * k + 3 * a], u = out->boxes[9 * k + 3 * a + 1];
+      r0[a] = g.n[a]; r1[a] = 0;
+      for (uint32_t i = 0; i < g.n[a]; ++i)
+        if ((float)i * g.cs[a] <= u && (float)(i + 1u) * g.cs[a] >= l) { r0[a] = std::min(r0[a], i); r1[a] = i; }
+      if (r0[a] > r1[a]) { *why = "a box outside the grid"; return false; }
+    }
+    for (uint32_t z = r0[2]; z <= r1[2]; ++z)
+      for (uint32_t y = r0[1]; y <= r1[1]; ++y)
+        for (uint32_t x = r0[0]; x <= r1[0]; ++x) lists[x + g.n[0] * (y + g.n[1] * z)].push_back((uint16_t)k);
+  }
+  out->cells.resize(n_cells);
+  for (uint32_t c = 0; c < n_cells; ++c) {
+    if (out->slots.size() + lists[c].size() > 0xFFFFu) { *why = "more than 65535 cell entries"; return false; }
+    out->cells[c] = (uint32_t)out->slots.size() | (uint32_t)lists[c].size() << 16;
+    out->slots.insert(out->slots.end(), lists[c].begin(), lists[c].end());
+    out->max_cell = std::max(out->max_cell, (uint32_t)lists[c].size());
+  }
+  return true;
+}
+
+
+bool grid_selftest(const FlatScene& fs, double lambda, const double* rays, uint64_t n, uint64_t* out, std::string* why) {
+  SphereGrid grid;
+  if (!build_sphere_grid(fs, lambda, &grid, why)) return false;
+  const rt::GridDesc& g = grid.desc;
+  const rt::FlatEntry& be = fs.entries[fs.top_level[0]];
+  const uint32_t n_slots = (uint32_t)(grid.boxes.size() / 9);
+  std::vector<rt::FlatSphere> sp(n_slots);
+  for (uint32_t k = 0; k < n_slots; ++k) sp[k] = fs.spheres[rt::primref_index(fs.refs[(uint32_t)be.b + k])];
+  for (int i = 0; i < 9; ++i) out[i] = 0;
+  std::vector<uint64_t> offered(n_slots, ~0ull);
+  for (uint64_t j = 0; j < n; ++j) {
+    const double* R = rays + 7 * j;
+    const rt::Ray r = rt::make_ray(rt::v3(R[0], R[1], R[2]), rt::v3(R[3], R[4], R[5]), 0.0);
+    const rt::real t_min = R[6];
+    rt::real best_t = RT_INFINITY;
+    uint32_t best_slot = 0;
+    bool best_hit = false;
+    auto offer = [&](uint32_t k) {
+      rt::real t;
+      ++out[5];
+      offered[k] = j;
+      if (rt::sphere_root(rt::v3(sp[k].cx, sp[k].cy, sp[k].cz), sp[k].radius, r, t_min, best_t, &t) && !(t == best_t && k < best_slot)) {
+        best_t = t; best_slot = k; best_hit = true;
+      }
+    };
+    const rt::Ray32 q0 = rt::make_ray32(r, t_min);
+    for (uint32_t i = 0; i < g.n_always; ++i)
+      if (rt::grid_always_may_hit(g, i, q0)) offer(g.always[i]);
+    rt::GridRay w;
+    if (rt::grid_ray_begin(g, r, t_min, best_t, &w)) {
+      const bool nx = w.q.ix < 0.f, ny = w.q.iy < 0.f, nz = w.q.iz < 0.f;
+      while (rt::grid_next_cell(g, &w, rt::grid_s_max(w, best_t))) {
+        ++out[3];
+        const uint32_t c = grid.cells[rt::grid_cell_index(g, w.cell)];
+        const float s_max = rt::grid_s_max(w, best_t);
+        for (uint32_t i = 0; i < (c >> 16); ++i) {
+          const uint32_t k = grid.slots[(c & 0xFFFFu) + i];
+          const float* b = &grid.boxes[9 * (size_t)k];
+          ++out[4];
+          if (rt::cull32_may_hit_nf_pos(b[nx ? 1 : 0], b[nx ? 2 : 1], b[ny ? 4 : 3], b[ny ? 5 : 4], b[nz ? 7 : 6], b[nz ? 8 : 7], w.q, s_max))
+            offer(k);
+        }
+      }
+    }
+    rt::real ex_t = RT_INFINITY;
+    uint32_t ex_slot = 0;
+    bool ex_hit = false;
+    for (uint32_t k = 0; k < n_slots; ++k) {
+      rt::real t;
+      if (rt::sphere_root(rt::v3(sp[k].cx, sp[k].cy, sp[k].cz), sp[k].radius, r, t_min, ex_t, &t) && !(t == ex_t && k < ex_slot)) {
+        ex_t = t; ex_slot = k; ex_hit = true;
+      }
+    }
+    for (uint32_t k = 0; k < n_slots; ++k) {
+      rt::real t;
+      if (offered[k] != j && rt::sphere_root(rt::v3(sp[k].cx, sp[k].cy, sp[k].cz), sp[k].radius, r, t_min, ex_t, &t)) ++out[1];
+    }
+    if (ex_hit != best_hit || (ex_hit && (!(ex_t == best_t) || ex_slot != best_slot))) ++out[2];
+    ++out[0];
+  }
+  out[6] = grid.cells.size();
+  out[7] = grid.slots.size();
+  out[8] = grid.max_cell;
+  return true;
+}
+
+}
diff --git a/ray-tracing-series-rust_amd/csrc/host/grid_build.hpp b/ray-tracing-series-rust_amd/csrc/host/grid_build.hpp
--- /dev/null
+++ b/ray-tracing-series-rust_amd/csrc/host/grid_build.hpp
@@ -0,0 +1,25 @@
+#pragma once
+#include <string>
+#include <vector>
+#include "../core/grid_dda.hpp"
+#include "flat_scene.hpp"
+
+namespace rtx {
+
+#define GRID_LAMBDA_DEFAULT 2.0
+
+struct SphereGrid {
+  rt::GridDesc desc;
+  std::vector<uint32_t> cells;
+  std::vector<uint16_t> slots;
+  std::vector<float> boxes;
+  uint32_t max_cell = 0;
+  float margin = 0.f;
+};
+
+bool build_sphere_grid(const FlatScene& fs, double lambda, SphereGrid* out, std::string* why);
+
+
+bool grid_selftest(const FlatScene& fs, double lambda, const double* rays, uint64_t n, uint64_t* out, std::string* why);
+
+}
```

Result: slower. 4349 (median of 2 runs) (-44.6%).
